# microsoft/ptgnn

Measured on AMD Instinct MI355X. Metric: edges/sec per MP layer, higher is better.
Workload: dtype f32; 1 GPU; cfg3: Graph2Class-style batch, 48 graphs N=115772, T0=8->T=17, E=625130 (incl. reverse+self), Typilus GGNN arch: 8 GGNN layers H=128 (+concat residual), max; hidden=128, mode=forward (inference), fp32, plan_build_in_step=True, message_rows=shared per (edge type, source) pair, parallelism=single GPU, minibatches_rotated=4

## Files before the change

### include/ptgnn_amd.h

```cpp
#ifndef PTGNN_AMD_H_
#define PTGNN_AMD_H_

#include <stddef.h>
#include <stdint.h>

#ifdef __cplusplus
extern "C" {
#endif

#pragma GCC visibility push(default)

#define PTGNN_AMD_VERSION 102

enum {
  PTGNN_AMD_OK = 0,
  PTGNN_AMD_EINVAL = -1,
  PTGNN_AMD_EUNSUPPORTED = -2,
  PTGNN_AMD_EHIP = -3,
  PTGNN_AMD_EWORKSPACE = -4,
  PTGNN_AMD_ERANGE = -5
};

enum { PTGNN_AMD_SUM = 0, PTGNN_AMD_MEAN = 1, PTGNN_AMD_MAX = 2, PTGNN_AMD_MIN = 3 };

// ... 157 lines not shown
                                int reduce, int epilogue, const float *ln_gamma,
                                const float *ln_beta, float ln_eps, float *out, int64_t ld_out,
                                int32_t *argout , int64_t num_edges,
                                int32_t hub_threshold, const int32_t *hub_entries ,
                                const int32_t *hub_count , void *hub_ws ,
                                size_t hub_ws_bytes, int32_t *hub_tickets ,
                                void *stream);
int ptgnn_amd_gather_reduce_rows_f32(const float *ysrc, int64_t ld_ysrc,
                                     const float *ydst , int64_t ld_ydst,
                                     const int32_t *rowptr, const int32_t *col,
                                     int32_t type_bits, int64_t num_nodes, int32_t msg_dim,
                                     int reduce, int epilogue, const float *ln_gamma,
                                     const float *ln_beta, float ln_eps, float *out, int64_t ld_out,
                                     int32_t *argout , int64_t num_edges,
                                     int32_t hub_threshold, const int32_t *hub_entries ,
                                     const int32_t *hub_count , void *hub_ws ,
                                     size_t hub_ws_bytes, int32_t *hub_tickets ,
                                     int64_t row_begin, int64_t row_end, void *stream);
int ptgnn_amd_row_headers(const int32_t *rowptr, const int32_t *entries, int64_t num_rows, int32_t *hdr, void *stream);
int ptgnn_amd_gather_reduce_hdr_f32(const float *ysrc, int64_t ld_ysrc,
                                    const float *ydst , int64_t ld_ydst,
                                    const int32_t *rowptr, const int32_t *col,
                                    int32_t type_bits, int64_t num_nodes, int32_t msg_dim,
                                    int reduce, int epilogue, const float *ln_gamma,
                                    const float *ln_beta, float ln_eps, float *out, int64_t ld_out,
                                    int32_t *argout , int64_t num_edges,
                                    int32_t hub_threshold, const int32_t *hub_entries ,
                                    const int32_t *hub_count , void *hub_ws ,
                                    size_t hub_ws_bytes, int32_t *hub_tickets ,
                                    int64_t row_begin, int64_t row_end,
                                    const int32_t *row_hdr , void *stream);

int ptgnn_amd_gather_update_supported(int32_t msg_dim, int32_t out_dim);
int ptgnn_amd_gather_update_f32(const float *msg, int64_t ld_msg, const int32_t *rowptr, const int32_t *col,
                                int32_t type_bits, int64_t num_nodes, int32_t msg_dim, int reduce, int epilogue,
                                const float *ln_gamma , const float *ln_beta , float ln_eps,
                                const float *w , const float *bias ,
                                int32_t out_dim, int act, float *out, int64_t ld_out, void *stream);

int ptgnn_amd_segment_mul_f32(const float *msg, int64_t ld_msg, const int32_t *rowptr, const int32_t *perm,
                              int64_t num_rows, int64_t num_edges, int32_t dim, float *out, int64_t ld_out,
                              void *stream);

int ptgnn_amd_gather_reduce_masked_f32(const float *grad, int64_t ld_grad, const int32_t *arg,
                                       const int32_t *rowptr, const int32_t *col,
                                       const int32_t *slot_of, int64_t num_rows, int32_t msg_dim,
                                       float *out, int64_t ld_out, int64_t num_edges,
                                       int32_t hub_threshold, const int32_t *hub_entries,
                                       const int32_t *hub_count, void *hub_ws ,
                                       size_t hub_ws_bytes, int32_t *hub_tickets ,
                                       void *stream);

int ptgnn_amd_linear_f32(const float *x, int64_t rows, int32_t k, int64_t ld_x, const float *w,
                         int32_t n_out, const float *bias, int act, float *y, int64_t ld_y,
                         void *stream);
int ptgnn_amd_linear_add_f32(const float *x, int64_t rows, int32_t k, int64_t ld_x, const float *w, int32_t n_out,
                             const float *bias , int act, const float *addend, int64_t ld_add, float *y,
                             int64_t ld_y, void *stream);

int ptgnn_amd_batch_offsets_i64(const int32_t *in, int64_t n_in, const int64_t *seg_start,
                                const int64_t *seg_add, int32_t num_segments, int64_t n_out,
                                int64_t *out, void *stream);

int ptgnn_amd_edge_linear_f32(const float *x, int64_t ld_x,
        int64_t num_rows ,
        int32_t state_dim,
                              const int64_t *const *src_per_type,
                              const int64_t *const *dst_per_type ,
                              const int64_t *edges_per_type, const float *const *w_per_type,
                              int32_t num_types, int32_t msg_dim, int act, float *msg,
                              int64_t ld_msg, void *stream);

int ptgnn_amd_edge_linear_feat_f32(const float *x, int64_t ld_x, int64_t num_rows, int32_t state_dim,
                                   const int64_t *const *src_per_type,
                                   const int64_t *const *dst_per_type ,
                                   const float *const *feat_per_type, int64_t ld_feat, int32_t feat_dim,
                                   const int64_t *edges_per_type, const float *const *w_per_type,
                                   int32_t num_types, int32_t msg_dim, int act, float *msg,
                                   int64_t ld_msg, void *stream);

int ptgnn_amd_edge_linear_dropout_f32(const float *x, int64_t ld_x,
        int64_t num_rows ,
        int32_t state_dim,
                                      const int64_t *const *src_per_type,
                                      const int64_t *edges_per_type, const float *const *w_per_type,
                                      int32_t num_types, int32_t msg_dim, float *msg, int64_t ld_msg,
                                      int dropout_mode, float dropout_p, uint64_t dropout_seed,
                                      void *stream);

size_t ptgnn_amd_dropout_bitmask_bytes(int64_t rows, int32_t width);
int ptgnn_amd_dropout_bitmask(int64_t rows, int32_t width, float dropout_p, uint64_t dropout_seed,
                              uint32_t *bits, void *stream);
int ptgnn_amd_edge_linear_masked_supported(int32_t state_dim, int32_t msg_dim, int dropout_mode);
int ptgnn_amd_edge_linear_masked_f32(const float *x, int64_t ld_x, int64_t num_rows, int32_t state_dim,
                                     const int64_t *const *src_per_type, const int64_t *edges_per_type,
                                     const float *const *w_per_type, int32_t num_types, int32_t msg_dim,
                                     float *msg, int64_t ld_msg, int dropout_mode, float dropout_p,
                                     const uint32_t *mask_bits, void *stream);
int ptgnn_amd_edge_weight_grad_masked_supported(int32_t state_dim, int32_t msg_dim);
int ptgnn_amd_edge_weight_grad_masked_f32(const float *x, int64_t ld_x, int64_t num_rows, int32_t state_dim,
                                          const int64_t *const *src_per_type, const int64_t *edges_per_type,
                                          const float *grad_msg, int64_t ld_grad_msg, int32_t num_types,
                                          int32_t msg_dim, float dropout_p, const uint32_t *mask_bits,
                                          float *grad_w, void *workspace, size_t workspace_bytes, void *stream);

size_t ptgnn_amd_edge_wgrad_workspace_bytes(int64_t num_edges, int32_t num_types, int32_t msg_dim,
                                            int32_t in_dim);
int ptgnn_amd_edge_weight_grad_f32(const float *x, int64_t ld_x,
        int64_t num_rows ,
        int32_t state_dim,
                                   const int64_t *const *src_per_type,
                                   const int64_t *const *dst_per_type ,
                                   const int64_t *edges_per_type, const float *grad_msg,
                                   int64_t ld_grad_msg, int32_t num_types, int32_t msg_dim,
                                   float dropout_p, uint64_t dropout_seed, float *grad_w,
                                   void *workspace, size_t workspace_bytes, void *stream);

int ptgnn_amd_linear_weight_grad_f32(const float *x, int64_t ld_x, int32_t k, const float *grad_y,
                                     int64_t ld_grad_y, int64_t rows, int32_t n_out, float *grad_w,
                                     float *grad_b , void *workspace,
                                     size_t workspace_bytes, void *stream);

int ptgnn_amd_gru_cell_train_f32(const float *a, int64_t ld_a, const float *h, int64_t ld_h,
                                 const float *w_ih, const float *w_hh, const float *b_ih,
                                 const float *b_hh, int64_t n, int32_t m, int32_t hd, float *out,
                                 int64_t ld_out, float *gates, void *stream);
int ptgnn_amd_gru_cell_backward_gates_f32(const float *grad_out, int64_t ld_grad_out, const float *gates,
                                          const float *h, int64_t ld_h, int64_t n, int32_t hd,
                                          float *d_gi, float *d_gh, float *d_h, void *stream);

int ptgnn_amd_segment_spread_f32(const float *grad, int64_t ld_grad, const int32_t *arg ,
                                 const int32_t *slot_row, const int32_t *perm, int64_t num_slots,
                                 int32_t dim, float *out, int64_t ld_out, void *stream);

int ptgnn_amd_row_epilogue_f32(const float *x, int64_t ld_x, int64_t rows, int32_t dim, int32_t flags,
                               const float *ln_gamma ,
                               const float *ln_beta , float ln_eps, float *y,
                               int64_t ld_y, void *stream);
size_t ptgnn_amd_row_epilogue_workspace_bytes(int64_t rows, int32_t dim);

int ptgnn_amd_act_dropout_backward_f32(const float *grad, const float *y, const uint8_t *keep, float scale, int act,
                                       int64_t n, float *out, void *stream);
int ptgnn_amd_row_epilogue_backward_f32(const float *x, int64_t ld_x, const float *grad_y, int64_t ld_gy,
                                        int64_t rows, int32_t dim, int32_t flags, const float *ln_gamma,
                                        float ln_eps, float *grad_x, int64_t ld_gx,
                                        float *grad_gamma ,
                                        float *grad_beta , void *workspace,
                                        size_t workspace_bytes, void *stream);

int ptgnn_amd_gru_cell_f32(const float *a, int64_t ld_a, const float *h, int64_t ld_h,
                           const float *w_ih, const float *w_hh, const float *b_ih,
                           const float *b_hh, int64_t n, int32_t m, int32_t hd, float *out,
                           int64_t ld_out, void *stream);

size_t ptgnn_amd_weighted_pool_workspace_bytes(int64_t num_segments, int64_t num_elements, int32_t dim);
int ptgnn_amd_weighted_pool_f32(const float *x, int64_t ld_x, const float *w, const int32_t *rowptr,
                                const int32_t *perm, int64_t num_segments, int64_t num_elements, int32_t dim,
                                float *out, int64_t ld_out, void *workspace, size_t workspace_bytes, void *stream);
size_t ptgnn_amd_weighted_pool_backward_workspace_bytes(int64_t num_elements, int32_t dim);
int ptgnn_amd_weighted_pool_backward_f32(const float *x, int64_t ld_x, const float *w, const int64_t *map,
                                         const float *grad_out, int64_t ld_go, int64_t num_elements, int32_t dim,
                                         float *grad_x, int64_t ld_gx, float *grad_w, void *workspace,
                                         size_t workspace_bytes, void *stream);

int ptgnn_amd_attention_pool_supported(int32_t dim, int32_t num_heads);
size_t ptgnn_amd_attention_pool_workspace_bytes(int64_t num_segments, int64_t num_elements, int32_t dim,
                                                int32_t num_heads);
int ptgnn_amd_attention_pool_f32(const float *x, int64_t ld_x, const float *u, const int32_t *rowptr,
                                 const int32_t *perm, int64_t num_segments, int64_t num_elements, int32_t dim,
                                 int32_t num_heads, float *out, float *stats, void *workspace, size_t workspace_bytes,
                                 void *stream);
size_t ptgnn_amd_attention_pool_backward_workspace_bytes(int64_t num_segments, int64_t num_elements, int32_t dim,
                                                         int32_t num_heads);
int ptgnn_amd_attention_pool_backward_f32(const float *x, int64_t ld_x, const float *u, const int32_t *rowptr,
                                          const int32_t *perm, int64_t num_segments, int64_t num_elements, int32_t dim,
                                          int32_t num_heads, const float *out, const float *stats,
                                          const float *grad_out, float *grad_x, int64_t ld_gx, float *grad_u,
                                          void *workspace, size_t workspace_bytes, void *stream);
int ptgnn_amd_head_projection_f32(int mode, const float *a ,
                                  const float *b , const float *w ,
                                  int64_t num_rows, int32_t num_heads, int32_t head_dim, int32_t dim, float scale,
                                  float *out, void *stream);

int ptgnn_amd_segment_scores_supported(int32_t dim, int32_t num_vectors);
size_t ptgnn_amd_segment_scores_workspace_bytes(int64_t num_segments, int64_t num_elements, int32_t dim,
                                                int32_t num_vectors);
int ptgnn_amd_segment_scores_f32(const float *y, int64_t ld_y, const float *v, const int32_t *rowptr,
                                 const int32_t *perm, int64_t num_segments, int64_t num_elements, int32_t dim,
                                 int32_t num_vectors, float *scores, float *lse, void *workspace, size_t workspace_bytes,
                                 void *stream);
size_t ptgnn_amd_segment_scores_backward_workspace_bytes(int64_t num_segments, int64_t num_elements, int32_t dim,
                                                         int32_t num_vectors);
int ptgnn_amd_segment_scores_backward_f32(const float *y, int64_t ld_y, const float *v, const int32_t *rowptr,
                                          const int32_t *perm, int64_t num_segments, int64_t num_elements, int32_t dim,
                                          int32_t num_vectors, const float *scores, const float *lse,
                                          const float *grad_scores, const float *grad_lse, float *grad_y, int64_t ld_gy,
                                          float *grad_v, void *workspace, size_t workspace_bytes, void *stream);

int ptgnn_amd_graph_norm_supported(int32_t dim);
size_t ptgnn_amd_graph_norm_workspace_bytes(int64_t num_segments, int64_t num_elements, int32_t dim);
int ptgnn_amd_graph_norm_f32(const float *x, int64_t ld_x, const float *gamma, const float *alpha, const float *bias,
                             float eps, const int32_t *rowptr, const int32_t *perm, int64_t num_segments,
                             int64_t num_elements, int32_t dim, float *y, int64_t ld_y, float *mean ,
                             void *workspace, size_t workspace_bytes, void *stream);
size_t ptgnn_amd_graph_norm_backward_workspace_bytes(int64_t num_segments, int64_t num_elements, int32_t dim);
int ptgnn_amd_graph_norm_backward_f32(const float *x, int64_t ld_x, const float *grad_y, int64_t ld_gy,
                                      const float *gamma, const float *alpha, float eps, const float *mean,
                                      const int32_t *rowptr, const int32_t *perm, int64_t num_segments,
                                      int64_t num_elements, int32_t dim,
                                      float *grad_x, int64_t ld_gx, float *grad_gamma, float *grad_alpha,
                                      float *grad_bias, void *workspace, size_t workspace_bytes, void *stream);

int ptgnn_amd_block_attention_supported(int32_t dk, int32_t dv);
int64_t ptgnn_amd_attention_windows_bound(int64_t num_graphs, int64_t num_rows, int32_t max_num_nodes);
int ptgnn_amd_attention_windows(const int32_t *rowptr, int64_t num_graphs, int64_t num_rows, int32_t max_num_nodes,
                                int32_t *windows, int64_t capacity, void *stream);
int ptgnn_amd_block_attention_f32(const float *kqv, int64_t ld_kqv, const int32_t *windows, int64_t num_windows,
                                  int64_t num_rows, int32_t max_num_nodes, int32_t num_heads, int32_t dk, int32_t dv,
                                  float dropout_p, uint64_t seed, float *out, int64_t ld_out, float *lse, void *stream);
size_t ptgnn_amd_block_attention_backward_workspace_bytes(int64_t num_rows, int32_t num_heads);
int ptgnn_amd_block_attention_backward_f32(const float *kqv, int64_t ld_kqv, const float *out, int64_t ld_out,
                                           const float *lse, const float *grad_out, int64_t ld_go,
                                           const int32_t *windows, int64_t num_windows, int64_t num_rows,
                                           int32_t max_num_nodes, int32_t num_heads, int32_t dk, int32_t dv,
                                           float dropout_p, uint64_t seed, float *grad_kqv, int64_t ld_gkqv,
                                           void *workspace, size_t workspace_bytes, void *stream);

int ptgnn_amd_egc_gather_combine_f32(const float *msg, int64_t ld_msg, const int32_t *rowptr, const int32_t *col,
                                     int32_t type_bits, int64_t num_nodes, int32_t num_heads, int32_t num_bases,
                                     int32_t head_dim, int reduce, const float *coef, int64_t ld_coef, float *out,
                                     int64_t ld_out, float *agg_out , int32_t *argout ,
                                     int64_t num_edges, int32_t hub_threshold,
                                     const int32_t *hub_entries , const int32_t *hub_count ,
                                     void *hub_ws , size_t hub_ws_bytes,
                                     int32_t *hub_tickets , void *stream);
int ptgnn_amd_egc_combine_f32(const float *agg, int64_t ld_agg, const float *coef, int64_t ld_coef, int64_t num_rows,
                              int32_t num_heads, int32_t num_bases, int32_t head_dim, float *out, int64_t ld_out,
                              void *stream);
int ptgnn_amd_egc_combine_backward_f32(const float *agg, int64_t ld_agg, const float *coef, int64_t ld_coef,
                                       const float *grad, int64_t ld_grad, int64_t num_rows, int32_t num_heads,
                                       int32_t num_bases, int32_t head_dim, float *grad_agg, int64_t ld_grad_agg,
                                       float *grad_coef, int64_t ld_grad_coef, void *stream);

int ptgnn_amd_pna_aggregate_f32(const float *ysrc, int64_t ld_y, const float *ydst , int64_t ld_yd,
                                const int32_t *rowptr, const int32_t *col, int32_t type_bits, int64_t num_nodes,
                                int32_t msg_dim, float delta, int epilogue, const float *ln_gamma ,
                                const float *ln_beta , float ln_eps, int32_t round_mode, float *out,
                                int64_t ld_out, int32_t *argmax , int32_t *argmin ,
                                float *agg_out , int64_t num_edges, void *stream);
int ptgnn_amd_pna_aggregate_backward_f32(const float *msg, int64_t ld_msg, const int32_t *rowptr, const int32_t *col,
                                         int64_t num_nodes, int32_t msg_dim, float delta, const float *agg,
                                         int64_t ld_agg, const int32_t *argmax, const int32_t *argmin,
                                         const float *grad, int64_t ld_grad, float *grad_msg, int64_t ld_grad_msg,
                                         int32_t round_mode, int64_t num_edges, void *stream);

int ptgnn_amd_gather_rows_f32(const float *x, int64_t ld_x, const int64_t *idx, int64_t n_idx,
                              int32_t dim, float *out, int64_t ld_out, void *stream);

int ptgnn_amd_embedding_bag_supported(int32_t dim, int32_t slots);
int ptgnn_amd_embedding_bag_f32(const float *table, int64_t ld_table, int64_t vocab, const int64_t *ids,
                                const int64_t *lengths, int64_t num_bags, int32_t slots, int32_t dim, int mode,
                                float *out, int64_t ld_out, int32_t *arg , void *stream);
int ptgnn_amd_embedding_bag_keys(const int64_t *ids, const int64_t *lengths, int64_t num_bags, int32_t slots,
                                 int64_t vocab, int64_t *src, int64_t *key, void *stream);
size_t ptgnn_amd_embedding_bag_backward_workspace_bytes(int64_t num_bags, int32_t slots, int32_t dim, int mode);
int ptgnn_amd_embedding_bag_backward_f32(const float *grad, int64_t ld_grad, const int64_t *lengths,
                                         const int32_t *arg , int64_t num_bags, int32_t slots,
                                         int64_t vocab, int32_t dim, int mode, const int32_t *rowptr,
                                         const int32_t *col, const int32_t *perm, float *grad_table, int64_t ld_gt,
                                         int32_t hub_threshold, const int32_t *hub_entries ,
                                         const int32_t *hub_count , void *hub_ws ,
                                         size_t hub_ws_bytes, int32_t *hub_tickets , void *workspace,
                                         size_t workspace_bytes, void *stream);

int ptgnn_amd_char_embed_supported(int32_t num_chars, int32_t window, int32_t dim);
int ptgnn_amd_char_embed_f32(const int64_t *chars, int64_t num_samples, int32_t length, int32_t num_chars,
                             int32_t window, const float *table, const float *bias , int32_t dim, int act,
                             float *out, int64_t ld_out, void *stream);
int32_t ptgnn_amd_char_embed_backward_chunk(void);
size_t ptgnn_amd_char_embed_backward_workspace_bytes(int64_t num_samples, int32_t num_chars, int32_t window,
                                                     int32_t dim);
int ptgnn_amd_char_embed_backward_f32(const float *grad, int64_t ld_grad, const float *a1, int64_t ld_a1,
                                      const int64_t *chars, int64_t num_samples, int32_t length, int32_t num_chars,
                                      int32_t window, int32_t dim, int act, float *grad_table,
                                      float *grad_bias , void *workspace, size_t workspace_bytes,
                                      void *stream);
int ptgnn_amd_window_linear_f32(const float *x, int64_t rows, int32_t c_in, int32_t window, int64_t ld_x,
                                const float *w, int32_t n_out, const float *bias , int act, float *y,
                                int64_t ld_y, void *stream);
int ptgnn_amd_window_weight_grad_f32(const float *x, int64_t rows, int32_t c_in, int32_t window, const float *grad_y,
                                     int64_t ld_grad_y, int32_t n_out, float *grad_w, float *grad_b ,
                                     void *workspace, size_t workspace_bytes, void *stream);
int ptgnn_amd_window_max_f32(const float *x, int64_t ld_x, int64_t num_samples, int32_t rows_per_sample, int32_t valid,
                             int32_t dim, float *out, int64_t ld_out, int32_t *arg , void *stream);
int ptgnn_amd_window_max_backward_f32(const float *grad, int64_t ld_grad, const int32_t *arg, int64_t num_samples,
                                      int32_t rows_per_sample, int32_t dim, float *grad_x, int64_t ld_gx, void *stream);

#define PTGNN_AMD_HEAD_TOTALS_BYTES 64
#define PTGNN_AMD_HEAD_METRICS_BYTES 32
enum { PTGNN_AMD_LOSS_SOFTMAX = 0, PTGNN_AMD_LOSS_SIGMOID = 1 };

size_t ptgnn_amd_logit_loss_workspace_bytes(int64_t rows);
int ptgnn_amd_logit_loss_f32(const float *logits, int64_t ld, int64_t rows, int32_t classes, int mode,
                             const void *targets , int64_t ld_t, float *lse,
                             int64_t *argmax , float *max_prob ,
                             float *row_loss , float *loss, void *totals, void *metrics ,
// ... 107 lines not shown
```

### ptgnn_amd/_lib.py

```python
import ctypes
import os
import threading

import torch

_HERE = os.path.dirname(os.path.abspath(__file__))
LIB_PATH = os.environ.get("PTGNN_AMD_LIB") or os.path.join(_HERE, "csrc", "libptgnn_amd.so")

_c = ctypes
_i64, _i32, _vp, _f32 = _c.c_int64, _c.c_int32, _c.c_void_p, _c.c_float

SIGNATURES = {
    "ptgnn_amd_version": (_c.c_int, []),
    "ptgnn_amd_last_error": (_c.c_char_p, []),
    "ptgnn_amd_set_gemm_mode": (_c.c_int, [_c.c_int]),
    "ptgnn_amd_get_gemm_mode": (_c.c_int, []),
    "ptgnn_amd_launch_count": (_i64, [_c.c_int]),
    "ptgnn_amd_launch_name": (_c.c_char_p, [_c.c_int]),
    "ptgnn_amd_csr_workspace_bytes": (_c.c_size_t, [_i64, _i64]),
    "ptgnn_amd_csr_control_bytes": (_c.c_size_t, []),
    "ptgnn_amd_set_plan_path": (_c.c_int, [_c.c_int]),
    "ptgnn_amd_type_bits": (_c.c_int, [_i32]),
    "ptgnn_amd_csr_build": (_c.c_int, [_vp, _vp, _vp, _i32, _i64, _i64, _c.c_int, _vp, _vp, _vp, _vp,
                                       _i32, _vp, _vp, _vp, _vp, _vp, _c.c_size_t, _vp]),
    "ptgnn_amd_hub_workspace_bytes": (_c.c_size_t, [_i64, _i32, _c.c_int]),
    "ptgnn_amd_hub_ticket_count": (_i64, [_i64, _i32]),
    "ptgnn_amd_hub_list": (_c.c_int, [_vp, _i64, _i32, _vp, _vp, _vp]),
    "ptgnn_amd_validate_indices": (_c.c_int, [_vp, _i64, _i64, _vp, _vp]),
    "ptgnn_amd_shard_index_workspace_bytes": (_c.c_size_t, [_i64]),
    "ptgnn_amd_shard_index": (_c.c_int, [_vp, _vp, _vp, _i32, _i64, _i64, _vp, _i32, _i64, _vp, _vp, _vp, _i64, _vp,
                                         _vp, _vp, _c.c_size_t, _vp]),
    "ptgnn_amd_unique_sources_workspace_bytes": (_c.c_size_t, [_i64, _i32]),
    "ptgnn_amd_edge_table_bytes": (_c.c_size_t, []),
    "ptgnn_amd_unique_sources": (_c.c_int, [_vp, _i64, _i32, _i32, _i64, _vp, _vp, _i64, _vp, _vp, _vp, _c.c_size_t,
                                            _vp]),
    "ptgnn_amd_edge_linear_shared_supported": (_c.c_int, [_i32, _i32, _i32]),
    "ptgnn_amd_edge_linear_shared_f32": (_c.c_int, [_vp, _i64, _i64, _i32, _vp, _vp, _i32, _i32, _c.c_int, _vp, _i64,
                                                    _vp]),
    "ptgnn_amd_gather_reduce_f32": (_c.c_int, [_vp, _i64, _vp, _i64, _vp, _vp, _i32, _i64, _i32, _c.c_int,
                                               _c.c_int, _vp, _vp, _f32, _vp, _i64, _vp, _i64, _i32, _vp,
                                               _vp, _vp, _c.c_size_t, _vp, _vp]),
    "ptgnn_amd_gather_reduce_rows_f32": (_c.c_int, [_vp, _i64, _vp, _i64, _vp, _vp, _i32, _i64, _i32, _c.c_int,
                                                    _c.c_int, _vp, _vp, _f32, _vp, _i64, _vp, _i64, _i32, _vp,
                                                    _vp, _vp, _c.c_size_t, _vp, _i64, _i64, _vp]),
    "ptgnn_amd_row_headers": (_c.c_int, [_vp, _vp, _i64, _vp, _vp]),
    "ptgnn_amd_gather_reduce_hdr_f32": (_c.c_int, [_vp, _i64, _vp, _i64, _vp, _vp, _i32, _i64, _i32, _c.c_int,
                                                   _c.c_int, _vp, _vp, _f32, _vp, _i64, _vp, _i64, _i32, _vp,
                                                   _vp, _vp, _c.c_size_t, _vp, _i64, _i64, _vp, _vp]),
    "ptgnn_amd_gather_update_supported": (_c.c_int, [_i32, _i32]),
    "ptgnn_amd_gather_update_f32": (_c.c_int, [_vp, _i64, _vp, _vp, _i32, _i64, _i32, _c.c_int, _c.c_int, _vp, _vp, _f32,
                                               _vp, _vp, _i32, _c.c_int, _vp, _i64, _vp]),
    "ptgnn_amd_gather_reduce_masked_f32": (_c.c_int, [_vp, _i64, _vp, _vp, _vp, _vp, _i64, _i32, _vp, _i64,
                                                      _i64, _i32, _vp, _vp, _vp, _c.c_size_t, _vp, _vp]),
    "ptgnn_amd_segment_mul_f32": (_c.c_int, [_vp, _i64, _vp, _vp, _i64, _i64, _i32, _vp, _i64, _vp]),
    "ptgnn_amd_linear_f32": (_c.c_int, [_vp, _i64, _i32, _i64, _vp, _i32, _vp, _c.c_int, _vp, _i64,
                                        _vp]),
    "ptgnn_amd_linear_add_f32": (_c.c_int, [_vp, _i64, _i32, _i64, _vp, _i32, _vp, _c.c_int, _vp, _i64, _vp, _i64,
                                            _vp]),
    "ptgnn_amd_batch_offsets_i64": (_c.c_int, [_vp, _i64, _vp, _vp, _i32, _i64, _vp, _vp]),
    "ptgnn_amd_edge_linear_f32": (_c.c_int, [_vp, _i64, _i64, _i32, _vp, _vp, _vp, _vp, _i32, _i32, _c.c_int, _vp,
                                             _i64, _vp]),
    "ptgnn_amd_edge_linear_feat_f32": (_c.c_int, [_vp, _i64, _i64, _i32, _vp, _vp, _vp, _i64, _i32, _vp, _vp, _i32, _i32,
                                                  _c.c_int, _vp, _i64, _vp]),
    "ptgnn_amd_edge_linear_dropout_f32": (_c.c_int, [_vp, _i64, _i64, _i32, _vp, _vp, _vp, _i32, _i32, _vp, _i64,
                                                     _c.c_int, _c.c_float, _c.c_uint64, _vp]),
    "ptgnn_amd_dropout_bitmask_bytes": (_c.c_size_t, [_i64, _i32]),
    "ptgnn_amd_dropout_bitmask": (_c.c_int, [_i64, _i32, _c.c_float, _c.c_uint64, _vp, _vp]),
    "ptgnn_amd_edge_linear_masked_supported": (_c.c_int, [_i32, _i32, _c.c_int]),
    "ptgnn_amd_edge_linear_masked_f32": (_c.c_int, [_vp, _i64, _i64, _i32, _vp, _vp, _vp, _i32, _i32, _vp, _i64,
                                                    _c.c_int, _c.c_float, _vp, _vp]),
    "ptgnn_amd_edge_weight_grad_masked_supported": (_c.c_int, [_i32, _i32]),
    "ptgnn_amd_edge_weight_grad_masked_f32": (_c.c_int, [_vp, _i64, _i64, _i32, _vp, _vp, _vp, _i64, _i32, _i32,
                                                         _c.c_float, _vp, _vp, _vp, _c.c_size_t, _vp]),
    "ptgnn_amd_edge_wgrad_workspace_bytes": (_c.c_size_t, [_i64, _i32, _i32, _i32]),
    "ptgnn_amd_edge_weight_grad_f32": (_c.c_int, [_vp, _i64, _i64, _i32, _vp, _vp, _vp, _vp, _i64, _i32, _i32,
                                                  _c.c_float, _c.c_uint64, _vp, _vp, _c.c_size_t, _vp]),
    "ptgnn_amd_linear_weight_grad_f32": (_c.c_int, [_vp, _i64, _i32, _vp, _i64, _i64, _i32, _vp, _vp, _vp,
                                                    _c.c_size_t, _vp]),
    "ptgnn_amd_segment_spread_f32": (_c.c_int, [_vp, _i64, _vp, _vp, _vp, _i64, _i32, _vp, _i64, _vp]),
    "ptgnn_amd_row_epilogue_f32": (_c.c_int, [_vp, _i64, _i64, _i32, _i32, _vp, _vp, _c.c_float, _vp, _i64, _vp]),
    "ptgnn_amd_row_epilogue_workspace_bytes": (_c.c_size_t, [_i64, _i32]),
    "ptgnn_amd_act_dropout_backward_f32": (_c.c_int, [_vp, _vp, _vp, _c.c_float, _c.c_int, _i64, _vp, _vp]),
    "ptgnn_amd_row_epilogue_backward_f32": (_c.c_int, [_vp, _i64, _vp, _i64, _i64, _i32, _i32, _vp, _c.c_float, _vp,
                                                       _i64, _vp, _vp, _vp, _c.c_size_t, _vp]),
    "ptgnn_amd_gru_cell_f32": (_c.c_int, [_vp, _i64, _vp, _i64, _vp, _vp, _vp, _vp, _i64, _i32, _i32,
                                          _vp, _i64, _vp]),
    "ptgnn_amd_gru_cell_train_f32": (_c.c_int, [_vp, _i64, _vp, _i64, _vp, _vp, _vp, _vp, _i64, _i32, _i32,
                                                _vp, _i64, _vp, _vp]),
    "ptgnn_amd_gru_cell_backward_gates_f32": (_c.c_int, [_vp, _i64, _vp, _vp, _i64, _i64, _i32, _vp, _vp, _vp,
                                                         _vp]),
    "ptgnn_amd_egc_gather_combine_f32": (_c.c_int, [_vp, _i64, _vp, _vp, _i32, _i64, _i32, _i32, _i32, _c.c_int, _vp,
                                                    _i64, _vp, _i64, _vp, _vp, _i64, _i32, _vp, _vp, _vp, _c.c_size_t,
                                                    _vp, _vp]),
    "ptgnn_amd_egc_combine_f32": (_c.c_int, [_vp, _i64, _vp, _i64, _i64, _i32, _i32, _i32, _vp, _i64, _vp]),
    "ptgnn_amd_egc_combine_backward_f32": (_c.c_int, [_vp, _i64, _vp, _i64, _vp, _i64, _i64, _i32, _i32, _i32, _vp,
                                                      _i64, _vp, _i64, _vp]),
    "ptgnn_amd_pna_aggregate_f32": (_c.c_int, [_vp, _i64, _vp, _i64, _vp, _vp, _i32, _i64, _i32, _f32, _c.c_int, _vp,
                                               _vp, _f32, _i32, _vp, _i64, _vp, _vp, _vp, _i64, _vp]),
    "ptgnn_amd_pna_aggregate_backward_f32": (_c.c_int, [_vp, _i64, _vp, _vp, _i64, _i32, _f32, _vp, _i64, _vp, _vp, _vp,
                                                        _i64, _vp, _i64, _i32, _i64, _vp]),
    "ptgnn_amd_gather_rows_f32": (_c.c_int, [_vp, _i64, _vp, _i64, _i32, _vp, _i64, _vp]),
    "ptgnn_amd_weighted_pool_workspace_bytes": (_c.c_size_t, [_i64, _i64, _i32]),
    "ptgnn_amd_weighted_pool_f32": (_c.c_int, [_vp, _i64, _vp, _vp, _vp, _i64, _i64, _i32, _vp, _i64, _vp, _c.c_size_t,
                                               _vp]),
    "ptgnn_amd_weighted_pool_backward_workspace_bytes": (_c.c_size_t, [_i64, _i32]),
    "ptgnn_amd_weighted_pool_backward_f32": (_c.c_int, [_vp, _i64, _vp, _vp, _vp, _i64, _i64, _i32, _vp, _i64, _vp, _vp,
                                                        _c.c_size_t, _vp]),
    "ptgnn_amd_attention_pool_supported": (_c.c_int, [_i32, _i32]),
    "ptgnn_amd_attention_pool_workspace_bytes": (_c.c_size_t, [_i64, _i64, _i32, _i32]),
    "ptgnn_amd_attention_pool_f32": (_c.c_int, [_vp, _i64, _vp, _vp, _vp, _i64, _i64, _i32, _i32, _vp, _vp, _vp,
                                                _c.c_size_t, _vp]),
    "ptgnn_amd_attention_pool_backward_workspace_bytes": (_c.c_size_t, [_i64, _i64, _i32, _i32]),
    "ptgnn_amd_attention_pool_backward_f32": (_c.c_int, [_vp, _i64, _vp, _vp, _vp, _i64, _i64, _i32, _i32, _vp, _vp,
                                                         _vp, _vp, _i64, _vp, _vp, _c.c_size_t, _vp]),
    "ptgnn_amd_head_projection_f32": (_c.c_int, [_c.c_int, _vp, _vp, _vp, _i64, _i32, _i32, _i32, _f32, _vp, _vp]),
    "ptgnn_amd_segment_scores_supported": (_c.c_int, [_i32, _i32]),
    "ptgnn_amd_segment_scores_workspace_bytes": (_c.c_size_t, [_i64, _i64, _i32, _i32]),
    "ptgnn_amd_segment_scores_f32": (_c.c_int, [_vp, _i64, _vp, _vp, _vp, _i64, _i64, _i32, _i32, _vp, _vp, _vp,
                                                _c.c_size_t, _vp]),
    "ptgnn_amd_segment_scores_backward_workspace_bytes": (_c.c_size_t, [_i64, _i64, _i32, _i32]),
    "ptgnn_amd_segment_scores_backward_f32": (_c.c_int, [_vp, _i64, _vp, _vp, _vp, _i64, _i64, _i32, _i32, _vp, _vp,
                                                         _vp, _vp, _vp, _i64, _vp, _vp, _c.c_size_t, _vp]),
    "ptgnn_amd_graph_norm_supported": (_c.c_int, [_i32]),
    "ptgnn_amd_graph_norm_workspace_bytes": (_c.c_size_t, [_i64, _i64, _i32]),
    "ptgnn_amd_graph_norm_f32": (_c.c_int, [_vp, _i64, _vp, _vp, _vp, _f32, _vp, _vp, _i64, _i64, _i32, _vp, _i64, _vp,
                                            _vp, _c.c_size_t, _vp]),
    "ptgnn_amd_graph_norm_backward_workspace_bytes": (_c.c_size_t, [_i64, _i64, _i32]),
    "ptgnn_amd_graph_norm_backward_f32": (_c.c_int, [_vp, _i64, _vp, _i64, _vp, _vp, _f32, _vp, _vp, _vp, _i64, _i64,
                                                     _i32, _vp, _i64, _vp, _vp, _vp, _vp, _c.c_size_t, _vp]),
    "ptgnn_amd_block_attention_supported": (_c.c_int, [_i32, _i32]),
    "ptgnn_amd_attention_windows_bound": (_i64, [_i64, _i64, _i32]),
    "ptgnn_amd_attention_windows": (_c.c_int, [_vp, _i64, _i64, _i32, _vp, _i64, _vp]),
    "ptgnn_amd_block_attention_f32": (_c.c_int, [_vp, _i64, _vp, _i64, _i64, _i32, _i32, _i32, _i32, _f32, _c.c_uint64,
                                                 _vp, _i64, _vp, _vp]),
    "ptgnn_amd_block_attention_backward_workspace_bytes": (_c.c_size_t, [_i64, _i32]),
    "ptgnn_amd_block_attention_backward_f32": (_c.c_int, [_vp, _i64, _vp, _i64, _vp, _vp, _i64, _vp, _i64, _i64, _i32,
                                                          _i32, _i32, _i32, _f32, _c.c_uint64, _vp, _i64, _vp,
                                                          _c.c_size_t, _vp]),
    "ptgnn_amd_embedding_bag_supported": (_c.c_int, [_i32, _i32]),
    "ptgnn_amd_embedding_bag_f32": (_c.c_int, [_vp, _i64, _i64, _vp, _vp, _i64, _i32, _i32, _c.c_int, _vp, _i64, _vp,
                                               _vp]),
    "ptgnn_amd_embedding_bag_keys": (_c.c_int, [_vp, _vp, _i64, _i32, _i64, _vp, _vp, _vp]),
    "ptgnn_amd_embedding_bag_backward_workspace_bytes": (_c.c_size_t, [_i64, _i32, _i32, _c.c_int]),
    "ptgnn_amd_embedding_bag_backward_f32": (_c.c_int, [_vp, _i64, _vp, _vp, _i64, _i32, _i64, _i32, _c.c_int, _vp, _vp,
                                                        _vp, _vp, _i64, _i32, _vp, _vp, _vp, _c.c_size_t, _vp, _vp,
                                                        _c.c_size_t, _vp]),
    "ptgnn_amd_char_embed_supported": (_c.c_int, [_i32, _i32, _i32]),
    "ptgnn_amd_char_embed_f32": (_c.c_int, [_vp, _i64, _i32, _i32, _i32, _vp, _vp, _i32, _c.c_int, _vp, _i64, _vp]),
    "ptgnn_amd_char_embed_backward_chunk": (_i32, []),
    "ptgnn_amd_char_embed_backward_workspace_bytes": (_c.c_size_t, [_i64, _i32, _i32, _i32]),
    "ptgnn_amd_char_embed_backward_f32": (_c.c_int, [_vp, _i64, _vp, _i64, _vp, _i64, _i32, _i32, _i32, _i32, _c.c_int,
                                                     _vp, _vp, _vp, _c.c_size_t, _vp]),
    "ptgnn_amd_window_linear_f32": (_c.c_int, [_vp, _i64, _i32, _i32, _i64, _vp, _i32, _vp, _c.c_int, _vp, _i64, _vp]),
    "ptgnn_amd_window_weight_grad_f32": (_c.c_int, [_vp, _i64, _i32, _i32, _vp, _i64, _i32, _vp, _vp, _vp, _c.c_size_t,
                                                    _vp]),
    "ptgnn_amd_window_max_f32": (_c.c_int, [_vp, _i64, _i64, _i32, _i32, _i32, _vp, _i64, _vp, _vp]),
    "ptgnn_amd_window_max_backward_f32": (_c.c_int, [_vp, _i64, _vp, _i64, _i32, _i32, _vp, _i64, _vp]),
    "ptgnn_amd_logit_loss_workspace_bytes": (_c.c_size_t, [_i64]),
    "ptgnn_amd_logit_loss_f32": (_c.c_int, [_vp, _i64, _i64, _i32, _c.c_int, _vp, _i64, _vp, _vp, _vp, _vp, _vp, _vp, _vp,
                                            _vp, _c.c_size_t, _vp]),
    "ptgnn_amd_logit_loss_backward_f32": (_c.c_int, [_vp, _i64, _i64, _i32, _c.c_int, _vp, _i64, _vp, _vp, _vp, _vp, _i64,
                                                     _vp]),
    "ptgnn_amd_candidate_scores_supported": (_c.c_int, [_i32]),
    "ptgnn_amd_candidate_scores_workspace_bytes": (_c.c_size_t, [_i64]),
    "ptgnn_amd_candidate_scores_f32": (_c.c_int, [_vp, _i64, _i64, _vp, _vp, _vp, _vp, _vp, _i64, _i64, _i32, _vp, _vp,
                                                  _vp, _vp, _vp, _vp, _vp, _vp, _vp, _c.c_size_t, _vp]),
    "ptgnn_amd_candidate_scores_backward_workspace_bytes": (_c.c_size_t, [_i64, _i32]),
    "ptgnn_amd_candidate_scores_backward_f32": (_c.c_int, [_vp, _i64, _i64, _vp, _vp, _vp, _vp, _vp, _i64, _i64, _i32,
                                                           _vp, _vp, _vp, _vp, _vp, _vp, _vp, _vp, _vp, _c.c_size_t,
                                                           _vp]),
    "ptgnn_amd_vocab_loss_workspace_bytes": (_c.c_size_t, [_i64, _i32]),
    "ptgnn_amd_vocab_loss_f32": (_c.c_int, [_vp, _i64, _i64, _i32, _vp, _vp, _vp, _vp, _vp, _vp, _vp, _c.c_size_t,
                                            _vp]),
    "ptgnn_amd_vocab_loss_backward_workspace_bytes": (_c.c_size_t, [_i64, _i32]),
    "ptgnn_amd_vocab_loss_backward_f32": (_c.c_int, [_vp, _i64, _i64, _i32, _vp, _vp, _vp, _vp, _vp, _vp, _vp, _i64, _vp,
                                                     _vp, _vp, _c.c_size_t, _vp]),
    "ptgnn_amd_copy_loss_finish_workspace_bytes": (_c.c_size_t, [_i64]),
    "ptgnn_amd_copy_loss_finish_f32": (_c.c_int, [_vp, _vp, _vp, _vp, _i64, _vp, _i64, _i32, _vp, _vp, _vp, _vp,
                                                  _c.c_size_t, _vp]),
    "ptgnn_amd_decode_step_workspace_bytes": (_c.c_size_t, [_i64, _i32, _i32]),
    "ptgnn_amd_decode_step_f32": (_c.c_int, [_vp, _i64, _vp, _vp, _vp, _vp, _vp, _vp, _i64, _i64, _i32, _i32, _i64, _i64,
                                             _i32, _i32, _vp, _vp, _vp, _vp, _vp, _vp, _vp, _c.c_size_t, _vp]),
    "ptgnn_amd_beam_step_workspace_bytes": (_c.c_size_t, [_i64, _i64, _i32, _i32, _i32]),
    "ptgnn_amd_beam_step_f32": (_c.c_int, [_vp, _i64, _vp, _vp, _vp, _vp, _vp, _vp, _i64, _i64, _i32, _i32, _i32, _i64,
                                           _i64, _i32, _i32, _vp, _vp, _vp, _vp, _vp, _vp, _vp, _vp, _vp, _vp, _vp, _vp,
                                           _c.c_size_t, _vp]),
    "ptgnn_amd_half_supported": (_c.c_int, [_c.c_int, _i32, _i32, _c.c_int]),
    "ptgnn_amd_half_linear": (_c.c_int, [_vp, _i64, _i32, _i64, _vp, _i32, _vp, _c.c_int, _c.c_int, _vp, _i64, _vp]),
    "ptgnn_amd_half_gru_cell": (_c.c_int, [_vp, _i64, _vp, _i64, _vp, _vp, _vp, _vp, _i64, _i32, _i32, _c.c_int, _vp,
                                           _i64, _vp]),
    "ptgnn_amd_linear_weight_grad16": (_c.c_int, [_vp, _i64, _i32, _vp, _i64, _i64, _i32, _c.c_int, _vp, _vp, _vp,
                                                  _c.c_size_t, _vp]),
    "ptgnn_amd_wgrad16_workspace_bytes": (_c.c_size_t, [_i64, _i32, _i32]),
    "ptgnn_amd_wgrad16_chunk_rows": (_i64, [_i64, _i32, _i32]),
    "ptgnn_amd_gru_cell_train16": (_c.c_int, [_vp, _i64, _vp, _i64, _vp, _vp, _vp, _vp, _i64, _i32, _i32, _c.c_int, _vp,
                                              _i64, _vp, _vp]),
    "ptgnn_amd_linear_add16": (_c.c_int, [_vp, _i64, _i32, _i64, _vp, _i32, _vp, _c.c_int, _c.c_int, _vp, _i64, _vp, _i64,
                                          _vp]),
    "ptgnn_amd_edge_linear16_supported": (_c.c_int, [_i32, _i32, _i32, _c.c_int]),
    "ptgnn_amd_edge_linear16": (_c.c_int, [_vp, _i64, _i64, _i32, _vp, _vp, _vp, _i32, _i32, _c.c_int, _c.c_int, _vp,
                                           _i64, _vp]),
    "ptgnn_amd_edge_linear16_shared": (_c.c_int, [_vp, _i64, _i64, _i32, _vp, _vp, _i32, _i32, _c.c_int, _c.c_int, _vp,
                                                  _i64, _vp]),
    "ptgnn_amd_edge_dst_linear16_supported": (_c.c_int, [_i32, _i32, _i32, _c.c_int]),
    "ptgnn_amd_edge_dst_linear16": (_c.c_int, [_vp, _i64, _i64, _i32, _vp, _vp, _vp, _vp, _i32, _i32, _c.c_int, _c.c_int,
                                               _vp, _i64, _vp]),
}

MIN_VERSION = 102

_lock = threading.Lock()
_lib = None


EUNSUPPORTED = -2


class PtgnnAmdError(RuntimeError):
    pass


def load():
    global _lib
    if _lib is not None:
        return _lib
    with _lock:
        if _lib is None:
            if not os.path.exists(LIB_PATH):
                raise PtgnnAmdError(
                    f"{LIB_PATH} is missing: build it with `python -m ptgnn_amd.build` "
                    "(ptgnn_amd has no CPU/eager fallback by design)")
            lib = ctypes.CDLL(LIB_PATH)
            for name, (res, args) in SIGNATURES.items():
                fn = getattr(lib, name)
                fn.restype, fn.argtypes = res, args
            have = lib.ptgnn_amd_version()
            if have < MIN_VERSION:
                raise PtgnnAmdError(f"{LIB_PATH} reports ABI version {have}, this host needs >= {MIN_VERSION}: "
                                    "rebuild it with `python -m ptgnn_amd.build --force`")
# ... 9 lines not shown
```

### ptgnn_amd/csrc/dense_f32.hip

```cpp
#include <stdlib.h>

#include <type_traits>

#include "dense_common.h"
#include "stream_gemm.h"

namespace ptgnn_amd {
namespace {

template <bool ALIGNED, int ACT, int NJ>
__global__ __launch_bounds__(256, (NJ == 1 ? 4 : 3)) void k_linear_tlp(
    const float *__restrict__ x, int64_t rows, int K, int64_t ld_x, const float *__restrict__ w,
    int n_out, const float *__restrict__ bias, float *__restrict__ y, int64_t ld_y,
    int64_t num_tiles, int col_tiles, int vec_store) {
  constexpr int BN = 64 * NJ;
  constexpr int B_FLOATS = BN * LDS_LD;
  constexpr int SLAB_LD = 32 * NJ + 4;
  constexpr int SLAB_FLOATS = 32 * SLAB_LD;
  constexpr int OPER = TILE_FLOATS + B_FLOATS;
  constexpr int kLds = OPER > 4 * SLAB_FLOATS ? OPER : 4 * SLAB_FLOATS;
  __shared__ __attribute__((aligned(16))) float smem[kLds];
  float *const As = smem, *const Bs = smem + TILE_FLOATS;

  const int64_t tile = xcd_swizzle(blockIdx.x, gridDim.x);
// ... 255 lines not shown
  }
}

__global__ __launch_bounds__(256) void k_gru_gates_backward(const float *__restrict__ g, int64_t ld_g,
                                                            const float *__restrict__ gates,
                                                            const float *__restrict__ h, int64_t ld_h,
                                                            int64_t n, int H, float *__restrict__ d_gi,
                                                            float *__restrict__ d_gh,
                                                            float *__restrict__ d_h) {
  const int q = H / 4;
  const int64_t total = n * q;
  for (int64_t i = blockIdx.x * (int64_t)256 + threadIdx.x; i < total; i += (int64_t)gridDim.x * 256) {
    const int64_t row = i / q;
    const int c = (int)(i - row * q) * 4;
    const float4 gv = *reinterpret_cast<const float4 *>(g + row * ld_g + c);
    const float4 hv = *reinterpret_cast<const float4 *>(h + row * ld_h + c);
    const float *gp = gates + row * (int64_t)(4 * H) + c;
    const float4 r = *reinterpret_cast<const float4 *>(gp);
    const float4 z = *reinterpret_cast<const float4 *>(gp + H);
    const float4 nn = *reinterpret_cast<const float4 *>(gp + 2 * H);
    const float4 hn = *reinterpret_cast<const float4 *>(gp + 3 * H);
    float4 o_r, o_z, o_n, o_hn, o_h;
#define PTGNN_GRU_BWD(C)                                         \
    {                                                            \
      const float dn = gv.C * (1.0f - z.C);                      \
      const float dz = gv.C * (hv.C - nn.C);                     \
      const float dnp = dn * (1.0f - nn.C * nn.C);               \
      o_h.C = gv.C * z.C;                                        \
      o_n.C = dnp;                                               \
      o_hn.C = dnp * r.C;                                        \
      o_r.C = (dnp * hn.C) * (r.C * (1.0f - r.C));               \
      o_z.C = dz * (z.C * (1.0f - z.C));                         \
    }
    PTGNN_GRU_BWD(x) PTGNN_GRU_BWD(y) PTGNN_GRU_BWD(z) PTGNN_GRU_BWD(w)
#undef PTGNN_GRU_BWD
    float *gi = d_gi + row * (int64_t)(3 * H) + c, *gh = d_gh + row * (int64_t)(3 * H) + c;
    *reinterpret_cast<float4 *>(gi) = o_r;
    *reinterpret_cast<float4 *>(gi + H) = o_z;
    *reinterpret_cast<float4 *>(gi + 2 * H) = o_n;
    *reinterpret_cast<float4 *>(gh) = o_r;
    *reinterpret_cast<float4 *>(gh + H) = o_z;
    *reinterpret_cast<float4 *>(gh + 2 * H) = o_hn;
    *reinterpret_cast<float4 *>(d_h + row * (int64_t)H + c) = o_h;
  }
}

}

int num_compute_units() {
  static int cus = 0;
  if (cus == 0) {
    int dev = 0;
    hipDeviceProp_t prop;
    if (hipGetDevice(&dev) == hipSuccess && hipGetDeviceProperties(&prop, dev) == hipSuccess)
      cus = prop.multiProcessorCount;
    if (cus <= 0) cus = 256;
  }
  return cus;
}

static int linear_nj() {
  static int nj = -1;
  if (nj < 0) {
    const char *e = getenv("PTGNN_AMD_LINEAR_NJ");
    nj = e ? atoi(e) : 0;
    if (nj < 0 || nj > 2) nj = 0;
  }
  return nj;
}

}

using namespace ptgnn_amd;

static int linear_launch(const float *x, int64_t rows, int32_t k, int64_t ld_x, const float *w, int32_t n_out,
                         const float *bias, int act, float *y, int64_t ld_y, void *stream_) {
  if (stream_linear(x, rows, k, ld_x, w, n_out, bias, act, y, ld_y, (hipStream_t)stream_)) {
    PTGNN_LAUNCH_CHECK();
    return PTGNN_AMD_OK;
  }
  int nj = linear_nj();
  if (nj == 0) nj = n_out <= 128 ? 1 : 2;
  const int bn = 64 * nj;
  const int64_t row_tiles = (rows + 127) / 128;
  const int col_tiles = (n_out + bn - 1) / bn;
  const int64_t num_tiles = row_tiles * col_tiles;
  PTGNN_REQUIRE(num_tiles < ((int64_t)1 << 31), PTGNN_AMD_EUNSUPPORTED, "linear: too many tiles");
  const unsigned grid = (unsigned)xcd_padded_blocks(num_tiles);
  const bool al = (k % 4 == 0) && (ld_x % 4 == 0) && aligned16(x) && aligned16(w);
  const int vec_store = ((ld_y % 4 == 0) && aligned16(y) ? 1 : 0) | ((bias && aligned16(bias) && n_out % 4 == 0) ? 2 : 0);
  hipStream_t st = (hipStream_t)stream_;
#define PTGNN_LINEAR_LAUNCH(AL, ACT, NJ)                                                         \
  k_linear_tlp<AL, ACT, NJ><<<grid, 256, 0, st>>>(x, rows, k, ld_x, w, n_out, bias, y, ld_y,     \
                                                  num_tiles, col_tiles, vec_store)
#define PTGNN_LINEAR_ACT(AL, NJ)                                                          \
  do {                                                                                    \
    if (act == PTGNN_AMD_ACT_TANH) PTGNN_LINEAR_LAUNCH(AL, PTGNN_AMD_ACT_TANH, NJ);       \
    else if (act == PTGNN_AMD_ACT_RELU) PTGNN_LINEAR_LAUNCH(AL, PTGNN_AMD_ACT_RELU, NJ);  \
    else PTGNN_LINEAR_LAUNCH(AL, PTGNN_AMD_ACT_NONE, NJ);                                 \
  } while (0)
  if (al) { if (nj == 1) PTGNN_LINEAR_ACT(true, 1); else PTGNN_LINEAR_ACT(true, 2); }
  else    { if (nj == 1) PTGNN_LINEAR_ACT(false, 1); else PTGNN_LINEAR_ACT(false, 2); }
#undef PTGNN_LINEAR_ACT
#undef PTGNN_LINEAR_LAUNCH
  PTGNN_LAUNCH_CHECK();
  count_launch(PTGNN_AMD_KERNEL_TILE_LINEAR);
  return PTGNN_AMD_OK;
}

extern "C" int ptgnn_amd_linear_f32(const float *x, int64_t rows, int32_t k, int64_t ld_x,
                                    const float *w, int32_t n_out, const float *bias, int act,
                                    float *y, int64_t ld_y, void *stream_) {
  PTGNN_REQUIRE(rows >= 0 && k > 0 && n_out > 0, PTGNN_AMD_EINVAL, "linear: bad sizes");
  PTGNN_REQUIRE(act >= 0 && act <= PTGNN_AMD_ACT_RELU, PTGNN_AMD_EINVAL, "linear: bad act");
  if (rows == 0) return PTGNN_AMD_OK;
  PTGNN_REQUIRE(x && w && y && ld_x >= k && ld_y >= n_out, PTGNN_AMD_EINVAL, "linear: null/ld");
  return linear_launch(x, rows, k, ld_x, w, n_out, bias, act, y, ld_y, stream_);
}

extern "C" int ptgnn_amd_window_linear_f32(const float *x, int64_t rows, int32_t c_in, int32_t window, int64_t ld_x,
                                           const float *w, int32_t n_out, const float *bias, int act, float *y,
                                           int64_t ld_y, void *stream_) {
  PTGNN_REQUIRE(rows >= 0 && c_in > 0 && window > 0 && n_out > 0 && (int64_t)c_in * window < ((int64_t)1 << 31),
                PTGNN_AMD_EINVAL, "window_linear: bad sizes");
  PTGNN_REQUIRE(act >= 0 && act <= PTGNN_AMD_ACT_RELU, PTGNN_AMD_EINVAL, "window_linear: bad act");
  if (rows == 0) return PTGNN_AMD_OK;
  PTGNN_REQUIRE(x && w && y && ld_x >= c_in && ld_y >= n_out, PTGNN_AMD_EINVAL, "window_linear: null/ld");
  PTGNN_REQUIRE(window == 1 || ld_x == c_in, PTGNN_AMD_EINVAL,
                "window_linear: a window spans rows only where they are packed (ld_x=%lld, c_in=%d)", (long long)ld_x,
                c_in);
  return linear_launch(x, rows, c_in * window, ld_x, w, n_out, bias, act, y, ld_y, stream_);
}

extern "C" int ptgnn_amd_linear_add_f32(const float *x, int64_t rows, int32_t k, int64_t ld_x, const float *w,
                                        int32_t n_out, const float *bias, int act, const float *addend,
                                        int64_t ld_add, float *y, int64_t ld_y, void *stream_) {
  PTGNN_REQUIRE(rows >= 0 && k > 0 && n_out > 0, PTGNN_AMD_EINVAL, "linear_add: bad sizes");
  PTGNN_REQUIRE(act >= 0 && act <= PTGNN_AMD_ACT_RELU, PTGNN_AMD_EINVAL, "linear_add: bad act");
  if (rows == 0) return PTGNN_AMD_OK;
  PTGNN_REQUIRE(x && w && y && addend && ld_x >= k && ld_y >= n_out && ld_add >= n_out, PTGNN_AMD_EINVAL,
                "linear_add: null/ld");
  PTGNN_REQUIRE(addend != y, PTGNN_AMD_EINVAL, "linear_add: in-place accumulation is not supported");
  if (stream_linear(x, rows, k, ld_x, w, n_out, bias, act, y, ld_y, (hipStream_t)stream_, addend, ld_add)) {
    PTGNN_LAUNCH_CHECK();
    return PTGNN_AMD_OK;
  }
  set_error("linear_add: rows=%lld k=%d n_out=%d is not a shape of the streaming GEMM (use ptgnn_amd_linear_f32 and add)",
            (long long)rows, k, n_out);
  return PTGNN_AMD_EUNSUPPORTED;
}

static int gru_launch(const float *a, int64_t ld_a, const float *h, int64_t ld_h, const float *w_ih,
                      const float *w_hh, const float *b_ih, const float *b_hh, int64_t n, int32_t m,
                      int32_t hd, float *out, int64_t ld_out, float *gates, void *stream_) {
  PTGNN_REQUIRE(n >= 0 && m > 0 && hd > 0, PTGNN_AMD_EINVAL, "gru_cell: bad sizes");
  if (n == 0) return PTGNN_AMD_OK;
  PTGNN_REQUIRE(a && h && w_ih && w_hh && b_ih && b_hh && out, PTGNN_AMD_EINVAL, "gru_cell: null");
  PTGNN_REQUIRE(ld_a >= m && ld_h >= hd && ld_out >= hd, PTGNN_AMD_EINVAL, "gru_cell: bad ld");
  PTGNN_REQUIRE(out != h, PTGNN_AMD_EINVAL, "gru_cell: in-place update is not supported");
  if (stream_gru(a, ld_a, h, ld_h, w_ih, w_hh, b_ih, b_hh, n, m, hd, out, ld_out, gates, (hipStream_t)stream_)) {
    PTGNN_LAUNCH_CHECK();
    return PTGNN_AMD_OK;
  }
  const int64_t row_tiles = (n + 127) / 128;
  const int col_tiles = (hd + 31) / 32;
  const int64_t num_tiles = row_tiles * col_tiles;
  PTGNN_REQUIRE(num_tiles < ((int64_t)1 << 31), PTGNN_AMD_EUNSUPPORTED, "gru_cell: too many tiles");
  const unsigned grid = (unsigned)xcd_padded_blocks(num_tiles);
  const bool al = (m % 4 == 0) && (hd % 4 == 0) && (ld_a % 4 == 0) && (ld_h % 4 == 0) &&
                  aligned16(a) && aligned16(h) && aligned16(w_ih) && aligned16(w_hh);
  if (al)
    k_gru<true><<<grid, 256, 0, (hipStream_t)stream_>>>(a, ld_a, h, ld_h, w_ih, w_hh, b_ih, b_hh, n, m, hd,
                                                        out, ld_out, num_tiles, col_tiles, gates);
  else
    k_gru<false><<<grid, 256, 0, (hipStream_t)stream_>>>(a, ld_a, h, ld_h, w_ih, w_hh, b_ih, b_hh, n, m, hd,
                                                         out, ld_out, num_tiles, col_tiles, gates);
  PTGNN_LAUNCH_CHECK();
  count_launch(PTGNN_AMD_KERNEL_TILE_GRU);
  return PTGNN_AMD_OK;
}

extern "C" int ptgnn_amd_gru_cell_f32(const float *a, int64_t ld_a, const float *h, int64_t ld_h,
                                      const float *w_ih, const float *w_hh, const float *b_ih,
                                      const float *b_hh, int64_t n, int32_t m, int32_t hd,
                                      float *out, int64_t ld_out, void *stream_) {
  return gru_launch(a, ld_a, h, ld_h, w_ih, w_hh, b_ih, b_hh, n, m, hd, out, ld_out, nullptr, stream_);
}

extern "C" int ptgnn_amd_gru_cell_train_f32(const float *a, int64_t ld_a, const float *h, int64_t ld_h,
                                            const float *w_ih, const float *w_hh, const float *b_ih,
                                            const float *b_hh, int64_t n, int32_t m, int32_t hd,
                                            float *out, int64_t ld_out, float *gates, void *stream_) {
  PTGNN_REQUIRE(gates != nullptr || n == 0, PTGNN_AMD_EINVAL, "gru_cell_train: gates is null");
  return gru_launch(a, ld_a, h, ld_h, w_ih, w_hh, b_ih, b_hh, n, m, hd, out, ld_out, gates, stream_);
}

extern "C" int ptgnn_amd_gru_cell_backward_gates_f32(const float *grad_out, int64_t ld_grad_out,
                                                     const float *gates, const float *h, int64_t ld_h,
                                                     int64_t n, int32_t hd, float *d_gi, float *d_gh,
                                                     float *d_h, void *stream_) {
  PTGNN_REQUIRE(n >= 0 && hd > 0, PTGNN_AMD_EINVAL, "gru_cell_backward_gates: bad sizes");
  if (n == 0) return PTGNN_AMD_OK;
  PTGNN_REQUIRE(grad_out && gates && h && d_gi && d_gh && d_h, PTGNN_AMD_EINVAL,
                "gru_cell_backward_gates: null pointer");
  PTGNN_REQUIRE(hd % 4 == 0 && ld_grad_out % 4 == 0 && ld_h % 4 == 0 && ld_grad_out >= hd && ld_h >= hd &&
                    aligned16(grad_out) && aligned16(gates) && aligned16(h) && aligned16(d_gi) &&
                    aligned16(d_gh) && aligned16(d_h),
                PTGNN_AMD_EUNSUPPORTED, "gru_cell_backward_gates: needs hd %% 4 == 0 and 16-byte aligned rows");
  const int64_t items = n * (hd / 4);
  int64_t blocks = (items + 255) / 256;
  if (blocks > 65536) blocks = 65536;
  k_gru_gates_backward<<<(unsigned)blocks, 256, 0, (hipStream_t)stream_>>>(grad_out, ld_grad_out, gates, h,
                                                                          ld_h, n, hd, d_gi, d_gh, d_h);
  PTGNN_LAUNCH_CHECK();
  return PTGNN_AMD_OK;
}
```

### ptgnn_amd/csrc/stream_gemm.h

```cpp
#pragma once
#include "common.h"

namespace ptgnn_amd {

constexpr int kStreamMaxTypes = 64;

struct StreamEdgeTable {
  const int64_t *src[kStreamMaxTypes];
  const int64_t *dst[kStreamMaxTypes];
  const float *w[kStreamMaxTypes];
  int64_t edge_off[kStreamMaxTypes + 1];
  int32_t unit_off[kStreamMaxTypes + 1];
  int32_t wg_off[kStreamMaxTypes + 1];
  int32_t num_types;
};

int num_compute_units();

int stream_gemm_mode();
void stream_gemm_set_mode(int mode);

int stream_linear(const float *x, int64_t rows, int32_t k, int64_t ld_x, const float *w, int32_t n_out,
                  const float *bias, int act, float *y, int64_t ld_y, hipStream_t st, const float *addend = nullptr,
                  int64_t ld_add = 0);
int stream_gru(const float *a, int64_t ld_a, const float *h, int64_t ld_h, const float *w_ih,
               const float *w_hh, const float *b_ih, const float *b_hh, int64_t n, int32_t m, int32_t hd,
               float *out, int64_t ld_out, float *gates, hipStream_t st);
int stream_edge_supported(int32_t state_dim, int32_t msg_dim, int use_dst);
int stream_edge_masked_supported(int32_t state_dim, int32_t msg_dim);
struct StreamEdgeMask {
  int mode;
  const uint32_t *bits;
  int ld, col0;
  float scale;
};
int stream_edge(const StreamEdgeTable &tab, const float *x, int64_t ld_x, int64_t num_rows, int32_t state_dim,
                int use_dst, int32_t msg_dim, int act, float *msg, int64_t ld_msg, int64_t msg_row_base,
                hipStream_t st, const StreamEdgeMask *mask = nullptr);

int edge_table_budget();
int stream_edge_indirect(const StreamEdgeTable *tab_dev, const float *const *w_per_type, int num_types, const float *x,
                         int64_t ld_x, int64_t num_rows, int32_t state_dim, int32_t msg_dim, int act, float *msg,
                         int64_t ld_msg, hipStream_t st);

}
```

### ptgnn_amd/csrc/stream_gemm.hip

```cpp
#include <stdlib.h>

#include "dense_common.h"
#include <atomic>

#include "stream_gemm.h"

namespace ptgnn_amd {
namespace {

using u32x4 = __attribute__((ext_vector_type(4))) uint32_t;

constexpr int kLdsBudget = 160 * 1024;
constexpr size_t kEpiBytes = 16 + 8 * 8 * 36 * sizeof(float);

__device__ __forceinline__ f32x16 zero16() {
  f32x16 v;
#pragma unroll
  for (int r = 0; r < 16; ++r) v[r] = 0.f;
  return v;
}

struct ARows {
  const float *c0, *c1, *n0, *n1;
};
// ... 12 lines not shown
template <int NBLK, int NACC, int PH, bool GRU>
__device__ __forceinline__ void chunk_f32(f32x16 (&acc)[NACC], float4 (&buf)[4], float4 (&bcur)[NBLK],
                                          const float *bl, int cbs, int kofs, int kofs_next, const ARows &rows,
                                          int cnext, int ch0, int nch) {
#pragma unroll
  for (int g = 0; g < 4; ++g) {
    float4 bn[NBLK];
    const int ko = g < 3 ? kofs + (g + 1) * 8 : kofs_next;
#pragma unroll
    for (int n = 0; n < NBLK; ++n) bn[n] = *reinterpret_cast<const float4 *>(bl + n * cbs + ko);
    __builtin_amdgcn_sched_barrier(0);
    const float4 a = buf[g];
#define PTGNN_STEP(C)                                                                     \
    _Pragma("unroll") for (int n = 0; n < NBLK; ++n) {                                    \
      const int t = (GRU && PH == 1 && n == NBLK - 1) ? NACC - 1 : n;                     \
      acc[t] = __builtin_amdgcn_mfma_f32_32x32x2f32(a.C, bcur[n].C, acc[t], 0, 0, 0);     \
    }
    PTGNN_STEP(x) PTGNN_STEP(y) PTGNN_STEP(z) PTGNN_STEP(w)
#undef PTGNN_STEP
    __builtin_amdgcn_sched_barrier(0);
#pragma unroll
    for (int n = 0; n < NBLK; ++n) bcur[n] = bn[n];
  }
#pragma unroll
  for (int g = 0; g < 4; ++g) {
    buf[g] = load_piece(rows, cnext, ch0, nch, g);
    __builtin_amdgcn_sched_barrier(0);
  }
}

struct Slab {
  int ld;
  __device__ __forceinline__ Slab(int K, int ) { ld = K + 4; }
  static size_t bytes(int K, int rows) { return (size_t)rows * (K + 4) * 4; }

  __device__ __forceinline__ void put4(float *smem, int r, int k, float4 v) const {
    *reinterpret_cast<float4 *>(smem + r * ld + k) = v;
  }
};

template <int NT, typename SrcFn, typename LiveFn>
__device__ __forceinline__ void fill_slab(float *smem, const Slab &sl, int rows, int kq, SrcFn src, LiveFn live) {
  constexpr int UB = 8;
  const int total = rows * kq;
  for (int i0 = threadIdx.x; i0 < total; i0 += NT * UB) {
    float4 v[UB];
    int rr[UB], qq[UB];
#pragma unroll
    for (int u = 0; u < UB; ++u) {
      const int i = i0 + u * NT;
      const int ic = i < total ? i : total - 1;
      rr[u] = ic / kq;
      qq[u] = ic - rr[u] * kq;
    }
#pragma unroll
    for (int u = 0; u < UB; ++u) {
      v[u] = *reinterpret_cast<const float4 *>(src(rr[u], qq[u]));
      __builtin_amdgcn_sched_barrier(0);
    }
#pragma unroll
    for (int u = 0; u < UB; ++u) {
      if (i0 + u * NT < total) sl.put4(smem, rr[u], qq[u] * 4, live(rr[u]) ? v[u] : make_float4(0.f, 0.f, 0.f, 0.f));
    }
  }
}

template <int NBLK, int NACC, bool GRU>
__device__ __forceinline__ void unit_kloop(f32x16 (&acc)[NACC], float4 (&a0)[4], float4 (&a1)[4],
                                           const float *smem, const Slab &sl, int li, int hi,
                                           const ARows &rows, int ch0, int nch) {
  const float *bl = smem + li * sl.ld + hi * 4;
  const int cbs = 32 * sl.ld;
  const int e0 = GRU ? ch0 : nch;
  float4 bcur[NBLK];
#pragma unroll
  for (int n = 0; n < NBLK; ++n) bcur[n] = *reinterpret_cast<const float4 *>(bl + n * cbs);
  for (int c = 0; c < e0; c += 2) {
    const int kn = c + 2 < nch ? c * 32 + 64 : 0;
    chunk_f32<NBLK, NACC, 0, GRU>(acc, a0, bcur, bl, cbs, c * 32, c * 32 + 32, rows, c + 2, ch0, nch);
    chunk_f32<NBLK, NACC, 0, GRU>(acc, a1, bcur, bl, cbs, c * 32 + 32, kn, rows, c + 3, ch0, nch);
  }
  if constexpr (GRU) {
    for (int c = ch0; c < nch; c += 2) {
      const int kn = c + 2 < nch ? c * 32 + 64 : 0;
      chunk_f32<NBLK, NACC, 1, GRU>(acc, a0, bcur, bl, cbs, c * 32, c * 32 + 32, rows, c + 2, ch0, nch);
      chunk_f32<NBLK, NACC, 1, GRU>(acc, a1, bcur, bl, cbs, c * 32 + 32, kn, rows, c + 3, ch0, nch);
    }
  }
}

__device__ __forceinline__ void prologue_loads(float4 (&a0)[4], float4 (&a1)[4], const ARows &rows, int ch0,
                                               int nch) {
#pragma unroll
  for (int g = 0; g < 4; ++g) {
    a0[g] = load_piece(rows, 0, ch0, nch, g);
    __builtin_amdgcn_sched_barrier(0);
  }
#pragma unroll
  for (int g = 0; g < 4; ++g) {
    a1[g] = load_piece(rows, 1, ch0, nch, g);
    __builtin_amdgcn_sched_barrier(0);
  }
}

__device__ __forceinline__ void unit_fence() {
  __builtin_amdgcn_s_waitcnt(0x0F70);
  __builtin_amdgcn_sched_barrier(0);
}

__device__ __forceinline__ int claim_unit(int *counter) {
  int v = 0;
  if ((threadIdx.x & 63) == 0) v = atomicAdd(counter, 1);
  return __builtin_amdgcn_readfirstlane(v);
}

#ifndef PTGNN_TAIL_SPLIT
#define PTGNN_TAIL_SPLIT 1
#endif
constexpr bool kSplitGru = PTGNN_TAIL_SPLIT != 0;

constexpr int kTqLd = 36;
constexpr int kTqFloats = 8 * kTqLd;

__device__ __forceinline__ float4 tq_transpose(float *tq, int lane, int li, int hi, float v0, float v1, float v2,
                                               float v3) {
  float *w = tq + (4 * hi) * kTqLd + li;
  w[0] = v0; w[kTqLd] = v1; w[2 * kTqLd] = v2; w[3 * kTqLd] = v3;
  __builtin_amdgcn_wave_barrier();
  const float4 o = *reinterpret_cast<const float4 *>(tq + (lane >> 3) * kTqLd + (lane & 7) * 4);
  __builtin_amdgcn_wave_barrier();
  return o;
}

__device__ __forceinline__ void tq_untranspose(float *tq, int lane, int li, int hi, float4 in, float (&v)[4]) {
  *reinterpret_cast<float4 *>(tq + (lane >> 3) * kTqLd + (lane & 7) * 4) = in;
  __builtin_amdgcn_wave_barrier();
  const float *r = tq + (4 * hi) * kTqLd + li;
  v[0] = r[0]; v[1] = r[kTqLd]; v[2] = r[2 * kTqLd]; v[3] = r[3 * kTqLd];
  __builtin_amdgcn_wave_barrier();
}

using u32x4 = __attribute__((ext_vector_type(4))) uint32_t;

__device__ __forceinline__ __amdgpu_buffer_rsrc_t rows_descriptor(float *base , int64_t ld, int64_t rows_left,
                                                                  int width ) {
  const uint64_t b = reinterpret_cast<uint64_t>(base);
  const uint32_t lo = __builtin_amdgcn_readfirstlane((uint32_t)b), hi = __builtin_amdgcn_readfirstlane((uint32_t)(b >> 32));
  const int64_t rows = rows_left < 32 ? rows_left : 32;
  const int64_t bytes = rows > 0 ? ((rows - 1) * ld + width) * 4 : 0;
  return __builtin_amdgcn_make_buffer_rsrc(reinterpret_cast<float *>(((uint64_t)hi << 32) | lo), 0,
                                           __builtin_amdgcn_readfirstlane((int)bytes), 0x00020000);
}

__device__ __forceinline__ void store_row4(__amdgpu_buffer_rsrc_t rsrc, int lane_bytes, int uniform_bytes, float4 o) {
  const u32x4 v = {__float_as_uint(o.x), __float_as_uint(o.y), __float_as_uint(o.z), __float_as_uint(o.w)};
  __builtin_amdgcn_raw_buffer_store_b128(v, rsrc, lane_bytes + uniform_bytes, 0, 0);
}

template <int ACT, bool BIAS = true>
__device__ __forceinline__ void store_block_tq(const f32x16 &c, float *tq, float *yblk ,
                                               int64_t ld_y, float bv, int64_t rows_left, int lane, int li, int hi,
                                               const float *addblk = nullptr, int64_t ld_add = 0) {
  auto val = [&](int r) { return BIAS ? act_apply<ACT>(c[r] + bv) : act_apply<ACT>(c[r]); };
  float4 addv[4];
  if (addblk) {
#pragma unroll
    for (int q = 0; q < 4; ++q) {
      int64_t r = 8 * q + (lane >> 3);
      r = r < rows_left ? r : rows_left - 1;
      addv[q] = *reinterpret_cast<const float4 *>(addblk + r * ld_add + (lane & 7) * 4);
    }
  }
#ifdef PTGNN_GLOBAL_STORES
  float *yp = yblk + (int64_t)(lane >> 3) * ld_y + (lane & 7) * 4;
#pragma unroll
  for (int q = 0; q < 4; ++q) {
    float4 o = tq_transpose(tq, lane, li, hi, val(4 * q), val(4 * q + 1), val(4 * q + 2), val(4 * q + 3));
    if (addblk) { o.x += addv[q].x; o.y += addv[q].y; o.z += addv[q].z; o.w += addv[q].w; }
    if (8 * q + (lane >> 3) < rows_left) *reinterpret_cast<float4 *>(yp + (int64_t)(8 * q) * ld_y) = o;
  }
#else
  const __amdgpu_buffer_rsrc_t rsrc = rows_descriptor(yblk, ld_y, rows_left, 32);
  const int ldb = (int)ld_y * 4;
  const int lane_bytes = (lane >> 3) * ldb + (lane & 7) * 16;
#pragma unroll
  for (int q = 0; q < 4; ++q) {
    float4 o = tq_transpose(tq, lane, li, hi, val(4 * q), val(4 * q + 1), val(4 * q + 2), val(4 * q + 3));
    if (addblk) { o.x += addv[q].x; o.y += addv[q].y; o.z += addv[q].z; o.w += addv[q].w; }
    store_row4(rsrc, lane_bytes, 8 * q * ldb, o);
  }
#endif
}

struct LinearArgs {
  const float *x; int64_t rows; int K; int64_t ld_x;
  const float *w; int n_out; const float *bias; int act;
  float *y; int64_t ld_y;
  const float *addend; int64_t ld_add;
  int nrb, ncs, rps, run_len;
  int lds_floats;
  int vec_store;
};

template <int ACT>
__device__ __forceinline__ void store_block(const f32x16 &c, float *yp, int64_t ld_y, float bv, int64_t row0,
                                            int64_t rows, int hi) {
  if (row0 + 32 <= rows) {
#pragma unroll
    for (int r = 0; r < 16; ++r)
      yp[(int64_t)((r & 3) + 8 * (r >> 2)) * ld_y] = act_apply<ACT>(c[r] + bv);
  } else {
#pragma unroll
    for (int r = 0; r < 16; ++r) {
      const int rr = (r & 3) + 8 * (r >> 2);
      if (row0 + rr + 4 * hi < rows) yp[(int64_t)rr * ld_y] = act_apply<ACT>(c[r] + bv);
    }
  }
}

template <int NB>
__device__ __forceinline__ void linear_epilogue(const LinearArgs &p, f32x16 (&acc)[NB], float *tq, int64_t row0,
                                                int col_base, int lane, int li, int hi) {
#pragma unroll
  for (int n = 0; n < NB; ++n) {
    const int col = col_base + n * 32 + li;
    if (col_base + n * 32 < p.n_out) {
      const float bv = p.bias ? p.bias[col] : 0.f;
      if (p.vec_store) {
        float *yb = p.y + row0 * p.ld_y + col_base + n * 32;
        const int64_t left = p.rows - row0;
        if (p.bias) {
#pragma unroll
          for (int r = 0; r < 16; ++r) acc[n][r] += bv;
        }
        const float *ab = p.addend ? p.addend + row0 * p.ld_add + col_base + n * 32 : nullptr;
        if (p.act == PTGNN_AMD_ACT_TANH) store_block_tq<PTGNN_AMD_ACT_TANH, false>(acc[n], tq, yb, p.ld_y, 0.f, left, lane, li, hi, ab, p.ld_add);
        else if (p.act == PTGNN_AMD_ACT_RELU) store_block_tq<PTGNN_AMD_ACT_RELU, false>(acc[n], tq, yb, p.ld_y, 0.f, left, lane, li, hi, ab, p.ld_add);
        else store_block_tq<PTGNN_AMD_ACT_NONE, false>(acc[n], tq, yb, p.ld_y, 0.f, left, lane, li, hi, ab, p.ld_add);
      } else {
        float *yp = p.y + (row0 + 4 * hi) * p.ld_y + col;
        if (p.act == PTGNN_AMD_ACT_TANH) store_block<PTGNN_AMD_ACT_TANH>(acc[n], yp, p.ld_y, bv, row0, p.rows, hi);
        else if (p.act == PTGNN_AMD_ACT_RELU) store_block<PTGNN_AMD_ACT_RELU>(acc[n], yp, p.ld_y, bv, row0, p.rows, hi);
        else store_block<PTGNN_AMD_ACT_NONE>(acc[n], yp, p.ld_y, bv, row0, p.rows, hi);
      }
    }
    acc[n] = zero16();
  }
}

template <int NB>
__global__ __launch_bounds__(512, 2) void k_stream_linear(LinearArgs p) {
  extern __shared__ __attribute__((aligned(16))) float smem[];
  constexpr int NT = 512, BN = 32 * NB;
  const int b = blockIdx.x, G = gridDim.x;
  int slab, part;
  if (G % (kNumXcd * p.ncs) == 0) {
    const int xcd = b % kNumXcd, j = b / kNumXcd;
    slab = j % p.ncs;
    part = xcd + kNumXcd * (j / p.ncs);
  } else {
    slab = b / p.rps;
    part = b % p.rps;
  }
  const int rb0 = part * p.run_len;
  const int rb1 = rb0 + p.run_len < p.nrb ? rb0 + p.run_len : p.nrb;
  if (rb0 >= rb1) return;
  const int count = rb1 - rb0;

  const Slab sl(p.K, BN);
  int *counter = reinterpret_cast<int *>(smem + p.lds_floats);
  float *const tq = smem + p.lds_floats + 4 + (threadIdx.x >> 6) * kTqFloats;
  if (threadIdx.x == 0) *counter = 0;
  const int col_base = slab * BN;
  fill_slab<NT>(smem, sl, BN, p.K >> 2,
                       [&](int r, int q) {
                         const int wr = col_base + r < p.n_out ? col_base + r : p.n_out - 1;
                         return p.w + (int64_t)wr * p.K + q * 4;
                       },
                       [&](int r) { return col_base + r < p.n_out; });
  __syncthreads();

  const int lane = threadIdx.x & 63;
  const int li = lane & 31, hi = lane >> 5;
  const int nch = p.K >> 5;
  const int lofs = lane_piece_offset(hi);
  auto rowp = [&](int u) {
    int64_t row = (int64_t)(rb0 + (u < count ? u : count - 1)) * 32 + li;
    row = row < p.rows ? row : p.rows - 1;
    return p.x + row * p.ld_x + lofs;
  };
  int cur = claim_unit(counter);
  if (cur >= count) return;
  int nxt = claim_unit(counter);
  ARows rows;
  rows.c0 = rows.c1 = rowp(cur);
  rows.n0 = rows.n1 = rowp(nxt);
  float4 a0[4], a1[4];
  prologue_loads(a0, a1, rows, nch, nch);
  f32x16 acc[NB];
#pragma unroll
  for (int n = 0; n < NB; ++n) acc[n] = zero16();

  while (cur < count) {
    const int nn = claim_unit(counter);
    unit_fence();
    unit_kloop<NB, NB, false>(acc, a0, a1, smem, sl, li, hi, rows, nch, nch);
    const int64_t row0 = (int64_t)(rb0 + cur) * 32;
    linear_epilogue<NB>(p, acc, tq, row0, col_base, lane, li, hi);
    cur = nxt;
    nxt = nn;
    rows.c0 = rows.c1 = rows.n0;
    rows.n0 = rows.n1 = rowp(nxt);
  }
}

struct GruArgs {
  const float *a; int64_t ld_a; const float *h; int64_t ld_h;
  const float *w_ih, *w_hh, *b_ih, *b_hh;
  int64_t n; int M, H;
  float *out; int64_t ld_out; float *gates;
  int nrb, ncs, rps, run_len;
  int lds_floats;
  int split;
};

constexpr int kGruSplitUnits = 6;
constexpr size_t kGruSplitBytes = (size_t)kGruSplitUnits * 2 * 4096 + 32;

__device__ __forceinline__ float fast_sigmoid(float v) {
  return __builtin_amdgcn_rcpf(1.0f + __builtin_amdgcn_exp2f(-1.4426950408889634f * v));
}

using f32x2 = __attribute__((ext_vector_type(2))) float;
__device__ __forceinline__ f32x2 splat2(float v) { return f32x2{v, v}; }
__device__ __forceinline__ f32x2 rcp_1_plus_exp2(f32x2 t) {
  const f32x2 d = f32x2{__builtin_amdgcn_exp2f(t.x), __builtin_amdgcn_exp2f(t.y)} + splat2(1.0f);
  return f32x2{__builtin_amdgcn_rcpf(d.x), __builtin_amdgcn_rcpf(d.y)};
}

__device__ __forceinline__ void gru_epilogue(const GruArgs &p, const f32x16 (&acc)[4], float *tq, int64_t row0,
                                             int j0, int lane, int li, int hi, float bir, float biz, float bin,
                                             float bhr, float bhz, float bhn) {
  const int trow = lane >> 3, tcol = (lane & 7) * 4;
#ifndef PTGNN_GLOBAL_STORES
  const __amdgpu_buffer_rsrc_t out_rsrc = rows_descriptor(p.out + row0 * p.ld_out + j0, p.ld_out, p.n - row0, 32);
  const __amdgpu_buffer_rsrc_t gate_rsrc =
      rows_descriptor(p.gates ? p.gates + row0 * (int64_t)(4 * p.H) + j0 : p.out, 4 * (int64_t)p.H, p.n - row0, 3 * p.H + 32);
#endif
#pragma unroll
  for (int q = 0; q < 4; ++q) {
    int64_t hrow = row0 + 8 * q + trow;
    const bool rvalid = hrow < p.n;
    hrow = rvalid ? hrow : p.n - 1;
    float hp[4];
    tq_untranspose(tq, lane, li, hi, *reinterpret_cast<const float4 *>(p.h + hrow * p.ld_h + j0 + tcol), hp);
    float res[4], rg[4], zg[4], ng[4], hn[4];
    {
#pragma clang fp contract(off)
#pragma unroll
      for (int i = 0; i < 4; i += 2) {
        const int r = 4 * q + i;
        const f32x2 ar = {acc[0][r], acc[0][r + 1]}, az = {acc[1][r], acc[1][r + 1]};
        const f32x2 an = {acc[2][r], acc[2][r + 1]}, ah = {acc[3][r], acc[3][r + 1]};
        const f32x2 hp2 = {hp[i], hp[i + 1]};
        const f32x2 r2 = rcp_1_plus_exp2(((ar + splat2(bir)) + splat2(bhr)) * splat2(-1.4426950408889634f));
        const f32x2 z2 = rcp_1_plus_exp2(((az + splat2(biz)) + splat2(bhz)) * splat2(-1.4426950408889634f));
        const f32x2 h2 = ah + splat2(bhn);
        const f32x2 pre = (an + splat2(bin)) + r2 * h2;
        const f32x2 n2 = splat2(2.0f) * rcp_1_plus_exp2(pre * splat2(-2.8853900817779268f)) - splat2(1.0f);
        const f32x2 o2 = (splat2(1.0f) - z2) * n2 + z2 * hp2;
        rg[i] = r2.x; rg[i + 1] = r2.y; zg[i] = z2.x; zg[i + 1] = z2.y; hn[i] = h2.x; hn[i + 1] = h2.y;
        ng[i] = n2.x; ng[i + 1] = n2.y; res[i] = o2.x; res[i + 1] = o2.y;
      }
    }
    const float4 o = tq_transpose(tq, lane, li, hi, res[0], res[1], res[2], res[3]);
#ifdef PTGNN_GLOBAL_STORES
    if (rvalid) *reinterpret_cast<float4 *>(p.out + hrow * p.ld_out + j0 + tcol) = o;
#else
    store_row4(out_rsrc, trow * (int)p.ld_out * 4 + tcol * 4, 8 * q * (int)p.ld_out * 4, o);
#endif
    if (p.gates) {
      const float4 o_r = tq_transpose(tq, lane, li, hi, rg[0], rg[1], rg[2], rg[3]);
      const float4 o_z = tq_transpose(tq, lane, li, hi, zg[0], zg[1], zg[2], zg[3]);
      const float4 o_n = tq_transpose(tq, lane, li, hi, ng[0], ng[1], ng[2], ng[3]);
      const float4 o_h = tq_transpose(tq, lane, li, hi, hn[0], hn[1], hn[2], hn[3]);
#ifdef PTGNN_GLOBAL_STORES
      float *gp = p.gates + hrow * (int64_t)(4 * p.H) + j0 + tcol;
      if (rvalid) {
        *reinterpret_cast<float4 *>(gp) = o_r;
        *reinterpret_cast<float4 *>(gp + p.H) = o_z;
        *reinterpret_cast<float4 *>(gp + 2 * p.H) = o_n;
        *reinterpret_cast<float4 *>(gp + 3 * p.H) = o_h;
      }
#else
      const int gl = trow * 16 * p.H + tcol * 4, gu = 8 * q * 16 * p.H;
      store_row4(gate_rsrc, gl, gu, o_r);
      store_row4(gate_rsrc, gl, gu + 4 * p.H, o_z);
      store_row4(gate_rsrc, gl, gu + 8 * p.H, o_n);
      store_row4(gate_rsrc, gl, gu + 12 * p.H, o_h);
#endif
    }
  }
}

__global__ __launch_bounds__(512, 2) void k_stream_gru(GruArgs p) {
  extern __shared__ __attribute__((aligned(16))) float smem[];
  constexpr int NT = 512;
  const int b = blockIdx.x, G = gridDim.x;
  int slab, part;
  if (G % (kNumXcd * p.ncs) == 0) {
    const int xcd = b % kNumXcd, j = b / kNumXcd;
    slab = j % p.ncs;
    part = xcd + kNumXcd * (j / p.ncs);
  } else {
    slab = b / p.rps;
    part = b % p.rps;
  }
  const int rb0 = part * p.run_len;
  const int rb1 = rb0 + p.run_len < p.nrb ? rb0 + p.run_len : p.nrb;
  if (rb0 >= rb1) return;
  const int count = rb1 - rb0;

  const int K = p.M + p.H;
  const Slab sl(K, 96);
  int *counter = reinterpret_cast<int *>(smem + p.lds_floats);
  float *const tq = smem + p.lds_floats + 4 + (threadIdx.x >> 6) * kTqFloats;
  float *const xch = smem + p.lds_floats + 4 + 8 * kTqFloats;
  int *const flags = reinterpret_cast<int *>(xch + kGruSplitUnits * 2048);
  if (threadIdx.x == 0) counter[0] = counter[1] = 0;
  if (kSplitGru && p.split && threadIdx.x < 8) flags[threadIdx.x] = 0;
  const int j0 = slab * 32;
  {
    const int mq = p.M >> 2;
    fill_slab<NT>(smem, sl, 96, K >> 2,
                         [&](int r, int q) {
                           const int gate = r >> 5, jj = j0 + (r & 31);
                           return q < mq ? p.w_ih + ((int64_t)gate * p.H + jj) * p.M + q * 4
                                         : p.w_hh + ((int64_t)gate * p.H + jj) * p.H + (q - mq) * 4;
                         },
                         [](int) { return true; });
  }
  __syncthreads();

  const int lane = threadIdx.x & 63;
  const int li = lane & 31, hi = lane >> 5;
  const int ch0 = p.M >> 5, nch = K >> 5;
  const int lofs = lane_piece_offset(hi);
  auto clampr = [&](int u) {
    const int64_t row = (int64_t)(rb0 + (u < count ? u : count - 1)) * 32 + li;
    return row < p.n ? row : p.n - 1;
  };
  int tail = kSplitGru && p.split ? count & 7 : 0;
  if (tail > kGruSplitUnits) tail = 0;
  const int whole = count - tail;
  const int j = j0 + li;
  const float bir = p.b_ih[j], biz = p.b_ih[p.H + j], bin = p.b_ih[2 * p.H + j];
  const float bhr = p.b_hh[j], bhz = p.b_hh[p.H + j], bhn = p.b_hh[2 * p.H + j];

  int cur = claim_unit(counter);
  if (cur < whole) {
    int nxt = claim_unit(counter);
    ARows rows;
    {
      const int64_t r0 = clampr(cur), r1 = clampr(nxt);
      rows.c0 = p.a + r0 * p.ld_a + lofs; rows.c1 = p.h + r0 * p.ld_h + lofs;
      rows.n0 = p.a + r1 * p.ld_a + lofs; rows.n1 = p.h + r1 * p.ld_h + lofs;
    }
    float4 a0[4], a1[4];
    prologue_loads(a0, a1, rows, ch0, nch);
    f32x16 acc[4];
#pragma unroll
    for (int n = 0; n < 4; ++n) acc[n] = zero16();

    while (cur < whole) {
      const int nn = claim_unit(counter);
      unit_fence();
      unit_kloop<3, 4, true>(acc, a0, a1, smem, sl, li, hi, rows, ch0, nch);
      gru_epilogue(p, acc, tq, (int64_t)(rb0 + cur) * 32, j0, lane, li, hi, bir, biz, bin, bhr, bhz, bhn);
#pragma unroll
      for (int n = 0; n < 4; ++n) acc[n] = zero16();
      cur = nxt;
      nxt = nn;
      rows.c0 = rows.n0; rows.c1 = rows.n1;
      const int64_t r1 = clampr(nxt);
      rows.n0 = p.a + r1 * p.ld_a + lofs; rows.n1 = p.h + r1 * p.ld_h + lofs;
    }
  }
  if (tail > 0) {
    const int nsub = 3 * tail;
    int s = claim_unit(counter + 1);
    if (s >= nsub) return;
    const int cbs = 32 * sl.ld;
    auto rows_of = [&](int q, const float *&ra, const float *&rh) {
      const int64_t r = clampr(whole + (q < nsub ? q : nsub - 1) / 3);
      ra = p.a + r * p.ld_a + lofs; rh = p.h + r * p.ld_h + lofs;
    };
    ARows rows;
    rows_of(s, rows.c0, rows.c1);
    rows_of(s + 8, rows.n0, rows.n1);
    float4 a0[4], a1[4];
    prologue_loads(a0, a1, rows, ch0, nch);
    for (; s < nsub; s += 8) {
      const int unit = s / 3, grp = s - unit * 3;
      float4 *const park = reinterpret_cast<float4 *>(xch) + (unit * 2) * 256 + lane;
      unit_fence();
      if (grp < 2) {
        f32x16 acc[1] = {zero16()};
        unit_kloop<1, 1, false>(acc, a0, a1, smem + grp * cbs, sl, li, hi, rows, ch0, nch);
#pragma unroll
        for (int q = 0; q < 4; ++q)
          park[grp * 256 + q * 64] = make_float4(acc[0][4 * q], acc[0][4 * q + 1], acc[0][4 * q + 2], acc[0][4 * q + 3]);
        if (lane == 0) __hip_atomic_fetch_add(flags + unit, 1, __ATOMIC_RELEASE, __HIP_MEMORY_SCOPE_WORKGROUP);
      } else {
        f32x16 nh[2] = {zero16(), zero16()};
        unit_kloop<1, 2, true>(nh, a0, a1, smem + 2 * cbs, sl, li, hi, rows, ch0, nch);
        while (__hip_atomic_load(flags + unit, __ATOMIC_ACQUIRE, __HIP_MEMORY_SCOPE_WORKGROUP) < 2) __builtin_amdgcn_s_sleep(1);
        f32x16 acc[4];
#pragma unroll
        for (int g = 0; g < 2; ++g) {
#pragma unroll
          for (int q = 0; q < 4; ++q) {
            const float4 v = park[g * 256 + q * 64];
            acc[g][4 * q] = v.x; acc[g][4 * q + 1] = v.y; acc[g][4 * q + 2] = v.z; acc[g][4 * q + 3] = v.w;
          }
        }
        acc[2] = nh[0]; acc[3] = nh[1];
        gru_epilogue(p, acc, tq, (int64_t)(rb0 + whole + unit) * 32, j0, lane, li, hi, bir, biz, bin, bhr, bhz, bhn);
      }
      rows.c0 = rows.n0; rows.c1 = rows.n1;
      rows_of(s + 16, rows.n0, rows.n1);
    }
  }
}

constexpr int kRingPanel = 64;
constexpr int kRingLd = kRingPanel + 4;
constexpr int kRingPanelFloats = 96 * kRingLd;
constexpr int kRingWaves = 4;

__global__ __launch_bounds__(kRingWaves * 64, 2) void k_stream_gru_ring(GruArgs p) {
  extern __shared__ __attribute__((aligned(16))) float smem[];
  const int b = blockIdx.x, G = gridDim.x;
  int slab, part;
  if (G % (kNumXcd * p.ncs) == 0) {
    const int xcd = b % kNumXcd, j = b / kNumXcd;
    slab = j % p.ncs;
    part = xcd + kNumXcd * (j / p.ncs);
  } else {
    slab = b / p.rps;
    part = b % p.rps;
  }
  const int rb0 = part * p.run_len;
  const int rb1 = rb0 + p.run_len < p.nrb ? rb0 + p.run_len : p.nrb;
  if (rb0 >= rb1) return;
// ... 516 lines not shown
          (void)yp;
#ifndef PTGNN_GLOBAL_STORES
          const __amdgpu_buffer_rsrc_t msg_rsrc = rows_descriptor(p.msg + out_row0 * p.ld_msg, p.ld_msg, left, 32 * NB);
          const int ldb = (int)p.ld_msg * 4;
#endif
#pragma unroll
          for (int n = 0; n < NB; ++n) {
#pragma unroll
            for (int r = 0; r < 4; ++r) {
#ifdef PTGNN_GLOBAL_STORES
              float *const yr = 8 * r + srow < left ? yp + (int64_t)(8 * r) * p.ld_msg : sink;
#endif
              float4 o = tq_transpose(tq, lane, li, hi, acc[n][4 * r], acc[n][4 * r + 1], acc[n][4 * r + 2],
                                      acc[n][4 * r + 3]);
              if constexpr (DROP == 2) {
                const uint32_t w = n == 0 ? mq[r].x : n == 1 ? mq[r].y : n == 2 ? mq[r].z : mq[r].w;
                const uint32_t m = w >> scol;
                o.x = keep_scaled(o.x, m, 0, q.scale); o.y = keep_scaled(o.y, m, 1, q.scale);
                o.z = keep_scaled(o.z, m, 2, q.scale); o.w = keep_scaled(o.w, m, 3, q.scale);
              }
#ifdef PTGNN_GLOBAL_STORES
              *reinterpret_cast<float4 *>(yr + n * 32) = o;
#else
              store_row4(msg_rsrc, srow * ldb + (scol + n * 32) * 4, 8 * r * ldb, o);
#endif
              __builtin_amdgcn_sched_barrier(0);
            }
          }
#pragma unroll
          for (int n = 0; n < NB; ++n) acc[n] = zero16();
        }
        if (nxt >= count) break;
        cur = nxt; nxt = n2;
        c0 = n0; c1 = n1;
        if constexpr (DROP == 1) mc = mn;
      }
    }
    u = seg_end;
  }
}

std::atomic<int> g_mode{-1};

bool debug_on() {
  static int v = -1;
  if (v < 0) v = getenv("PTGNN_AMD_DEBUG") ? 1 : 0;
  return v == 1;
}

template <typename Kern>
bool set_lds(Kern kern, size_t bytes) {
  const char *why = "";
  if (raise_dynamic_lds(kern, bytes, &why)) return true;
  if (debug_on()) fprintf(stderr, "[ptgnn_amd] stream kernel: %zu B of LDS refused (%s) -> tile kernel\n", bytes, why);
  return false;
}

void dense_runs(int nrb, int ncs, int &rps, int &run_len, int max_wg = 0) {
  if (max_wg <= 0) max_wg = num_compute_units();
  rps = max_wg / ncs;
  if (rps < 1) rps = 1;
  if (rps >= kNumXcd && (rps / kNumXcd * kNumXcd) * ncs * 10 >= max_wg * 9) rps = rps / kNumXcd * kNumXcd;
  if (rps > nrb) rps = nrb;
  run_len = (nrb + rps - 1) / rps;
  rps = (nrb + run_len - 1) / run_len;
}

}

int stream_gemm_mode() {
  int mode = g_mode.load(std::memory_order_relaxed);
  if (mode < 0) {
    const char *e = getenv("PTGNN_AMD_GEMM");
    const int m = e ? atoi(e) : 1;
    mode = (m == 0 || m == 1) ? m : 1;
    g_mode.store(mode, std::memory_order_relaxed);
  }
  return mode;
}

void stream_gemm_set_mode(int mode) { g_mode.store(mode, std::memory_order_relaxed); }

#define PTGNN_STREAM_DISPATCH_NB(NBV, KERN, ...)     \
  switch (NBV) {                                      \
    case 1: KERN(1, __VA_ARGS__); break;              \
    case 2: KERN(2, __VA_ARGS__); break;              \
    case 3: KERN(3, __VA_ARGS__); break;              \
    default: KERN(4, __VA_ARGS__); break;             \
  }

int stream_linear(const float *x, int64_t rows, int32_t k, int64_t ld_x, const float *w, int32_t n_out,
                  const float *bias, int act, float *y, int64_t ld_y, hipStream_t st, const float *addend,
                  int64_t ld_add) {
  const int mode = stream_gemm_mode();
  if (mode == 0) return 0;
  if (addend && (ld_y % 4 != 0 || !aligned16(y) || ld_add % 4 != 0 || !aligned16(addend))) return 0;
  if (k % 64 != 0 || n_out % 32 != 0 || ld_x % 4 != 0 || !aligned16(x) || !aligned16(w)) return 0;
  if (rows >= ((int64_t)1 << 31) * 32) return 0;
  int bn = n_out >= 128 ? 128 : n_out;
  {
    const bool fits128 = Slab::bytes(k, 128) + kEpiBytes <= (size_t)kLdsBudget;
    const bool fits64 = Slab::bytes(k, 64) + kEpiBytes <= (size_t)kLdsBudget;
    const char *bn_env = getenv("PTGNN_AMD_LINEAR_BN");
    const int want = bn_env ? atoi(bn_env) : 0;
    const char *ring_force = getenv("PTGNN_AMD_LINEAR_RING");
    const bool ring_forced = ring_force && ring_force[0] == '1';
    if (!ring_forced && n_out % 128 == 0 && n_out <= 256 && fits64 && (want == 64 || (want != 128 && !fits128))) bn = 64;
  }
  const int nb = bn / 32;
  const char *ring_env = getenv("PTGNN_AMD_LINEAR_RING");
  const bool force_ring = ring_env && ring_env[0] == '1', no_ring = ring_env && ring_env[0] == '0';
  const char *force = getenv("PTGNN_AMD_FORCE_STREAM");
  const bool forced = force && force[0] == '1';
  const bool ring_shape = n_out % 128 == 0 && (int64_t)n_out * k < ((int64_t)1 << 30) && (rows >= 32 * 64 || forced);
  const bool ring = ring_shape && (force_ring || (!no_ring && Slab::bytes(k, bn) + kEpiBytes > (size_t)kLdsBudget));
  if (!ring) {
    const int64_t units = (rows + 31) / 32 * ((n_out + bn - 1) / bn);
    if (!forced && (units < (int64_t)num_compute_units() * 8 * 3 || (n_out + bn - 1) / bn > 4)) return 0;
  }
  const size_t slab = Slab::bytes(k, bn);
  const size_t lds = slab + 16 + 8 * kTqFloats * sizeof(float);
  LinearArgs p;
  p.x = x; p.rows = rows; p.K = k; p.ld_x = ld_x; p.w = w; p.n_out = n_out; p.bias = bias; p.act = act;
  p.y = y; p.ld_y = ld_y; p.addend = addend; p.ld_add = ld_add;
  p.nrb = (int)((rows + 31) / 32);
  p.ncs = (n_out + bn - 1) / bn;
  p.vec_store = (ld_y % 4 == 0 && aligned16(y)) ? 1 : 0;
  if (ring) {
    const size_t rlds = (size_t)(2 * kLinRingPanelFloats + kRingWaves * kTqFloats) * sizeof(float);
    dense_runs(p.nrb, p.ncs, p.rps, p.run_len, 2 * num_compute_units());
    p.lds_floats = 0;
    auto kern = k_stream_linear_ring;
    if (!set_lds(kern, rlds)) return 0;
    kern<<<(unsigned)(p.ncs * p.rps), kRingWaves * 64, rlds, st>>>(p);
    count_launch(PTGNN_AMD_KERNEL_STREAM_LINEAR_RING);
    return 1;
  }
  if (lds > (size_t)kLdsBudget) return 0;
  dense_runs(p.nrb, p.ncs, p.rps, p.run_len);
  p.lds_floats = (int)(slab / 4);
  const unsigned grid = (unsigned)(p.ncs * p.rps);
#define PTGNN_K(NBV, UNUSED)                                                        \
  do {                                                                              \
    auto kern = k_stream_linear<NBV>;                                               \
    if (!set_lds(kern, lds)) return 0;                                              \
    kern<<<grid, 512, lds, st>>>(p);                                                \
  } while (0)
  PTGNN_STREAM_DISPATCH_NB(nb, PTGNN_K, 0);
#undef PTGNN_K
  count_launch(PTGNN_AMD_KERNEL_STREAM_LINEAR);
  return 1;
}

int stream_gru(const float *a, int64_t ld_a, const float *h, int64_t ld_h, const float *w_ih,
               const float *w_hh, const float *b_ih, const float *b_hh, int64_t n, int32_t m, int32_t hd,
               float *out, int64_t ld_out, float *gates, hipStream_t st) {
  const int mode = stream_gemm_mode();
  if (mode == 0) return 0;
  if (m % 64 != 0 || hd % 64 != 0 || ld_a % 4 != 0 || ld_h % 4 != 0 || ld_out % 4 != 0 || !aligned16(a) ||
      !aligned16(h) || !aligned16(out) || (gates && !aligned16(gates)) || !aligned16(w_ih) || !aligned16(w_hh))
    return 0;
  if (n >= ((int64_t)1 << 31) * 32) return 0;
  const int K = m + hd;
  const size_t slab = Slab::bytes(K, 96);
  const size_t lds = slab + 16 + 8 * kTqFloats * sizeof(float);
  GruArgs p;
  p.a = a; p.ld_a = ld_a; p.h = h; p.ld_h = ld_h; p.w_ih = w_ih; p.w_hh = w_hh; p.b_ih = b_ih; p.b_hh = b_hh;
  p.n = n; p.M = m; p.H = hd; p.out = out; p.ld_out = ld_out; p.gates = gates;
  p.nrb = (int)((n + 31) / 32);
  p.ncs = hd / 32;
  p.split = 0;
  const char *ring_env = getenv("PTGNN_AMD_GRU_RING");
  const bool force_ring = ring_env && ring_env[0] == '1';
  if ((lds > (size_t)kLdsBudget && !(ring_env && ring_env[0] == '0')) || force_ring) {
    const size_t rlds = (size_t)(2 * kRingPanelFloats + kRingWaves * kTqFloats) * sizeof(float);
    dense_runs(p.nrb, p.ncs, p.rps, p.run_len, 2 * num_compute_units());
    p.lds_floats = 0;
    auto kern = k_stream_gru_ring;
    if (!set_lds(kern, rlds)) return 0;
    kern<<<(unsigned)(p.ncs * p.rps), kRingWaves * 64, rlds, st>>>(p);
    count_launch(PTGNN_AMD_KERNEL_STREAM_GRU_RING);
    return 1;
  }
  if (lds > (size_t)kLdsBudget) return 0;
  dense_runs(p.nrb, p.ncs, p.rps, p.run_len);
  p.lds_floats = (int)(slab / 4);
  p.split = (kSplitGru && !gates && lds + kGruSplitBytes <= (size_t)kLdsBudget) ? 1 : 0;
  const size_t lds_launch = p.split ? lds + kGruSplitBytes : lds;
  const unsigned grid = (unsigned)(p.ncs * p.rps);
  {
    auto kern = k_stream_gru;
    if (!set_lds(kern, lds_launch)) return 0;
    kern<<<grid, 512, lds_launch, st>>>(p);
  }
  count_launch(PTGNN_AMD_KERNEL_STREAM_GRU);
  return 1;
}

static bool edge_v2_shape(int32_t state_dim, int32_t msg_dim, int use_dst, int act) {
  if (stream_gemm_mode() != 1 || act != PTGNN_AMD_ACT_NONE || use_dst) return false;
  const int K = state_dim;
  if (!(K == 64 || K == 128 || K == 256)) return false;
  if (!(msg_dim == 64 || msg_dim == 128)) return false;
  return Slab::bytes(K, msg_dim) + kEpiBytes <= (size_t)kLdsBudget;
}

template <int DROP>
static int edge_v2_launch(const EdgeV2Args &q, int K, int msg_dim, unsigned grid, size_t lds, hipStream_t st) {
#define PTGNN_K(NBV, NCHV)                                            \
  do {                                                                \
    auto kern = k_stream_edge_v2<NBV, NCHV, DROP, 0>;                 \
    if (!set_lds(kern, lds)) return 0;                                \
    kern<<<grid, 512, lds, st>>>(q);                                  \
    count_launch(PTGNN_AMD_KERNEL_STREAM_EDGE_V2);                    \
    return 1;                                                         \
  } while (0)
  if (msg_dim == 128) {
    if (K == 64) PTGNN_K(4, 2);
    if (K == 128) PTGNN_K(4, 4);
    if (K == 256) PTGNN_K(4, 8);
  } else {
    if (K == 64) PTGNN_K(2, 2);
    if (K == 128) PTGNN_K(2, 4);
    if (K == 256) PTGNN_K(2, 8);
  }
#undef PTGNN_K
  return 0;
}

constexpr size_t kEdgeEpiBytes = 16 + (size_t)kEdgeWaves * kTqFloats * sizeof(float);

static int edge_plan(int32_t state_dim, int32_t msg_dim, int use_dst, size_t *slab_bytes) {
  const int mode = stream_gemm_mode();
  if (mode == 0) return 0;
  const int K = use_dst ? 2 * state_dim : state_dim;
  if (K % 64 != 0 || state_dim % 32 != 0 || msg_dim % 32 != 0 || msg_dim > 128) return 0;
  if (Slab::bytes(K, msg_dim) + kEdgeEpiBytes <= (size_t)kLdsBudget) {
    *slab_bytes = Slab::bytes(K, msg_dim);
    return 1;
  }
  return 0;
}

int stream_edge_supported(int32_t state_dim, int32_t msg_dim, int use_dst) {
  size_t b;
  return edge_plan(state_dim, msg_dim, use_dst, &b) != 0;
}

int stream_edge_masked_supported(int32_t state_dim, int32_t msg_dim) {
  return edge_v2_shape(state_dim, msg_dim, 0, PTGNN_AMD_ACT_NONE) ? 1 : 0;
}

int stream_edge(const StreamEdgeTable &tab, const float *x, int64_t ld_x, int64_t num_rows, int32_t state_dim,
                int use_dst, int32_t msg_dim, int act, float *msg, int64_t ld_msg, int64_t msg_row_base,
                hipStream_t st, const StreamEdgeMask *mask) {
  size_t slab = 0;
  const int kind = edge_plan(state_dim, msg_dim, use_dst, &slab);
  const bool v2 = edge_v2_shape(state_dim, msg_dim, use_dst, act);
  if (mask && mask->mode != 0 && !v2) return 0;
  if (kind == 0) return 0;
  const int nb = msg_dim / 32;
  const size_t lds = slab + 16 + kEdgeWaves * kTqFloats * sizeof(float);
  const int total = tab.unit_off[tab.num_types];
  if (total == 0) return 1;
  EdgeArgs p;
  p.tab = tab; p.tab_dev = nullptr; p.x = x; p.ld_x = ld_x; p.H = state_dim; p.use_dst = use_dst; p.M = msg_dim; p.act = act;
  p.msg = msg; p.ld_msg = ld_msg; p.msg_row_base = msg_row_base; p.num_rows = num_rows;
  int budget = num_compute_units();
  if (budget > total / 8 + 1) budget = total / 8 + 1;
  int w[kStreamMaxTypes], sum = 0, nonempty = 0;
  for (int t = 0; t < tab.num_types; ++t) {
    const int64_t u_t = tab.unit_off[t + 1] - tab.unit_off[t];
    w[t] = u_t == 0 ? 0 : (int)(u_t * budget / total);
    if (u_t > 0 && w[t] == 0) w[t] = 1;
    sum += w[t];
    nonempty += u_t > 0;
  }
  if (budget < nonempty) budget = nonempty;
  while (sum != budget) {
    int best = -1;
    double best_v = 0.0;
    for (int t = 0; t < tab.num_types; ++t) {
      const double u_t = (double)(tab.unit_off[t + 1] - tab.unit_off[t]);
      if (u_t == 0) continue;
      if (sum < budget) {
        const double v = u_t / w[t];
        if (best < 0 || v > best_v) { best = t; best_v = v; }
      } else if (w[t] > 1) {
        const double v = u_t / (w[t] - 1);
        if (best < 0 || v < best_v) { best = t; best_v = v; }
      }
    }
    if (best < 0) break;
    w[best] += sum < budget ? 1 : -1;
    sum += sum < budget ? 1 : -1;
  }
  p.tab.wg_off[0] = 0;
  for (int t = 0; t < tab.num_types; ++t) p.tab.wg_off[t + 1] = p.tab.wg_off[t] + w[t];
  for (int t = tab.num_types + 1; t <= kStreamMaxTypes; ++t) {
    p.tab.wg_off[t] = p.tab.wg_off[tab.num_types];
    p.tab.unit_off[t] = p.tab.unit_off[tab.num_types];
  }
  p.run_len = 0;
  p.lds_floats = (int)(slab / 4);
  const unsigned grid = (unsigned)p.tab.wg_off[tab.num_types];
  if (mask && mask->mode != 0) {
    EdgeV2Args q;
    q.e = p;
    q.mask = mask->bits; q.mask_ld = mask->ld; q.mask_col0 = mask->col0; q.scale = mask->scale;
    return mask->mode == 1 ? edge_v2_launch<1>(q, state_dim, msg_dim, grid, lds, st)
                           : edge_v2_launch<2>(q, state_dim, msg_dim, grid, lds, st);
  }
#define PTGNN_K(NBV, UNUSED)                                  \
  do {                                                        \
    auto kern = k_stream_edge<NBV, false>;                    \
    if (!set_lds(kern, lds)) return 0;                        \
    kern<<<grid, kEdgeWaves * 64, lds, st>>>(p);              \
  } while (0)
  PTGNN_STREAM_DISPATCH_NB(nb, PTGNN_K, 0);
#undef PTGNN_K
  count_launch(PTGNN_AMD_KERNEL_STREAM_EDGE);
  return 1;
}

int stream_edge_indirect(const StreamEdgeTable *tab_dev, const float *const *w_per_type, int num_types, const float *x,
                         int64_t ld_x, int64_t num_rows, int32_t state_dim, int32_t msg_dim, int act, float *msg,
                         int64_t ld_msg, hipStream_t st) {
  if (num_types > kStreamMaxTypes) return 0;
  size_t slab = 0;
  const int kind = edge_plan(state_dim, msg_dim, 0, &slab);
  if (kind == 0) return 0;
  const int nb = msg_dim / 32;
  const size_t lds = slab + 16 + kEdgeWaves * kTqFloats * sizeof(float);
  EdgeArgs p;
  p.tab.num_types = num_types;
  for (int t = 0; t < num_types; ++t) p.tab.w[t] = w_per_type[t];
  p.tab_dev = tab_dev;
  p.x = x; p.ld_x = ld_x; p.H = state_dim; p.use_dst = 0; p.M = msg_dim; p.act = act;
  p.msg = msg; p.ld_msg = ld_msg; p.msg_row_base = 0; p.num_rows = num_rows;
  p.run_len = 0;
  p.lds_floats = (int)(slab / 4);
  const unsigned grid = (unsigned)edge_table_budget();
#define PTGNN_K(NBV, UNUSED)                                  \
  do {                                                        \
    auto kern = k_stream_edge<NBV, true>;                     \
// ... 28 lines not shown
```

### ptgnn_amd/gnn.py

```python
from typing import Any, Dict, List, NamedTuple, Optional, Tuple

import torch
from torch import nn

from ptgnn_amd import ops
from ptgnn_amd.layers import AbstractMessagePassingLayer, ConcatResidualLayer, forward_scope, set_output_hint

try:
    from ptgnn.neuralmodels.gnn.structs import GnnOutput
except Exception:
    class GnnOutput(NamedTuple):
        input_node_representations: torch.Tensor
        output_node_representations: torch.Tensor
        node_to_graph_idx: torch.Tensor
        node_idx_references: Dict[str, torch.Tensor]
        node_graph_idx_reference: Dict[str, torch.Tensor]
        num_graphs: int

        @property
        def reference_nodes_idx(self) -> Dict[str, torch.Tensor]:
            return self.node_idx_references

        @property
        def reference_nodes_graph_idx(self) -> Dict[str, torch.Tensor]:
            return self.node_graph_idx_reference

try:
    from ptgnn.baseneuralmodel import ModuleWithMetrics
except Exception:
    class ModuleWithMetrics(nn.Module):

        def __init__(self):
            super().__init__()
            self._reset_module_metrics()

        def _reset_module_metrics(self) -> None:
            pass

        def _module_metrics(self) -> Dict[str, Any]:
            return {}

        def report_metrics(self) -> Dict[str, Any]:
            out: Dict[str, Any] = {}
            for m in self.modules():
                if isinstance(m, ModuleWithMetrics):
                    out.update(m._module_metrics())
            return out

        def reset_metrics(self) -> None:
            for m in self.modules():
                if isinstance(m, ModuleWithMetrics):
                    m._reset_module_metrics()

        def train(self, mode: bool = True):
            self.reset_metrics()
            return super().train(mode)


class GraphNeuralNetwork(ModuleWithMetrics):

    def __init__(self, message_passing_layers: List[AbstractMessagePassingLayer],
                 node_embedder: nn.Module, introduce_backwards_edges: bool, add_self_edges: bool,
                 edge_dropout_rate: float = 0.0, edge_feature_embedder: Optional[nn.Module] = None):
        super().__init__()
        self.__message_passing_layers = nn.ModuleList(message_passing_layers)
        self.__node_embedder = node_embedder
        self.__introduce_backwards_edges = introduce_backwards_edges
        self.__add_self_edges = add_self_edges
        assert 0 <= edge_dropout_rate < 1
        self.__edge_dropout_rate = edge_dropout_rate
        self.__edge_feature_embedder = edge_feature_embedder
        self._idents: Optional[torch.Tensor] = None

    @property
    def input_node_state_dim(self) -> int:
        return self.__message_passing_layers[0].input_state_dimension

    @property
    def output_node_state_dim(self) -> int:
        return self.__message_passing_layers[-1].output_state_dimension

    @property
    def message_passing_layers(self):
        return self.__message_passing_layers

    def _reset_module_metrics(self) -> None:
        self.__num_graphs, self.__num_edges, self.__num_nodes = 0, 0, 0

    def _module_metrics(self) -> Dict[str, Any]:
        if torch.cuda.is_available():
            from ptgnn_amd import ops
            ops.check_indices(sync=True)
        return {"num_graphs": int(self.__num_graphs), "num_nodes": int(self.__num_nodes),
                "num_edges": int(self.__num_edges)}

    def _identity_edges(self, num_nodes: int, device) -> torch.Tensor:
        ids = self._idents
        if ids is None or ids.shape[0] != num_nodes or ids.device != device:
            ids = torch.arange(num_nodes, dtype=torch.int64, device=device)
            self._idents = ids
        return ids

    def gnn(self, node_representations: torch.Tensor,
            adjacency_lists: List[Tuple[torch.Tensor, torch.Tensor]],
            edge_feature_embeddings: List[torch.Tensor], node_to_graph_idx: torch.Tensor,
            reference_node_ids: Dict[str, torch.Tensor],
            reference_node_graph_idx: Dict[str, torch.Tensor],
            return_all_states: bool = False) -> torch.Tensor:
        if self.__edge_dropout_rate > 0 and self.training:
            kept_adj, kept_feats = [], []
            for (src, dst), feats in zip(adjacency_lists, edge_feature_embeddings):
                mask = torch.rand_like(src, dtype=torch.float32) > self.__edge_dropout_rate
                kept_adj.append((src.masked_select(mask), dst.masked_select(mask)))
                kept_feats.append(feats[mask])
            adjacency_lists, edge_feature_embeddings = kept_adj, kept_feats

        if node_representations.is_cuda:
            ops.plan_for(adjacency_lists, node_representations.shape[0])
        all_states = [node_representations]
        with forward_scope():
            layers = list(self.__message_passing_layers)
            for li, mp_layer in enumerate(layers):
                buf = None
                nxt = layers[li + 1] if li + 1 < len(layers) else None
                if (isinstance(nxt, ConcatResidualLayer) and node_representations.is_cuda and not return_all_states
                        and node_representations.dtype == torch.float32
                        and not (torch.is_grad_enabled() and (node_representations.requires_grad or self.training))):
                    out_dim = mp_layer.output_state_dimension
                    buf = nxt.make_result_buffer(node_representations.shape[0], out_dim, node_representations)
                    set_output_hint(buf[:, buf.shape[1] - out_dim:])
                try:
                    node_representations = mp_layer(
                        node_states=node_representations, adjacency_lists=adjacency_lists,
                        node_to_graph_idx=node_to_graph_idx, reference_node_ids=reference_node_ids,
                        reference_node_graph_idx=reference_node_graph_idx,
                        edge_features=edge_feature_embeddings)
                finally:
                    set_output_hint(None)
                if buf is not None and node_representations.data_ptr() == buf[:, buf.shape[1] - out_dim:].data_ptr():
                    node_representations._ptgnn_amd_concat_buffer = buf
                all_states.append(node_representations)
        if return_all_states:
            node_representations = torch.cat(all_states, dim=-1)
        return node_representations

    def forward(self, *, node_data, adjacency_lists: List[Tuple[torch.Tensor, torch.Tensor]],
                edge_feature_data: List, node_to_graph_idx: torch.Tensor,
                reference_node_ids: Dict[str, torch.Tensor],
                reference_node_graph_idx: Dict[str, torch.Tensor], num_graphs, **kwargs) -> GnnOutput:
        initial = self.__node_embedder(**node_data)
        device = node_to_graph_idx.device
        if self.__edge_feature_embedder is None:
            feats = [torch.empty(f.shape[0], 0, device=device) for f, _ in adjacency_lists]
        else:
            feats = [self.__edge_feature_embedder(**e) for e in edge_feature_data]

        adj = list(adjacency_lists)
        if self.__introduce_backwards_edges:
            adj += [(t, f) for f, t in adj]
            feats += [e for e in feats]
        if self.__add_self_edges:
            num_nodes = node_to_graph_idx.shape[0]
            idents = self._identity_edges(num_nodes, device)
            adj.append((idents, idents))
            feats.append(torch.zeros(num_nodes, feats[-1].shape[-1], device=device))

        output = self.gnn(initial, adj, feats, node_to_graph_idx, reference_node_ids,
                          reference_node_graph_idx, **kwargs)
        with torch.no_grad():
            self.__num_edges += sum(a[0].shape[0] for a in adj)
            self.__num_graphs += num_graphs
            self.__num_nodes += node_to_graph_idx.shape[0]
        return GnnOutput(input_node_representations=initial, output_node_representations=output,
                         node_to_graph_idx=node_to_graph_idx, node_idx_references=reference_node_ids,
                         node_graph_idx_reference=reference_node_graph_idx, num_graphs=num_graphs)
```

### ptgnn_amd/layers.py

```python
import contextlib
import os
import threading
import weakref
from typing import Dict, List, Optional, Tuple, Union

import torch
from torch import nn

from ptgnn_amd import _lib, dense, ops, precision, torch_route
from ptgnn_amd.scatter import (block_attention as block_attention_autograd, edge_linear as edge_linear_autograd,
                               edge_linear_feat as edge_linear_feat_autograd,
                               gather_reduce as gather_reduce_autograd, graph_norm as graph_norm_autograd,
                               pna_aggregate as pna_aggregate_autograd, scatter_mean, segment_reduce)

try:
    from ptgnn.neuralmodels.gnn.messagepassing.abstractmessagepassing import (
        AbstractMessageAggregation, AbstractMessagePassingLayer)
except Exception:
    class AbstractMessagePassingLayer(nn.Module):

        def forward(self, node_states, adjacency_lists, node_to_graph_idx, reference_node_ids,
                    reference_node_graph_idx, edge_features) -> torch.Tensor:
            raise NotImplementedError

        def _aggregate_messages(self, messages, message_targets, num_nodes, aggregation_fn: str):
            from ptgnn_amd.scatter import scatter
            msg_dtype = messages.dtype
            return scatter(messages.to(torch.float32), index=message_targets, dim=0,
                           dim_size=num_nodes, reduce=aggregation_fn).to(msg_dtype)

        @property
        def input_state_dimension(self) -> int:
            raise NotImplementedError

        @property
        def output_state_dimension(self) -> int:
            raise NotImplementedError

    class AbstractMessageAggregation(nn.Module):
        def forward(self, messages, message_targets, num_nodes):
            raise NotImplementedError

        def output_state_size(self, message_input_size: int) -> int:
            raise NotImplementedError

Adj = List[Tuple[torch.Tensor, torch.Tensor]]


_SCOPE = threading.local()


@contextlib.contextmanager
def forward_scope():
    outer = getattr(_SCOPE, "cache", None)
    if outer is None:
        _SCOPE.cache = {}
        from ptgnn_amd import dense
        dense.clear_transposed_cache()
    try:
        yield
    finally:
        _SCOPE.cache = outer


def _scoped(owner, name, make):
    cache = getattr(_SCOPE, "cache", None)
    if cache is None or not torch.is_grad_enabled():
        return make()
    key = (owner, name)
    val = cache.get(key)
    if val is None:
        val = cache[key] = make()
    return val


def set_output_hint(buf: Optional[torch.Tensor]) -> None:
    _SCOPE.out_hint = buf


def _take_output_hint(rows: int, cols: int, like: torch.Tensor, vector_stores: bool = False) -> Optional[torch.Tensor]:
    hint = getattr(_SCOPE, "out_hint", None)
    _SCOPE.out_hint = None
    if hint is None or torch.is_grad_enabled() and like.requires_grad:
        return None
    if tuple(hint.shape) != (rows, cols) or hint.dtype != torch.float32 or hint.device != like.device:
        return None
    if vector_stores and (hint.data_ptr() % 16 != 0 or (rows > 1 and hint.stride(0) % 4 != 0) or hint.stride(1) != 1):
        return None
    return hint


def _no_grad_needed(*tensors) -> bool:
    if not torch.is_grad_enabled():
        return True
    return not any(t is not None and t.requires_grad for t in tensors)


EDGE_PATH_BIAS = 1.25
UNIQUE_MESSAGES = os.environ.get("PTGNN_AMD_UNIQUE_MESSAGES", "1") not in ("", "0")


def _prefer_edge_path(num_edges: int, num_nodes: int, num_types: int, state_dim: int, msg_dim: int) -> bool:
    if state_dim % 32 != 0 or msg_dim % 4 != 0 or num_types < 2:
        return False
    return num_edges * EDGE_PATH_BIAS < num_nodes * num_types


def _has_edge_features(feature_dim: int, edge_features) -> bool:
    return feature_dim != 0 or any(f is not None and f.shape[-1] != 0 for f in edge_features)


def _stack_detached(weights) -> torch.Tensor:
    return weights[0].detach() if len(weights) == 1 else torch.cat([w.detach() for w in weights], dim=0)


def _kernel_act(act: Optional[nn.Module]) -> Optional[str]:
    return "tanh" if isinstance(act, nn.Tanh) else ("relu" if isinstance(act, nn.ReLU) else None)


def _edge_messages(table: torch.Tensor, adjacency_lists, plan, weights, inputs=None, rounded=None):
    if UNIQUE_MESSAGES and ops.edge_linear_shared_supported(table.shape[1], weights[0].shape[0], len(weights)):
        uniq = plan.unique_messages()
        if uniq is not None:
            return ops.edge_linear_shared(table, uniq, weights, inputs=inputs, rounded=rounded), uniq.slot_row
    return ops.edge_linear(table, adjacency_lists, weights, False, inputs=inputs, rounded=rounded), plan.perm


def _feat_gemm_ok(node_states, edge_features, state_dim: int, out_dim: int, *params, shapes_only: bool = False) -> bool:
    if node_states.dtype != torch.float32 or state_dim % 32 != 0 or out_dim % 4 != 0:
        return False
    if any(f is None or f.shape[-1] == 0 or f.device != node_states.device or f.dtype != torch.float32
           for f in edge_features):
        return False
    if len({int(f.shape[-1]) for f in edge_features}) != 1:
        return False
    if shapes_only:
        return True
    return (not torch.is_grad_enabled()) or _no_grad_needed(node_states, *edge_features, *params)


def _edge_training_ok(state_dim: int, msg_dim: int) -> bool:
    return state_dim % 32 == 0 and msg_dim % 32 == 0


def _dropout_seed() -> int:
    return int(torch.randint(0, 2 ** 62, (1,), dtype=torch.int64).item())


def _train_edge_messages(owner, x, plan, weights, use_dst: bool, p: float = 0.0, seed_xor: int = 0, key: str = "edge_w"):
    w_stack = _scoped(owner, key, lambda: torch.stack(weights))
    return edge_linear_autograd(x, plan, w_stack, use_dst, p, (_dropout_seed() ^ seed_xor) if p > 0 else 0)


_AMP_DTYPES = (torch.float16, torch.bfloat16)


def _half_weights(owner, name: str, dtype, kind: int, k_or_m: int, n_out_or_hd: int, make):
    if dtype == torch.float32 or not ops.half_supported(kind, k_or_m, n_out_or_hd, dtype):
        return None
    return _scoped(owner, (name, dtype), make)


def _amp_forward(layer, node_states, adjacency_lists, edge_features, cast_features: bool = True) -> torch.Tensor:
    if cast_features:
        edge_features = [f.float() if f is not None and f.dtype in _AMP_DTYPES else f for f in edge_features]
    return layer.forward(node_states.float(), adjacency_lists, None, None, None, edge_features).to(node_states.dtype)


def _overlap_reduces():
    from ptgnn_amd import sharded
    return sharded.OVERLAP_REDUCES


def _run_mlp(mlp: "MLP", x: torch.Tensor) -> torch.Tensor:
    for m in mlp.modules_in_order:
        x = dense.linear(x, m.weight, m.bias) if isinstance(m, nn.Linear) else m(x)
    return x


def _first_linear_gemm_ok(mlps, training: bool, state_dim: int, differentiable: bool) -> bool:
    first = [m.linears[0] for m in mlps]
    if any(l.bias is not None for l in first):
        return False
    if training and any(isinstance(m, nn.Dropout) and m.p > 0 for e in mlps for m in e.modules_in_order):
        return False
    if not differentiable:
        return True
    return len({tuple(l.weight.shape) for l in first}) == 1 and _edge_training_ok(state_dim, first[0].weight.shape[0])


def _edge_mlp_tail(mlps, adjacency_lists, hid: torch.Tensor, differentiable: bool, single_block_as_is: bool = False):
    messages = None
    if not differentiable:
        messages = torch.empty(hid.shape[0], mlps[0].linears[-1].out_features, dtype=torch.float32, device=hid.device)
    outs, off = [], 0
    for (src, _), edge_mlp in zip(adjacency_lists, mlps):
        n = int(src.shape[0])
        mods = edge_mlp.modules_in_order
        rest = mods[next(i for i, m in enumerate(mods) if isinstance(m, nn.Linear)) + 1:]
        h = hid[off:off + n]
        last = max((i for i, m in enumerate(rest) if isinstance(m, nn.Linear)), default=-1)
        for i, m in enumerate(rest):
            if not isinstance(m, nn.Linear):
                h = m(h)
            elif differentiable:
                h = dense.linear(h, m.weight, m.bias)
            else:
                h = ops.linear(h, m.weight, m.bias, out=messages[off:off + n] if i == last and n > 0 else None)
        if differentiable:
            outs.append(h)
        elif last < 0 and n > 0:
            messages[off:off + n].copy_(h)
        off += n
    if not differentiable:
        return messages
    return outs[0] if single_block_as_is and len(outs) == 1 else torch.cat(outs, dim=0)


def _shard_source_table(shard, node_states: torch.Tensor, w: torch.Tensor) -> torch.Tensor:
    if w.shape[0] <= w.shape[1]:
        y = shard.new_table(w.shape[0], node_states)
        ops.linear(node_states, w, out=y[: shard.n_local])
        shard.exchange_into(y)
        return y
    return ops.linear(shard.exchange(node_states), w)


def _shard_source_table_autograd(shard, node_states: torch.Tensor, w: torch.Tensor) -> torch.Tensor:
    if w.shape[0] <= w.shape[1]:
        return shard.exchange_autograd(dense.linear(node_states, w))
    return dense.linear(shard.exchange_autograd(node_states), w)


def _shard_two_blocks(shard, node_states: torch.Tensor, w: Optional[torch.Tensor], edge_messages=None):
    n, H = shard.n_local, node_states.shape[1]
    if edge_messages is not None or w.shape[0] > H:
        table = shard.new_table(H, node_states)
        table[:n].copy_(node_states)
        work = shard.begin_exchange(table)
        if edge_messages is not None:
            def table_of(block):
                adj, plan = (shard.adj_own, shard.plan_own) if block == "own" else (shard.adj_halo, shard.plan_halo)
# ... 40 lines not shown
    return ops.plan_for([(index, index)], int(num_samples))


class MLP(nn.Module):
    def __init__(self, input_dimension: int, output_dimension: int,
                 hidden_layers: Union[List[int], int] = 1, use_biases: bool = False,
                 activation: Optional[nn.Module] = nn.ReLU(), dropout_rate: float = 0.0):
        super().__init__()
        if isinstance(hidden_layers, int):
            width = 32 if output_dimension == 1 else output_dimension
            sizes = [width] * hidden_layers
        else:
            sizes = list(hidden_layers)
        if len(sizes) > 1:
            assert activation is not None, "Multiple linear layers without an activation"
        mods: List[nn.Module] = []
        d = input_dimension
        for h in sizes:
            lin = nn.Linear(d, h, bias=use_biases)
            nn.init.xavier_uniform_(lin.weight)
            mods += [nn.Dropout(p=dropout_rate), lin] + ([activation] if activation is not None else [])
            d = h
        out = nn.Linear(d, output_dimension, bias=use_biases)
        nn.init.xavier_uniform_(out.weight)
        mods += [nn.Dropout(p=dropout_rate), out]
        self.__mlp_modules = nn.Sequential(*mods)

    @property
    def linears(self) -> List[nn.Linear]:
        return [m for m in self.__mlp_modules if isinstance(m, nn.Linear)]

    @property
    def modules_in_order(self) -> List[nn.Module]:
        return list(self.__mlp_modules)

    @property
    def is_single_linear(self) -> bool:
        ls = self.linears
        return len(ls) == 1 and ls[0].bias is None

    def forward(self, x: torch.Tensor) -> torch.Tensor:
        return self.__mlp_modules(x)


class GatedMessagePassingLayer(AbstractMessagePassingLayer):

    def __init__(self, state_dimension: int, message_dimension: int, num_edge_types: int,
                 message_aggregation_function: str, dropout_rate: float = 0.0,
                 edge_feature_dimension: int = 0):
        super().__init__()
        self.__edge_message_transformation_layers = nn.ModuleList(
            [nn.Linear(state_dimension + edge_feature_dimension, message_dimension, bias=False)
             for _ in range(num_edge_types)])
        for lin in self.__edge_message_transformation_layers:
            nn.init.xavier_normal_(lin.weight, gain=(1 / num_edge_types) ** 0.5)
        self.__state_update = nn.GRUCell(input_size=message_dimension, hidden_size=state_dimension)
        nn.init.orthogonal_(self.__state_update.weight_hh)
        nn.init.xavier_uniform_(self.__state_update.weight_ih)
        nn.init.normal_(self.__state_update.bias_hh, std=1e-5)
        nn.init.normal_(self.__state_update.bias_ih, std=1e-5)
        self.__state_dimension = state_dimension
        self.__aggregation_fn = message_aggregation_function
        self.__dropout = nn.Dropout(p=dropout_rate)
        self._message_dimension = message_dimension
        self._edge_feature_dimension = edge_feature_dimension

    def _stacked_edge_weights(self) -> torch.Tensor:
        return _stack_detached([lin.weight for lin in self.__edge_message_transformation_layers])

    def _table_ok(self, node_states, edge_features) -> bool:
        if _has_edge_features(self._edge_feature_dimension, edge_features):
            return False
        if self.training and self.__dropout.p > 0:
            return False
        if self.__aggregation_fn not in ops.REDUCE_IDS:
            return False
        return node_states.dtype == torch.float32

    def _fused_ok(self, node_states, edge_features) -> bool:
        if not self._table_ok(node_states, edge_features):
            return False
        return (not torch.is_grad_enabled()) or _no_grad_needed(node_states, *self.parameters())

    def forward(self, node_states: torch.Tensor, adjacency_lists: Adj, node_to_graph_idx,
                reference_node_ids: Dict[str, torch.Tensor],
                reference_node_graph_idx: Dict[str, torch.Tensor],
                edge_features: List[torch.Tensor]) -> torch.Tensor:
        assert len(adjacency_lists) == len(self.__edge_message_transformation_layers)
        if _on_host(node_states):
            return torch_route.ggnn_layer(node_states, adjacency_lists, edge_features,
                                          list(self.__edge_message_transformation_layers), self.__dropout,
                                          self.__state_update, self.__aggregation_fn,
                                          inputs=self._host_matrix_inputs(node_states, edge_features))
        if node_states.dtype in _AMP_DTYPES:
            return _amp_forward(self, node_states, adjacency_lists, edge_features)
        num_nodes, H, M = node_states.shape[0], self.__state_dimension, self._message_dimension
        plan = ops.plan_for(adjacency_lists, num_nodes)
        if self._fused_ok(node_states, edge_features):
            return self._forward_fused(node_states, adjacency_lists, plan)

        agg_fn = self.__aggregation_fn
        has_feats = _has_edge_features(self._edge_feature_dimension, edge_features)
        p = self.__dropout.p if self.training else 0.0
        ws = [l.weight for l in self.__edge_message_transformation_layers]
        train_inputs = precision.training_inputs(node_states)
        if (not has_feats and node_states.dtype == torch.float32 and _edge_training_ok(H, M)
                and (p > 0 or _prefer_edge_path(plan.num_edges, num_nodes, len(ws), H, M))):
            agg = segment_reduce(_train_edge_messages(self, node_states, plan, ws, False, p), plan, agg_fn)
        elif self._table_ok(node_states, edge_features):
            agg = gather_reduce_autograd(dense.linear(node_states, torch.cat(ws, dim=0), inputs=train_inputs), None, plan,
                                         M, agg_fn)
        elif (has_feats and p == 0.0 and agg_fn in ops.REDUCE_IDS
                and _feat_gemm_ok(node_states, edge_features, H, M, *self.parameters())):
            return self._forward_features_inference(node_states, adjacency_lists, plan, edge_features)
        elif (has_feats and p == 0.0 and agg_fn in ops.REDUCE_IDS and _edge_training_ok(H, M)
                and _feat_gemm_ok(node_states, edge_features, H, M, shapes_only=True)):
            agg = segment_reduce(edge_linear_feat_autograd(node_states, plan, ws, False, edge_features), plan, agg_fn)
        else:
            agg = segment_reduce(self._general_messages(node_states, adjacency_lists, edge_features), plan, agg_fn)
        return dense.gru_cell(self.__state_update, agg, node_states, inputs=train_inputs)

    def _host_matrix_inputs(self, node_states, edge_features):
        if node_states.dtype != torch.float32 or (self.training and self.__dropout.p > 0):
            return torch.float32
        if torch.is_grad_enabled() and not _no_grad_needed(node_states, *self.parameters(),
                                                           *[f for f in edge_features if f is not None]):
            return torch.float32
        return precision.resolve(node_states)

    def _rounded_gru_weights(self, dtype):
        gru = self.__state_update
        return _half_weights(self, "gru_w16", dtype, ops.HALF_KIND_GRU, self._message_dimension, self.__state_dimension,
                             lambda: (gru.weight_ih.detach().to(dtype).contiguous(),
                                      gru.weight_hh.detach().to(dtype).contiguous()))

    def _forward_fused(self, node_states, adjacency_lists, plan) -> torch.Tensor:
        num_nodes, H, M = node_states.shape[0], self.__state_dimension, self._message_dimension
        gru = self.__state_update
        inputs = precision.resolve(node_states)
        if _prefer_edge_path(plan.num_edges, num_nodes, len(adjacency_lists), H, M):
            weights = [l.weight for l in self.__edge_message_transformation_layers]
            edge_inputs = precision.edge_gemm_inputs(node_states)
            w16 = None
            if edge_inputs != torch.float32 and ops.edge_linear16_supported(H, M, len(weights), edge_inputs):
                w16 = _scoped(self, ("edge_stack16", edge_inputs),
                              lambda: torch.stack([w.detach() for w in weights]).to(edge_inputs))
            msgs, col = _edge_messages(node_states, adjacency_lists, plan, weights, inputs=edge_inputs, rounded=w16)
            tb = 0
        else:
            w = self._stacked_edge_weights()
            w16 = _half_weights(self, "edge_w16", inputs, ops.HALF_KIND_LINEAR, H, w.shape[0],
                                lambda: w.to(inputs).contiguous())
            msgs, col, tb = ops.linear(node_states, w, inputs=inputs, rounded=w16), None, None
        return ops.aggregate_gru(msgs, plan, M, self.__aggregation_fn, node_states, gru.weight_ih, gru.weight_hh,
                                 gru.bias_ih, gru.bias_hh, type_bits=tb, col=col,
                                 out=_take_output_hint(num_nodes, H, node_states), inputs=inputs,
                                 rounded=self._rounded_gru_weights(inputs))

    def _forward_features_inference(self, node_states, adjacency_lists, plan, edge_features) -> torch.Tensor:
        gru = self.__state_update
        inputs = precision.resolve(node_states)
        msgs = ops.edge_linear(node_states, adjacency_lists,
                               [l.weight for l in self.__edge_message_transformation_layers], False,
                               edge_feats=edge_features)
        agg = ops.gather_reduce(msgs, plan, self._message_dimension, self.__aggregation_fn, type_bits=0, col=plan.perm)
        return ops.gru_cell(agg, node_states, gru.weight_ih, gru.weight_hh, gru.bias_ih, gru.bias_hh, inputs=inputs,
                            rounded=self._rounded_gru_weights(inputs))

    def _general_messages(self, node_states, adjacency_lists, edge_features) -> torch.Tensor:
        all_messages = []
        for (src, _), feats, lin in zip(adjacency_lists, edge_features,
                                        self.__edge_message_transformation_layers):
            inp = node_states.index_select(0, src)
            if feats is not None and feats.shape[-1] > 0:
                inp = torch.cat([inp, feats.to(inp.dtype)], dim=-1)
            all_messages.append(dense.linear(self.__dropout(inp), lin.weight))
        return torch.cat(all_messages, dim=0)

    def forward_sharded(self, node_states: torch.Tensor, shard) -> torch.Tensor:
        _check_device(node_states)
        feats = [None] * len(shard.local_adj)
        T = len(shard.local_adj)
        assert T == len(self.__edge_message_transformation_layers)
        if self._edge_feature_dimension != 0 or node_states.dtype != torch.float32:
            raise _lib.PtgnnAmdError("forward_sharded: edge features / non-fp32 states are not supported on a "
                                     "sharded graph")
        agg_fn = self.__aggregation_fn
        if agg_fn not in ops.REDUCE_IDS:
            raise _lib.PtgnnAmdError(f"forward_sharded: aggregation {agg_fn!r} is not supported on a "
                                     "sharded graph (sum / mean / max / min are)")
        M, H = self._message_dimension, self.__state_dimension
        gru = self.__state_update
        p = self.__dropout.p if self.training else 0.0
        ws = [l.weight for l in self.__edge_message_transformation_layers]
        edge_form = _prefer_edge_path(*shard.form_sizes(T * M > H), T, H, M)
        if not self._fused_ok(node_states, feats):
            if _edge_training_ok(H, M) and (p > 0 or edge_form):
                msgs = _train_edge_messages(self, shard.exchange_autograd(node_states), shard.plan, ws, False, p,
                                            seed_xor=0x9E3779B97F4A7C15 * (shard.rank + 1) & (2 ** 62 - 1))
                agg = segment_reduce(msgs, shard.plan, agg_fn)
            elif p > 0:
                raise _lib.PtgnnAmdError("forward_sharded: per-edge dropout needs state and message widths that "
                                         "are multiples of 32")
            else:
                y = _shard_source_table_autograd(shard, node_states, torch.cat(ws, dim=0))
                agg = gather_reduce_autograd(y, None, shard.plan, M, agg_fn)
            return dense.gru_cell(gru, agg, node_states)

        def edge_messages(table, adj, plan):
            return _edge_messages(table, adj, plan, ws)
        if shard.overlap and agg_fn in _overlap_reduces():
            from ptgnn_amd import sharded
            work, table_of = _shard_two_blocks(shard, node_states, None if edge_form else self._stacked_edge_weights(),
                                               edge_messages if edge_form else None)
            agg = sharded.aggregate_two_blocks(shard, work, table_of, M, agg_fn)
        elif edge_form:
            msgs, col = edge_messages(shard.exchange(node_states), shard.local_adj, shard.plan)
            agg = ops.gather_reduce(msgs, shard.plan, M, agg_fn, type_bits=0, col=col)
        else:
            y = _shard_source_table(shard, node_states, self._stacked_edge_weights())
            agg = ops.gather_reduce(y, shard.plan, M, agg_fn)
        return ops.gru_cell(agg, node_states, gru.weight_ih, gru.weight_hh, gru.bias_ih, gru.bias_hh)

    @property
    def input_state_dimension(self) -> int:
        return self.__state_dimension

    @property
    def output_state_dimension(self) -> int:
        return self.__state_dimension

    def export_weights(self) -> Dict:
        gru = self.__state_update
        return {"kind": "ggnn",
                "edge_w": [l.weight.detach().cpu() for l in self.__edge_message_transformation_layers],
                "w_ih": gru.weight_ih.detach().cpu(), "w_hh": gru.weight_hh.detach().cpu(),
                "b_ih": gru.bias_ih.detach().cpu(), "b_hh": gru.bias_hh.detach().cpu(),
                "agg": self.__aggregation_fn}


class EGCMessagePassingLayer(AbstractMessagePassingLayer):

    def __init__(self, input_state_dimension: int, output_state_dimension: int, num_edge_types: int,
                 message_aggregation_function: str, num_bases: int = 4, num_heads: int = 8,
                 dropout_rate: float = 0.0):
        super().__init__()
        self.__input_state_dim = input_state_dimension
        assert output_state_dimension % num_heads == 0
        self.__aggregation_fn = message_aggregation_function
        self.__num_bases = num_bases
        self.__num_heads = num_heads
        self.__output_state_dim = output_state_dimension
        self.__dropout = nn.Dropout(p=dropout_rate)
        self.__bases = nn.ModuleList(
            [nn.Linear(input_state_dimension, num_bases * output_state_dimension, bias=False)
             for _ in range(num_edge_types)])
        self.__weight_coeffs = nn.Linear(input_state_dimension, num_heads * num_bases)

    def forward(self, node_states: torch.Tensor, adjacency_lists: Adj, node_to_graph_idx,
                reference_node_ids: Dict[str, torch.Tensor],
                reference_node_graph_idx: Dict[str, torch.Tensor],
                edge_features: List[torch.Tensor]) -> torch.Tensor:
        assert len(adjacency_lists) == len(self.__bases)
        K, B, D = self.__num_heads, self.__num_bases, self.__output_state_dim
        if _on_host(node_states):
            return torch_route.egc_layer(node_states, adjacency_lists, edge_features, list(self.__bases),
                                         self.__weight_coeffs, self.__dropout, K, B, D, self.__aggregation_fn)
        if node_states.dtype in _AMP_DTYPES:
            return _amp_forward(self, node_states, adjacency_lists, edge_features, cast_features=False)
        if node_states.dtype != torch.float32:
            raise _lib.PtgnnAmdError(f"EGCMessagePassingLayer: node states must be float32 / float16 / bfloat16 on the "
                                     f"GPU (got {node_states.dtype})")
        N, H, T = node_states.shape[0], self.__input_state_dim, len(adjacency_lists)
        Dh, M = D // K, B * D
        agg_fn = self.__aggregation_fn
        plan = ops.plan_for(adjacency_lists, N)
        wc = self.__weight_coeffs
        weights = [l.weight for l in self.__bases]
        p = self.__dropout.p if self.training else 0.0
        reduce_ok = agg_fn in ops.REDUCE_IDS
        edge_form = _prefer_edge_path(plan.num_edges, N, T, H, M)

        if reduce_ok and p == 0.0 and _no_grad_needed(node_states, *self.parameters()):
            coef = ops.linear(node_states, wc.weight, wc.bias)
            if edge_form:
                msgs = ops.edge_linear(node_states, adjacency_lists, weights, False)
                return ops.gather_combine(msgs, plan, K, B, Dh, agg_fn, coef, type_bits=0, col=plan.perm)
            return ops.gather_combine(ops.linear(node_states, _stack_detached(weights)), plan, K, B, Dh, agg_fn,
                                      coef)

        coef = dense.linear(node_states, wc.weight, wc.bias)
        if reduce_ok and _edge_training_ok(H, M) and (p > 0 or edge_form):
            agg = segment_reduce(_train_edge_messages(self, node_states, plan, weights, False, p), plan, agg_fn)
        elif reduce_ok and p == 0.0:
            y = dense.linear(node_states, weights[0] if T == 1 else torch.cat(weights, dim=0))
            agg = gather_reduce_autograd(y, None, plan, M, agg_fn)
        else:
            msgs = [dense.linear(self.__dropout(node_states.index_select(0, src)), lin.weight)
                    for (src, _), lin in zip(adjacency_lists, self.__bases)]
            agg = segment_reduce(torch.cat(msgs, dim=0), plan, agg_fn)
        return dense.basis_combine(agg, coef, K, B, Dh)

    def forward_sharded(self, node_states: torch.Tensor, shard) -> torch.Tensor:
        raise _lib.PtgnnAmdError("EGCMessagePassingLayer is not supported under dst-range sharding "
                                 "(ptgnn_amd.sharded); run it unsharded")

    @property
    def input_state_dimension(self) -> int:
        return self.__input_state_dim

# ... 409 lines not shown

        if type(self.__aggregation_fn) is PnaMessageAggregation:
            out = self._forward_pna(node_states, adjacency_lists, edge_features)
            if out is not None:
                return out
        if self._fused_ok(node_states, edge_features):
            return self._forward_fused(node_states, adjacency_lists)
        if self._table_ok(node_states, edge_features):
            return self._forward_training(node_states, adjacency_lists)

        mlps = list(self.__edge_message_transformation_layers)
        H, hidden = self.__input_state_dim, mlps[0].linears[0].weight.shape[0]
        string_agg = isinstance(self.__aggregation_fn, str)
        if (_has_edge_features(0, edge_features) and string_agg
                and _first_linear_gemm_ok(mlps, self.training, H, differentiable=False)
                and _feat_gemm_ok(node_states, edge_features, H, hidden, *self.parameters())):
            return self._forward_features_inference(node_states, adjacency_lists, edge_features, mlps)
        has_feats = _has_edge_features(self._features_dimension, edge_features)
        gemm_ok = string_agg and _first_linear_gemm_ok(mlps, self.training, H, differentiable=True)
        if gemm_ok and has_feats and _feat_gemm_ok(node_states, edge_features, H, hidden, shapes_only=True):
            return self._forward_features_training(node_states, adjacency_lists, edge_features, mlps)
        if gemm_ok and not has_feats and node_states.dtype == torch.float32:
            return self._forward_deep_mlps(node_states, adjacency_lists, mlps)
        return self._forward_general(node_states, adjacency_lists, edge_features)

    def _forward_fused(self, node_states, adjacency_lists) -> torch.Tensor:
        N, T = node_states.shape[0], len(adjacency_lists)
        plan = ops.plan_for(adjacency_lists, N)
        if _prefer_edge_path(plan.num_edges, N, T, self.__input_state_dim, self._message_dimension):
            msgs = self._edge_form_messages(node_states, adjacency_lists)
            return self._aggregate_and_update(msgs, None, plan, col=plan.perm, type_bits=0)
        ysrc, ydst = self._table_halves(self._message_table(node_states), T)
        return self._aggregate_and_update(ysrc, ydst, plan)

    def _message_table(self, node_states) -> torch.Tensor:
        w = self._stacked_edge_weights()
        inputs = precision.mlp_inputs(node_states)
        w16 = _half_weights(self, "mlp_table_w16", inputs, ops.HALF_KIND_LINEAR, self.__input_state_dim, w.shape[0],
                            lambda: w.to(inputs).contiguous())
        return ops.linear(node_states, w, inputs=inputs, rounded=w16)

    def _edge_form_messages(self, node_states, adjacency_lists) -> torch.Tensor:
        ws = self._first_weights()
        use_dst = self.__use_target_state_as_message_input
        H, M, T = self.__input_state_dim, self._message_dimension, len(ws)
        inputs = precision.mlp_inputs(node_states)
        w16 = None
        if inputs != torch.float32 and (ops.edge_linear16_dst_supported if use_dst
                                        else ops.edge_linear16_supported)(H, M, T, inputs):
            w16 = _scoped(self, ("mlp_edge_stack16", inputs), lambda: torch.stack([w.detach() for w in ws]).to(inputs))
        return ops.edge_linear(node_states, adjacency_lists, ws, use_dst, inputs=inputs, rounded=w16)

    def _host_matrix_inputs(self, node_states, edge_features):
        if node_states.dtype != torch.float32 or _has_edge_features(self._features_dimension, edge_features):
            return torch.float32
        if not all(m.is_single_linear for m in self.__edge_message_transformation_layers):
            return torch.float32
        agg = self.__aggregation_fn
        if not (agg in ops.REDUCE_IDS if isinstance(agg, str) else type(agg) is PnaMessageAggregation):
            return torch.float32
        if torch.is_grad_enabled() and not _no_grad_needed(node_states, *self.parameters()):
            return torch.float32
        return precision.mlp_inputs(node_states)

    def _forward_training(self, node_states, adjacency_lists) -> torch.Tensor:
        N, T, M, H = node_states.shape[0], len(adjacency_lists), self._message_dimension, self.__input_state_dim
        plan = ops.plan_for(adjacency_lists, N)
        if _edge_training_ok(H, M) and _prefer_edge_path(plan.num_edges, N, T, H, M):
            msgs = _train_edge_messages(self, node_states, plan, self._first_weights(),
                                        self.__use_target_state_as_message_input)
            return self._aggregate_edge_messages(msgs, plan, False)
        ysrc, ydst = self._table_halves(dense.linear(node_states, self._stacked_edge_weights(detach=False)), T)
        return self._update(gather_reduce_autograd(ysrc, ydst, plan, M, self.__aggregation_fn), False)

    def _forward_features_inference(self, node_states, adjacency_lists, edge_features, mlps) -> torch.Tensor:
        plan = ops.plan_for(adjacency_lists, node_states.shape[0])
        messages = ops.edge_linear(node_states, adjacency_lists, self._first_weights(),
                                   self.__use_target_state_as_message_input, edge_feats=edge_features)
        if not all(m.is_single_linear for m in mlps):
            messages = _edge_mlp_tail(mlps, adjacency_lists, messages, differentiable=True)
        return self._aggregate_edge_messages(messages, plan, True)

    def _forward_features_training(self, node_states, adjacency_lists, edge_features, mlps) -> torch.Tensor:
        plan = ops.plan_for(adjacency_lists, node_states.shape[0])
        hid = edge_linear_feat_autograd(node_states, plan, self._first_weights(),
                                        self.__use_target_state_as_message_input, edge_features)
        messages = _edge_mlp_tail(mlps, adjacency_lists, hid, differentiable=True, single_block_as_is=True)
        return self._aggregate_edge_messages(messages, plan, False)

    def _forward_deep_mlps(self, node_states, adjacency_lists, mlps) -> torch.Tensor:
        plan = ops.plan_for(adjacency_lists, node_states.shape[0])
        grad = not _no_grad_needed(node_states, *self.parameters())
        use_dst = self.__use_target_state_as_message_input
        if grad:
            hid = _train_edge_messages(self, node_states, plan, self._first_weights(), use_dst, key="edge_w0")
        else:
            hid = ops.edge_linear(node_states, adjacency_lists, self._first_weights(), use_dst)
        messages = _edge_mlp_tail(mlps, adjacency_lists, hid, differentiable=grad)
        return self._aggregate_edge_messages(messages, plan, not grad)

    def _forward_general(self, node_states, adjacency_lists, edge_features) -> torch.Tensor:
        all_targets, all_messages = [], []
        for (src, dst), feats, edge_mlp in zip(adjacency_lists, edge_features,
                                               self.__edge_message_transformation_layers):
            all_targets.append(dst)
            inp = node_states.index_select(0, src)
            if self.__use_target_state_as_message_input:
                inp = torch.cat([inp, node_states.index_select(0, dst)], dim=-1)
            if feats is not None and feats.shape[-1] > 0:
                inp = torch.cat([inp, feats.to(inp.dtype)], dim=-1)
            all_messages.append(_run_mlp(edge_mlp, inp))
        messages = torch.cat(all_messages, dim=0)
        if isinstance(self.__aggregation_fn, str):
            plan = ops.plan_for(adjacency_lists, node_states.shape[0])
            return self._aggregate_edge_messages(messages, plan, False)
        agg = self.__aggregation_fn(messages=messages, message_targets=torch.cat(all_targets, dim=0),
                                    num_nodes=node_states.shape[0])
        return self._update(agg, False)

    @property
    def input_state_dimension(self) -> int:
        return self.__input_state_dim

    @property
    def output_state_dimension(self) -> int:
        return self.__output_state_dim

    def export_weights(self) -> Dict:
        c = lambda t: None if t is None else t.detach().cpu()
        return {"kind": "mlp",
                "edge_mlp": [[l.weight.detach().cpu() for l in m.linears]
                             for m in self.__edge_message_transformation_layers],
                "use_target": self.__use_target_state_as_message_input, "agg": self.__aggregation_fn,
                "gelu": self.__message_activation is not None,
                "ln_w": c(self._ln.weight) if self._ln is not None else None,
                "ln_b": c(self._ln.bias) if self._ln is not None else None,
                "dense_w": c(self._dense.weight) if self._dense is not None else None,
                "dense_b": c(self._dense.bias) if self._dense is not None else None,
                "tanh": self._dense_act is not None}


class _ResidualOriginLayer(AbstractMessagePassingLayer):
    def __init__(self, input_dim: int, target_layer):
        super().__init__()
        self.__target_layer = target_layer
        self.__input_dim = input_dim

    def forward(self, node_states, adjacency_lists, node_to_graph_idx, reference_node_ids,
                reference_node_graph_idx, edge_features):
        self.__target_layer._original_input = node_states
        return node_states

    @property
    def input_state_dimension(self) -> int:
        return self.__input_dim

    @property
    def output_state_dimension(self) -> int:
        return self.__input_dim


class _ResidualBase(AbstractMessagePassingLayer):
    def __init__(self, input_dim: int):
        super().__init__()
        self._original_input = None
        self._input_dim = input_dim

    def pass_through_dummy_layer(self) -> _ResidualOriginLayer:
        return _ResidualOriginLayer(self._input_dim, target_layer=self)

    def _pop(self) -> torch.Tensor:
        assert self._original_input is not None, "Initial Pass Through Layer was not used."
        x, self._original_input = self._original_input, None
        return x

    @property
    def input_state_dimension(self) -> int:
        return self._input_dim


class MeanResidualLayer(_ResidualBase):
    def forward(self, node_states, adjacency_lists, node_to_graph_idx, reference_node_ids,
                reference_node_graph_idx, edge_features):
        return (self._pop() + node_states) * 0.5

    @property
    def output_state_dimension(self) -> int:
        return self._input_dim


class ConcatResidualLayer(_ResidualBase):
    def forward(self, node_states, adjacency_lists, node_to_graph_idx, reference_node_ids,
                reference_node_graph_idx, edge_features):
        orig = self._pop()
        buf = getattr(node_states, "_ptgnn_amd_concat_buffer", None)
        if (buf is not None and buf.shape[1] == orig.shape[1] + node_states.shape[1] and buf.dtype == orig.dtype
                and node_states.data_ptr() == buf[:, orig.shape[1]:].data_ptr()):
            buf[:, : orig.shape[1]].copy_(orig)
            return buf
        return torch.cat((orig, node_states), dim=-1)

    def make_result_buffer(self, num_nodes: int, next_dim: int, like: torch.Tensor) -> torch.Tensor:
        return torch.empty(num_nodes, self._input_dim + next_dim, dtype=like.dtype, device=like.device)

    @property
    def output_state_dimension(self) -> int:
        return 2 * self._input_dim


class LinearResidualLayer(_ResidualBase):
    def __init__(self, state_dimension1: int, state_dimension2: int, target_state_size: int,
                 dropout_rate: float = 0.0):
        super().__init__(state_dimension1)
        self.__input_dim2 = state_dimension2
        self.__linear_combination = nn.Linear(state_dimension1 + state_dimension2, target_state_size,
                                              bias=False)
        self.__dropout = nn.Dropout(p=dropout_rate)

    def forward(self, node_states, adjacency_lists, node_to_graph_idx, reference_node_ids,
                reference_node_graph_idx, edge_features):
        x = torch.cat((self._pop(), node_states), dim=-1)
        lin = self.__linear_combination
        if _on_host(x):
            return self.__dropout(lin(x))
        if x.dtype in _AMP_DTYPES:
            return self.__dropout(dense.linear(x.float(), lin.weight).to(x.dtype))
        if _no_grad_needed(x, lin.weight):
            return self.__dropout(ops.linear(x, lin.weight))
        return self.__dropout(dense.linear(x, lin.weight))

    @property
    def input_state_dimension(self) -> int:
        return self.__input_dim2

    @property
    def output_state_dimension(self) -> int:
        return self.__linear_combination.out_features
```

### ptgnn_amd/ops.py

```python
import ctypes
import os
import weakref
from typing import List, Optional, Sequence, Tuple

import torch

from ptgnn_amd import _lib
from ptgnn_amd._readback import LOCK, Backoff, Readback, take_arrived

REDUCE_IDS = {"sum": 0, "add": 0, "mean": 1, "max": 2, "min": 3}
EPI_NONE, EPI_GELU, EPI_LAYERNORM, EPI_GELU_LAYERNORM = 0, 1, 2, 3
ACT_IDS = {None: 0, "none": 0, "tanh": 1, "relu": 2}


GEMM_MODES = {"tile": 0, "stream": 1}


def set_gemm_mode(mode) -> int:
    lib = _lib.load()
    prev = lib.ptgnn_amd_get_gemm_mode()
    if isinstance(mode, str) and mode not in GEMM_MODES:
        raise _lib.PtgnnAmdError(f"unknown GEMM mode {mode!r} (have {sorted(GEMM_MODES)}; the split mode was removed)")
    _lib.check(lib.ptgnn_amd_set_gemm_mode(int(GEMM_MODES.get(mode, mode))), "ptgnn_amd_set_gemm_mode")
    return prev


def get_gemm_mode() -> int:
    return _lib.load().ptgnn_amd_get_gemm_mode()


_AGG_FAMILY_FIRST = 64


_CHAR_FAMILY_FIRST = 128


_HEAD_FAMILY_FIRST = 192


_SEQ_FAMILY_FIRST = 256


_DECODE_FAMILY_FIRST = 320


_BEAM_FAMILY_FIRST = 384


_HALF_FAMILY_FIRST = 448


_EDGE16_FAMILY_FIRST = 512


_HALF_TRAIN_FAMILY_FIRST = 576


_EDGE16_DST_FAMILY_FIRST = 640


def launch_counts(aggregation: bool = False, char_cnn: bool = False, heads: bool = False,
                  sequence: bool = False, decode: bool = False, beam: bool = False, half: bool = False,
                  edge16: bool = False, half_training: bool = False, edge16_dst: bool = False) -> dict:
    lib = _lib.load()
    out = {}
    for first in (0,) + ((_AGG_FAMILY_FIRST,) if aggregation else ()) + ((_CHAR_FAMILY_FIRST,) if char_cnn else ()) \
            + ((_HEAD_FAMILY_FIRST,) if heads else ()) + ((_SEQ_FAMILY_FIRST,) if sequence else ()) \
            + ((_DECODE_FAMILY_FIRST,) if decode else ()) + ((_BEAM_FAMILY_FIRST,) if beam else ()) \
            + ((_HALF_FAMILY_FIRST,) if half else ()) + ((_EDGE16_FAMILY_FIRST,) if edge16 else ()) \
            + ((_HALF_TRAIN_FAMILY_FIRST,) if half_training else ()) \
            + ((_EDGE16_DST_FAMILY_FIRST,) if edge16_dst else ()):
        i = first
        while True:
            name = lib.ptgnn_amd_launch_name(i)
            if name is None:
                break
            out[name.decode()] = int(lib.ptgnn_amd_launch_count(i))
            i += 1
    return out


def launches_since(before: dict) -> dict:
    now = launch_counts(aggregation=True, char_cnn=True, heads=True, sequence=True, decode=True, beam=True, half=True,
                        edge16=True, half_training=True, edge16_dst=True)
    return {k: now[k] - v for k, v in before.items() if now[k] != v}


def _stream(t: torch.Tensor) -> int:
    return torch.cuda.current_stream(t.device).cuda_stream


class KernelTimer:

    def __init__(self):
        self.records = []

    def summary(self):
        torch.cuda.synchronize()
        out = {}
        for name, s, e, work in self.records:
            d = out.setdefault(name, {"calls": 0, "ms": 0.0, "bytes": 0.0, "flops": 0.0})
            d["calls"] += 1
            d["ms"] += s.elapsed_time(e)
            b, f = work.get("bytes", 0.0), work.get("flops", 0.0)
            d["bytes"] += b() if callable(b) else b
            d["flops"] += f() if callable(f) else f
        return out


_TIMER: Optional[KernelTimer] = None


def set_kernel_timer(timer: Optional[KernelTimer]):
    global _TIMER
    _TIMER = timer


class _timed:
    __slots__ = ("name", "work", "s")

    def __init__(self, name, **work):
        self.name, self.work = name, work

    def __enter__(self):
        if _TIMER is not None:
            self.s = torch.cuda.Event(enable_timing=True)
            self.s.record()
        return self

    def __exit__(self, *exc):
        if _TIMER is not None:
            e = torch.cuda.Event(enable_timing=True)
            e.record()
            _TIMER.records.append((self.name, self.s, e, self.work))
        return False


def _require_cuda_f32(name: str, t: torch.Tensor, dims: int = 2):
    if not t.is_cuda:
        raise _lib.PtgnnAmdError(
            f"{name} must live on the GPU: the C-ABI wrappers have no CPU path (got device {t.device}; CPU tensors are served "
            "one level up, by the layers' and the facade's plain-torch route)")
    if t.dtype != torch.float32:
        raise _lib.PtgnnAmdError(f"{name} must be float32 (got {t.dtype})")
    if t.dim() != dims:
        raise _lib.PtgnnAmdError(f"{name} must be {dims}-D (got shape {tuple(t.shape)})")


def _rowmajor(t: torch.Tensor) -> torch.Tensor:
    if t.stride(1) == 1 and t.stride(0) >= t.shape[1]:
        return t
    if t.shape[1] == 1 and t.stride(0) >= 1:
        return t
    return t.contiguous()


def _ptr_or(t: torch.Tensor, stand_in: torch.Tensor) -> int:
    return t.data_ptr() if t.numel() else stand_in.data_ptr()


def _ld(t: torch.Tensor) -> int:
    return t.stride(0) if t.shape[0] > 1 else max(t.stride(0), t.shape[1])


def _rows_arg(t: torch.Tensor, d: int):
    return (t.data_ptr(), _ld(t)) if t.numel() else (None, d)


def _workspace(nbytes: int, device) -> torch.Tensor:
    return torch.empty(max(nbytes, 1), dtype=torch.uint8, device=device)


class _DeviceState:
    __slots__ = ("device", "bad_ids", "bad_readback", "uniq_backoff", "uniq_pending", "hub_backoff", "hub_pending",
                 "side_stream", "plan_control")

    def __init__(self, index: int):
        self.device = torch.device("cuda", index)
        self.bad_ids = self.bad_readback = self.side_stream = None
        self.uniq_backoff, self.uniq_pending = Backoff(), []
        self.hub_backoff, self.hub_pending = Backoff(), []
        self.plan_control = {}


_STATES = {}


def _device_state(device) -> _DeviceState:
    key = torch.device(device).index or 0
    st = _STATES.get(key)
    if st is None:
        with LOCK:
            st = _STATES.setdefault(key, _DeviceState(key))
    return st


class GraphPlan:

    __slots__ = ("rowptr", "col", "perm", "type_bits", "num_nodes", "num_edges", "num_types",
                 "num_src_rows", "_backward", "_adj", "_adj_refs", "_inv_perm", "_ready", "_waited",
                 "_hub_tickets", "hub_entries", "hub_count", "_slot_rows", "_ident", "_transposed", "_uniq", "_hub_posted",
                 "_has_hubs", "_hdrs", "__weakref__")

    def __init__(self, rowptr, col, perm, type_bits, num_nodes, num_edges, num_types):
        self.rowptr, self.col, self.perm = rowptr, col, perm
        self.type_bits, self.num_nodes = type_bits, num_nodes
        self.num_edges, self.num_types = num_edges, num_types
        self.num_src_rows = num_nodes
        self._backward = None
        self._adj = None
        self._adj_refs = None
        self._inv_perm = None
        self._ready = None
        self._waited = set()
        self._hub_tickets = {}
        self.hub_entries = self.hub_count = None
        self._slot_rows = self._ident = self._transposed = None
        self._uniq = None
        self._hub_posted = False
        self._has_hubs = None
        self._hdrs = {}

    def may_have_hubs(self) -> bool:
        return self.hub_entries is not None

    def hub_tickets(self, msg_dim: int) -> torch.Tensor:
        n = _lib.load().ptgnn_amd_hub_ticket_count(self.num_edges, msg_dim)
        dev = self.rowptr.device
        key = (n, torch.cuda.current_stream(dev).cuda_stream)
        t = self._hub_tickets.get(key)
        if t is None:
            t = torch.zeros(max(n, 1), dtype=torch.int32, device=dev)
            self._hub_tickets[key] = t
        return t

    def wait(self) -> None:
        if self._ready is not None:
            cur = torch.cuda.current_stream(self.rowptr.device)
# ... 1142 lines not shown
            gm_ptr, _ld(grad_msg) if E > 0 else M, T, M, float(dropout_p),
            int(dropout_seed) & 0xFFFFFFFFFFFFFFFF, grad_w.data_ptr(), ws.data_ptr(), ws_bytes, _stream(grad_w))
    _lib.check(rc, "ptgnn_amd_edge_weight_grad_f32")
    return grad_w


def linear_weight_grad(x: torch.Tensor, grad_y: torch.Tensor, want_bias: bool = False):
    lib = _lib.load()
    _require_cuda_f32("x", x)
    _require_cuda_f32("grad_y", grad_y)
    x, grad_y = _rowmajor(x), _rowmajor(grad_y)
    rows, k = x.shape
    n_out = grad_y.shape[1]
    if grad_y.shape[0] != rows:
        raise _lib.PtgnnAmdError("linear_weight_grad: x and grad_y row counts differ")
    if rows == 0:
        gw = torch.zeros(n_out, k, dtype=torch.float32, device=x.device)
        return (gw, torch.zeros(n_out, dtype=torch.float32, device=x.device)) if want_bias else gw
    grad_w = torch.empty(n_out, k, dtype=torch.float32, device=x.device)
    grad_b = torch.empty(n_out, dtype=torch.float32, device=x.device) if want_bias else None
    ws_bytes = lib.ptgnn_amd_edge_wgrad_workspace_bytes(rows, 1, n_out, k)
    ws = torch.empty(max(ws_bytes, 1), dtype=torch.uint8, device=x.device)
    with _timed("linear_weight_grad", flops=2.0 * rows * k * n_out, bytes=4.0 * (rows * k + rows * n_out + n_out * k)):
        rc = lib.ptgnn_amd_linear_weight_grad_f32(x.data_ptr(), _ld(x), k, grad_y.data_ptr(), _ld(grad_y),
                                                  rows, n_out, grad_w.data_ptr(),
                                                  grad_b.data_ptr() if want_bias else None,
                                                  ws.data_ptr(), ws_bytes, _stream(grad_w))
    _lib.check(rc, "ptgnn_amd_linear_weight_grad_f32")
    return (grad_w, grad_b) if want_bias else grad_w


def half_wgrad_chunk_rows(rows: int, n_out: int, k: int) -> int:
    return int(_lib.load().ptgnn_amd_wgrad16_chunk_rows(int(rows), int(n_out), int(k)))


def half_linear_weight_grad(x: torch.Tensor, grad_y: torch.Tensor, dtype, want_bias: bool = False):
    lib = _lib.load()
    _require_cuda_f32("x", x)
    _require_cuda_f32("grad_y", grad_y)
    x, grad_y = _rowmajor(x), _rowmajor(grad_y)
    rows, k = x.shape
    n_out = grad_y.shape[1]
    if grad_y.shape[0] != rows:
        raise _lib.PtgnnAmdError("half_linear_weight_grad: x and grad_y row counts differ")
    half = _half_inputs(dtype)
    if half is None or not half_supported(HALF_KIND_WGRAD, k, n_out, half) or not (_half_rows_ok(x)
                                                                                   and _half_rows_ok(grad_y)):
        return linear_weight_grad(x, grad_y, want_bias=want_bias)
    if rows == 0:
        gw = torch.zeros(n_out, k, dtype=torch.float32, device=x.device)
        return (gw, torch.zeros(n_out, dtype=torch.float32, device=x.device)) if want_bias else gw
    grad_w = torch.empty(n_out, k, dtype=torch.float32, device=x.device)
    grad_b = torch.empty(n_out, dtype=torch.float32, device=x.device) if want_bias else None
    ws_bytes = lib.ptgnn_amd_wgrad16_workspace_bytes(rows, n_out, k)
    ws = torch.empty(max(ws_bytes, 1), dtype=torch.uint8, device=x.device)
    with _timed("half_linear_weight_grad", flops=2.0 * rows * k * n_out,
                bytes=4.0 * (rows * k + rows * n_out + n_out * k) + 2.0 * ws_bytes):
        rc = lib.ptgnn_amd_linear_weight_grad16(x.data_ptr(), _ld(x), k, grad_y.data_ptr(), _ld(grad_y), rows, n_out,
                                                HALF_IDS[half], grad_w.data_ptr(),
                                                grad_b.data_ptr() if want_bias else None, ws.data_ptr(), ws_bytes,
                                                _stream(grad_w))
    _lib.check(rc, "ptgnn_amd_linear_weight_grad16")
    return (grad_w, grad_b) if want_bias else grad_w


def segment_spread(grad: torch.Tensor, arg: Optional[torch.Tensor], plan: GraphPlan) -> torch.Tensor:
    lib = _lib.load()
    _require_cuda_f32("grad", grad)
    grad = _rowmajor(grad)
    E, D = plan.num_edges, grad.shape[1]
    out = torch.empty(E, D, dtype=torch.float32, device=grad.device)
    if E == 0:
        return out
    if arg is not None:
        arg = arg.contiguous()
    plan.wait()
    with _timed("segment_spread", bytes=E * (4.0 * D + 8) + plan.num_nodes * 4.0 * D * (2 if arg is not None else 1)):
        rc = lib.ptgnn_amd_segment_spread_f32(grad.data_ptr(), _ld(grad),
                                              arg.data_ptr() if arg is not None else None,
                                              plan.slot_rows().data_ptr(), plan.perm.data_ptr(), E, D,
                                              out.data_ptr(), D, _stream(out))
    _lib.check(rc, "ptgnn_amd_segment_spread_f32")
    return out


def row_epilogue(x: torch.Tensor, flags: int, ln_weight: Optional[torch.Tensor] = None,
                 ln_bias: Optional[torch.Tensor] = None, ln_eps: float = 1e-5) -> torch.Tensor:
    lib = _lib.load()
    _require_cuda_f32("x", x)
    x = _rowmajor(x)
    n, d = x.shape
    y = torch.empty(n, d, dtype=torch.float32, device=x.device)
    if flags & EPI_LAYERNORM:
        ln_weight, ln_bias = ln_weight.contiguous(), ln_bias.contiguous()
    with _timed("row_epilogue", bytes=8.0 * n * d):
        rc = lib.ptgnn_amd_row_epilogue_f32(x.data_ptr(), _ld(x), n, d, flags,
                                            ln_weight.data_ptr() if flags & EPI_LAYERNORM else None,
                                            ln_bias.data_ptr() if flags & EPI_LAYERNORM else None, float(ln_eps),
                                            y.data_ptr(), d, _stream(y))
    _lib.check(rc, "ptgnn_amd_row_epilogue_f32")
    return y


def row_epilogue_backward(x: torch.Tensor, grad_y: torch.Tensor, flags: int, ln_weight: Optional[torch.Tensor] = None,
                          ln_eps: float = 1e-5):
    lib = _lib.load()
    _require_cuda_f32("x", x)
    _require_cuda_f32("grad_y", grad_y)
    x, grad_y = _rowmajor(x), _rowmajor(grad_y)
    n, d = x.shape
    gx = torch.empty(n, d, dtype=torch.float32, device=x.device)
    ln = bool(flags & EPI_LAYERNORM)
    gg = gb = ws = None
    ws_bytes = 0
    if ln:
        ln_weight = ln_weight.contiguous()
        gg = torch.empty(d, dtype=torch.float32, device=x.device)
        gb = torch.empty(d, dtype=torch.float32, device=x.device)
        ws_bytes = int(lib.ptgnn_amd_row_epilogue_workspace_bytes(n, d))
        ws = torch.empty(max(ws_bytes, 1), dtype=torch.uint8, device=x.device)
    with _timed("row_epilogue_backward", bytes=12.0 * n * d):
        rc = lib.ptgnn_amd_row_epilogue_backward_f32(x.data_ptr(), _ld(x), grad_y.data_ptr(), _ld(grad_y), n, d, flags,
                                                     ln_weight.data_ptr() if ln else None, float(ln_eps),
                                                     gx.data_ptr(), d, gg.data_ptr() if ln else None,
                                                     gb.data_ptr() if ln else None,
                                                     ws.data_ptr() if ln else None, ws_bytes, _stream(gx))
    _lib.check(rc, "ptgnn_amd_row_epilogue_backward_f32")
    return gx, gg, gb


def act_dropout_backward(grad: torch.Tensor, y: torch.Tensor, keep: Optional[torch.Tensor], scale: float,
                         act: Optional[str], out: Optional[torch.Tensor] = None) -> torch.Tensor:
    lib = _lib.load()
    _require_cuda_f32("grad", grad)
    grad, y = grad.contiguous(), y.contiguous()
    n = grad.numel()
    if out is None:
        out = torch.empty_like(grad)
    elif not (out.is_cuda and out.dtype == torch.float32 and out.is_contiguous() and out.numel() == n):
        raise _lib.PtgnnAmdError("act_dropout_backward: out must be a contiguous float32 CUDA tensor of grad's size")
    if keep is not None:
        keep = keep.contiguous()
        if keep.dtype != torch.bool or keep.numel() != n:
            raise _lib.PtgnnAmdError("act_dropout_backward: keep must be a bool mask of grad's shape")
    with _timed("act_dropout_backward", bytes=(12.0 + (1.0 if keep is not None else 0.0)) * n):
        rc = lib.ptgnn_amd_act_dropout_backward_f32(grad.data_ptr(), y.data_ptr(),
                                                    keep.data_ptr() if keep is not None else None, float(scale),
                                                    ACT_IDS[act], n, out.data_ptr(), _stream(out))
    _lib.check(rc, "ptgnn_amd_act_dropout_backward_f32")
    return out


def gru_cell(a: torch.Tensor, h: torch.Tensor, w_ih, w_hh, b_ih, b_hh, out: Optional[torch.Tensor] = None,
             inputs=None, rounded=None) -> torch.Tensor:
    lib = _lib.load()
    _require_cuda_f32("a", a)
    _require_cuda_f32("h", h)
    a, h = _rowmajor(a), _rowmajor(h)
    n, m = a.shape
    hd = h.shape[1]
    if out is None:
        out = torch.empty(n, hd, dtype=torch.float32, device=a.device)
    elif tuple(out.shape) != (n, hd) or out.dtype != torch.float32 or out.stride(1) != 1 or not out.is_cuda:
        raise _lib.PtgnnAmdError(f"gru_cell: `out` must be a float32 CUDA [{n}, {hd}] view with unit inner stride")
    half = _half_inputs(inputs)
    if half is not None and half_supported(HALF_KIND_GRU, m, hd, half) and _half_rows_ok(a) and _half_rows_ok(h):
        given = rounded if rounded is not None else (None, None)
        wi16, wh16 = _rounded_weight(w_ih, half, given[0]), _rounded_weight(w_hh, half, given[1])
        with _timed("half_gru_cell", flops=2.0 * n * 3 * hd * (m + hd), bytes=4.0 * n * (m + 2 * hd) + 6.0 * hd * (m + hd)):
            rc = lib.ptgnn_amd_half_gru_cell(a.data_ptr(), _ld(a), h.data_ptr(), _ld(h), wi16.data_ptr(), wh16.data_ptr(),
                                             b_ih.contiguous().data_ptr(), b_hh.contiguous().data_ptr(), n, m, hd,
                                             HALF_IDS[half], out.data_ptr(), _ld(out), _stream(out))
        _lib.check(rc, "ptgnn_amd_half_gru_cell")
        return out
    with _timed("gru_cell", flops=2.0 * n * 3 * hd * (m + hd), bytes=4.0 * (n * (m + 2 * hd) + 3 * hd * (m + hd))):
        rc = lib.ptgnn_amd_gru_cell_f32(a.data_ptr(), _ld(a), h.data_ptr(), _ld(h),
                                        w_ih.contiguous().data_ptr(), w_hh.contiguous().data_ptr(),
                                        b_ih.contiguous().data_ptr(), b_hh.contiguous().data_ptr(),
                                        n, m, hd, out.data_ptr(), _ld(out), _stream(out))
    _lib.check(rc, "ptgnn_amd_gru_cell_f32")
    return out


AGG_PIPELINE = int(os.environ.get("PTGNN_AMD_AGG_PIPELINE", "1"))
AGG_PIPELINE_MIN_ROWS = int(os.environ.get("PTGNN_AMD_AGG_PIPELINE_MIN_ROWS", "65536"))


def aggregate_gru(ysrc: torch.Tensor, plan: GraphPlan, msg_dim: int, reduce: str, h: torch.Tensor, w_ih, w_hh, b_ih,
                  b_hh, type_bits: Optional[int] = None, col: Optional[torch.Tensor] = None,
                  out: Optional[torch.Tensor] = None, inputs=None, rounded=None) -> torch.Tensor:
    N = plan.num_nodes
    pieces = AGG_PIPELINE
    if (pieces < 2 or N < AGG_PIPELINE_MIN_ROWS or N < 64 * pieces or torch.cuda.is_current_stream_capturing()):
        agg = gather_reduce(ysrc, plan, msg_dim, reduce, type_bits=type_bits, col=col)
        return gru_cell(agg, h, w_ih, w_hh, b_ih, b_hh, out=out, inputs=inputs, rounded=rounded)
    dev = h.device
    hd = h.shape[1]
    agg = torch.empty(N, msg_dim, dtype=torch.float32, device=dev)
    if out is None:
        out = torch.empty(N, hd, dtype=torch.float32, device=dev)
    bounds = [min(N, (N * i // pieces + 31) // 32 * 32) for i in range(pieces)] + [N]
    main, side = torch.cuda.current_stream(dev), _side_stream(dev)
    plan.wait()
    gather_reduce(ysrc, plan, msg_dim, reduce, type_bits=type_bits, col=col, out=agg, rows=(bounds[0], bounds[1]))
    first_done = torch.cuda.Event()
    first_done.record(main)
    ready = []
    with torch.cuda.stream(side):
        side.wait_event(first_done)
        for i in range(1, pieces):
            gather_reduce(ysrc, plan, msg_dim, reduce, type_bits=type_bits, col=col, out=agg,
                          rows=(bounds[i], bounds[i + 1]))
            ev = torch.cuda.Event()
            ev.record(side)
            ready.append(ev)
    for i in range(pieces):
        if i > 0:
            main.wait_event(ready[i - 1])
        lo, hi = bounds[i], bounds[i + 1]
        if hi > lo:
            gru_cell(agg[lo:hi], h[lo:hi], w_ih, w_hh, b_ih, b_hh, out=out[lo:hi], inputs=inputs, rounded=rounded)
    return out


def gru_cell_train(a: torch.Tensor, h: torch.Tensor, w_ih, w_hh, b_ih, b_hh, inputs=None, rounded=None):
    lib = _lib.load()
    _require_cuda_f32("a", a)
    _require_cuda_f32("h", h)
    a, h = _rowmajor(a), _rowmajor(h)
    n, m = a.shape
    hd = h.shape[1]
    out = torch.empty(n, hd, dtype=torch.float32, device=a.device)
    gates = torch.empty(n, 4 * hd, dtype=torch.float32, device=a.device)
    half = _half_inputs(inputs)
    if half is not None and half_supported(HALF_KIND_GRU, m, hd, half) and _half_rows_ok(a) and _half_rows_ok(h):
        given = rounded if rounded is not None else (None, None)
        wi16, wh16 = _rounded_weight(w_ih, half, given[0]), _rounded_weight(w_hh, half, given[1])
        with _timed("half_gru_cell_train", flops=2.0 * n * 3 * hd * (m + hd),
                    bytes=4.0 * n * (m + 2 * hd + 4 * hd) + 6.0 * hd * (m + hd)):
            rc = lib.ptgnn_amd_gru_cell_train16(a.data_ptr(), _ld(a), h.data_ptr(), _ld(h), wi16.data_ptr(),
                                                wh16.data_ptr(), b_ih.contiguous().data_ptr(),
                                                b_hh.contiguous().data_ptr(), n, m, hd, HALF_IDS[half], out.data_ptr(),
                                                _ld(out), gates.data_ptr(), _stream(out))
        _lib.check(rc, "ptgnn_amd_gru_cell_train16")
        return out, gates
    with _timed("gru_cell", flops=2.0 * n * 3 * hd * (m + hd),
                bytes=4.0 * (n * (m + 2 * hd + 4 * hd) + 3 * hd * (m + hd))):
        rc = lib.ptgnn_amd_gru_cell_train_f32(a.data_ptr(), _ld(a), h.data_ptr(), _ld(h),
                                              w_ih.contiguous().data_ptr(), w_hh.contiguous().data_ptr(),
                                              b_ih.contiguous().data_ptr(), b_hh.contiguous().data_ptr(),
                                              n, m, hd, out.data_ptr(), hd, gates.data_ptr(), _stream(out))
    _lib.check(rc, "ptgnn_amd_gru_cell_train_f32")
    return out, gates


def gru_gates_backward(grad_out: torch.Tensor, gates: torch.Tensor, h: torch.Tensor):
    lib = _lib.load()
    _require_cuda_f32("grad_out", grad_out)
    _require_cuda_f32("h", h)
    grad_out, h = _rowmajor(grad_out), _rowmajor(h)
    n, hd = h.shape
    d_gi = torch.empty(n, 3 * hd, dtype=torch.float32, device=h.device)
    d_gh = torch.empty(n, 3 * hd, dtype=torch.float32, device=h.device)
    d_h = torch.empty(n, hd, dtype=torch.float32, device=h.device)
    with _timed("gru_gates_backward", bytes=4.0 * n * hd * 13):
        rc = lib.ptgnn_amd_gru_cell_backward_gates_f32(grad_out.data_ptr(), _ld(grad_out), gates.data_ptr(),
                                                       h.data_ptr(), _ld(h), n, hd, d_gi.data_ptr(),
                                                       d_gh.data_ptr(), d_h.data_ptr(), _stream(d_h))
    _lib.check(rc, "ptgnn_amd_gru_cell_backward_gates_f32")
    return d_gi, d_gh, d_h


def gather_rows(x: torch.Tensor, idx: torch.Tensor) -> torch.Tensor:
    lib = _lib.load()
    _require_cuda_f32("x", x)
    x = _rowmajor(x)
    if idx.dtype != torch.int64 or not idx.is_cuda:
        raise _lib.PtgnnAmdError("gather_rows: idx must be a CUDA int64 tensor")
    idx = idx.contiguous()
    out = torch.empty(idx.shape[0], x.shape[1], dtype=torch.float32, device=x.device)
    rc = lib.ptgnn_amd_gather_rows_f32(x.data_ptr(), _ld(x), idx.data_ptr(), idx.shape[0],
                                       x.shape[1], out.data_ptr(), x.shape[1], _stream(out))
    _lib.check(rc, "ptgnn_amd_gather_rows_f32")
    return out


def weighted_pool(x: torch.Tensor, w: torch.Tensor, plan: GraphPlan) -> torch.Tensor:
    lib = _lib.load()
    _require_cuda_f32("x", x)
    x = _rowmajor(x)
    n, d = x.shape
    if n != plan.num_edges or w.numel() != d or plan.perm is None:
        raise _lib.PtgnnAmdError(f"weighted_pool: x {tuple(x.shape)}, w {tuple(w.shape)} do not fit a plan over "
                                 f"{plan.num_edges} elements")
    w = w.detach().reshape(-1).contiguous()
    G = plan.num_nodes
    out = torch.empty(G, d, dtype=torch.float32, device=x.device)
    ws_bytes = int(lib.ptgnn_amd_weighted_pool_workspace_bytes(G, n, d))
    ws = _workspace(ws_bytes, x.device)
    plan.wait()
    with _timed("weighted_pool", bytes=4.0 * (n * d + G * d + d) + 4.0 * n):
        rc = lib.ptgnn_amd_weighted_pool_f32(*_rows_arg(x, d), w.data_ptr(),
                                             plan.rowptr.data_ptr(), plan.perm.data_ptr(), G, n, d, out.data_ptr(), d,
                                             ws.data_ptr(), ws_bytes, _stream(out))
    _lib.check(rc, "ptgnn_amd_weighted_pool_f32")
    return out


def weighted_pool_backward(x: torch.Tensor, w: torch.Tensor, index: torch.Tensor, grad_out: torch.Tensor):
    lib = _lib.load()
    _require_cuda_f32("x", x)
    _require_cuda_f32("grad_out", grad_out)
    x, grad_out = _rowmajor(x), _rowmajor(grad_out)
    n, d = x.shape
    if index.dtype != torch.int64 or not index.is_cuda or index.shape[0] != n:
        raise _lib.PtgnnAmdError("weighted_pool_backward: the map must be a CUDA int64 tensor with one entry per element")
    index = index.contiguous()
    w = w.detach().reshape(-1).contiguous()
    gx = torch.empty(n, d, dtype=torch.float32, device=x.device)
    gw = torch.empty(d, dtype=torch.float32, device=x.device)
    ws_bytes = int(lib.ptgnn_amd_weighted_pool_backward_workspace_bytes(n, d))
    ws = _workspace(ws_bytes, x.device)
    with _timed("weighted_pool_backward", bytes=4.0 * (3 * n * d) + 8.0 * n):
        rc = lib.ptgnn_amd_weighted_pool_backward_f32(*_rows_arg(x, d), w.data_ptr(),
                                                      index.data_ptr() if n else None,
                                                      *_rows_arg(grad_out, d), n, d,
                                                      gx.data_ptr() if n else None, d, gw.data_ptr(), ws.data_ptr(),
                                                      ws_bytes, _stream(gx))
    _lib.check(rc, "ptgnn_amd_weighted_pool_backward_f32")
    return gx, gw


def attention_pool_supported(dim: int, num_heads: int) -> bool:
    return bool(_lib.load().ptgnn_amd_attention_pool_supported(int(dim), int(num_heads)))


def _attention_pool_args(x: torch.Tensor, u: torch.Tensor, plan: GraphPlan, what: str):
    _require_cuda_f32("x", x)
    _require_cuda_f32("u", u, dims=3)
    x = _rowmajor(x)
    n, d = x.shape
    G, H = plan.num_nodes, u.shape[1]
    if n != plan.num_edges or tuple(u.shape) != (G, H, d) or plan.perm is None:
        raise _lib.PtgnnAmdError(f"{what}: x {tuple(x.shape)}, u {tuple(u.shape)} do not fit a plan of "
                                 f"{plan.num_edges} elements in {G} samples")
    return x, u.contiguous(), n, d, G, H


def attention_pool(x: torch.Tensor, u: torch.Tensor, plan: GraphPlan):
    lib = _lib.load()
    x, u, n, d, G, H = _attention_pool_args(x, u, plan, "attention_pool")
    out = torch.empty(G, H, d, dtype=torch.float32, device=x.device)
    stats = torch.empty(G, 2 * H, dtype=torch.float32, device=x.device)
    if G == 0:
        return out, stats
    ws_bytes = int(lib.ptgnn_amd_attention_pool_workspace_bytes(G, n, d, H))
    ws = _workspace(ws_bytes, x.device)
    plan.wait()
    with _timed("attention_pool", bytes=4.0 * (n * d + 2 * G * H * d) + 4.0 * n):
        rc = lib.ptgnn_amd_attention_pool_f32(*_rows_arg(x, d), u.data_ptr(),
                                              plan.rowptr.data_ptr(), plan.perm.data_ptr() if n else None, G, n, d, H,
                                              out.data_ptr(), stats.data_ptr(), ws.data_ptr(), ws_bytes, _stream(out))
    _lib.check(rc, "ptgnn_amd_attention_pool_f32")
    return out, stats


def attention_pool_backward(x: torch.Tensor, u: torch.Tensor, plan: GraphPlan, pooled: torch.Tensor,
                            stats: torch.Tensor, grad_out: torch.Tensor):
    lib = _lib.load()
    x, u, n, d, G, H = _attention_pool_args(x, u, plan, "attention_pool_backward")
    _require_cuda_f32("grad_out", grad_out, dims=3)
    pooled, stats, grad_out = pooled.contiguous(), stats.contiguous(), grad_out.contiguous()
    if tuple(grad_out.shape) != (G, H, d) or tuple(pooled.shape) != (G, H, d) or tuple(stats.shape) != (G, 2 * H):
        raise _lib.PtgnnAmdError(f"attention_pool_backward: grad_out {tuple(grad_out.shape)} / pooled "
                                 f"{tuple(pooled.shape)} / stats {tuple(stats.shape)} do not match ({G}, {H}, {d})")
    gx = torch.empty(n, d, dtype=torch.float32, device=x.device)
    gu = torch.empty(G, H, d, dtype=torch.float32, device=x.device)
    if G == 0:
# ... 977 lines not shown
```

Baseline: 1.335 billion edges/s.

## Mirror GRU input rows into concat residual buffer to skip residual copy

The GRU kernel can now write its input hidden state into a preallocated concat-residual buffer while it already has those rows loaded. The Python model loop sets up that buffer ahead of time and tells the later ConcatResidualLayer, which then skips its separate copy when the source tensor's version is unchanged. This removes one N×H read/write pass per residual in exchange for extra stores inside the GRU kernel, cross-layer hint bookkeeping, and an early hoist of the h loads. It also adds a compile-time store-policy macro.

```diff
diff --git a/include/ptgnn_amd.h b/include/ptgnn_amd.h
--- a/include/ptgnn_amd.h
+++ b/include/ptgnn_amd.h
@@ -333,6 +333,10 @@
                            const float *w_ih, const float *w_hh, const float *b_ih,
                            const float *b_hh, int64_t n, int32_t m, int32_t hd, float *out,
                            int64_t ld_out, void *stream);
+int ptgnn_amd_gru_cell_mirror_f32(const float *a, int64_t ld_a, const float *h, int64_t ld_h,
+                                  const float *w_ih, const float *w_hh, const float *b_ih,
+                                  const float *b_hh, int64_t n, int32_t m, int32_t hd, float *out,
+                                  int64_t ld_out, float *mirror, int64_t ld_mirror, int *mirrored, void *stream);
 
 size_t ptgnn_amd_weighted_pool_workspace_bytes(int64_t num_segments, int64_t num_elements, int32_t dim);
 int ptgnn_amd_weighted_pool_f32(const float *x, int64_t ld_x, const float *w, const int32_t *rowptr,
diff --git a/ptgnn_amd/_lib.py b/ptgnn_amd/_lib.py
--- a/ptgnn_amd/_lib.py
+++ b/ptgnn_amd/_lib.py
@@ -85,6 +85,8 @@
                                                        _i64, _vp, _vp, _vp, _c.c_size_t, _vp]),
     "ptgnn_amd_gru_cell_f32": (_c.c_int, [_vp, _i64, _vp, _i64, _vp, _vp, _vp, _vp, _i64, _i32, _i32,
                                           _vp, _i64, _vp]),
+    "ptgnn_amd_gru_cell_mirror_f32": (_c.c_int, [_vp, _i64, _vp, _i64, _vp, _vp, _vp, _vp, _i64, _i32, _i32,
+                                                 _vp, _i64, _vp, _i64, _c.POINTER(_c.c_int), _vp]),
     "ptgnn_amd_gru_cell_train_f32": (_c.c_int, [_vp, _i64, _vp, _i64, _vp, _vp, _vp, _vp, _i64, _i32, _i32,
                                                 _vp, _i64, _vp, _vp]),
     "ptgnn_amd_gru_cell_backward_gates_f32": (_c.c_int, [_vp, _i64, _vp, _vp, _i64, _i64, _i32, _vp, _vp, _vp,
diff --git a/ptgnn_amd/csrc/dense_f32.hip b/ptgnn_amd/csrc/dense_f32.hip
--- a/ptgnn_amd/csrc/dense_f32.hip
+++ b/ptgnn_amd/csrc/dense_f32.hip
@@ -431,13 +431,18 @@
 
 static int gru_launch(const float *a, int64_t ld_a, const float *h, int64_t ld_h, const float *w_ih,
                       const float *w_hh, const float *b_ih, const float *b_hh, int64_t n, int32_t m,
-                      int32_t hd, float *out, int64_t ld_out, float *gates, void *stream_) {
+                      int32_t hd, float *out, int64_t ld_out, float *gates, void *stream_, float *mirror = nullptr,
+                      int64_t ld_mirror = 0, int *mirrored = nullptr) {
+  if (mirrored) *mirrored = 0;
   PTGNN_REQUIRE(n >= 0 && m > 0 && hd > 0, PTGNN_AMD_EINVAL, "gru_cell: bad sizes");
   if (n == 0) return PTGNN_AMD_OK;
   PTGNN_REQUIRE(a && h && w_ih && w_hh && b_ih && b_hh && out, PTGNN_AMD_EINVAL, "gru_cell: null");
   PTGNN_REQUIRE(ld_a >= m && ld_h >= hd && ld_out >= hd, PTGNN_AMD_EINVAL, "gru_cell: bad ld");
   PTGNN_REQUIRE(out != h, PTGNN_AMD_EINVAL, "gru_cell: in-place update is not supported");
-  if (stream_gru(a, ld_a, h, ld_h, w_ih, w_hh, b_ih, b_hh, n, m, hd, out, ld_out, gates, (hipStream_t)stream_)) {
+  PTGNN_REQUIRE(!mirror || (mirrored && mirror != out && ld_mirror >= hd), PTGNN_AMD_EINVAL,
+                "gru_cell: a mirror needs `mirrored`, ld_mirror >= hd and rows of its own");
+  if (stream_gru(a, ld_a, h, ld_h, w_ih, w_hh, b_ih, b_hh, n, m, hd, out, ld_out, gates, (hipStream_t)stream_, mirror,
+                 ld_mirror, mirrored)) {
     PTGNN_LAUNCH_CHECK();
     return PTGNN_AMD_OK;
   }
@@ -464,6 +469,16 @@
                                       const float *b_hh, int64_t n, int32_t m, int32_t hd,
                                       float *out, int64_t ld_out, void *stream_) {
   return gru_launch(a, ld_a, h, ld_h, w_ih, w_hh, b_ih, b_hh, n, m, hd, out, ld_out, nullptr, stream_);
+}
+
+extern "C" int ptgnn_amd_gru_cell_mirror_f32(const float *a, int64_t ld_a, const float *h, int64_t ld_h,
+                                             const float *w_ih, const float *w_hh, const float *b_ih,
+                                             const float *b_hh, int64_t n, int32_t m, int32_t hd,
+                                             float *out, int64_t ld_out, float *mirror, int64_t ld_mirror,
+                                             int *mirrored, void *stream_) {
+  PTGNN_REQUIRE(mirrored != nullptr, PTGNN_AMD_EINVAL, "gru_cell_mirror: mirrored is null");
+  return gru_launch(a, ld_a, h, ld_h, w_ih, w_hh, b_ih, b_hh, n, m, hd, out, ld_out, nullptr, stream_, mirror,
+                    ld_mirror, mirrored);
 }
 
 extern "C" int ptgnn_amd_gru_cell_train_f32(const float *a, int64_t ld_a, const float *h, int64_t ld_h,
diff --git a/ptgnn_amd/csrc/stream_gemm.h b/ptgnn_amd/csrc/stream_gemm.h
--- a/ptgnn_amd/csrc/stream_gemm.h
+++ b/ptgnn_amd/csrc/stream_gemm.h
@@ -25,7 +25,8 @@
                   int64_t ld_add = 0);
 int stream_gru(const float *a, int64_t ld_a, const float *h, int64_t ld_h, const float *w_ih,
                const float *w_hh, const float *b_ih, const float *b_hh, int64_t n, int32_t m, int32_t hd,
-               float *out, int64_t ld_out, float *gates, hipStream_t st);
+               float *out, int64_t ld_out, float *gates, hipStream_t st, float *mirror = nullptr,
+               int64_t ld_mirror = 0, int *mirrored = nullptr);
 int stream_edge_supported(int32_t state_dim, int32_t msg_dim, int use_dst);
 int stream_edge_masked_supported(int32_t state_dim, int32_t msg_dim);
 struct StreamEdgeMask {
diff --git a/ptgnn_amd/csrc/stream_gemm.hip b/ptgnn_amd/csrc/stream_gemm.hip
--- a/ptgnn_amd/csrc/stream_gemm.hip
+++ b/ptgnn_amd/csrc/stream_gemm.hip
@@ -188,9 +188,14 @@
                                            __builtin_amdgcn_readfirstlane((int)bytes), 0x00020000);
 }
 
+#ifndef PTGNN_STORE_POLICY
+#define PTGNN_STORE_POLICY 0
+#endif
+constexpr int kStoreAux = PTGNN_STORE_POLICY == 1 ? 0x10 : PTGNN_STORE_POLICY == 2 ? 0x2 : 0;
+
 __device__ __forceinline__ void store_row4(__amdgpu_buffer_rsrc_t rsrc, int lane_bytes, int uniform_bytes, float4 o) {
   const u32x4 v = {__float_as_uint(o.x), __float_as_uint(o.y), __float_as_uint(o.z), __float_as_uint(o.w)};
-  __builtin_amdgcn_raw_buffer_store_b128(v, rsrc, lane_bytes + uniform_bytes, 0, 0);
+  __builtin_amdgcn_raw_buffer_store_b128(v, rsrc, lane_bytes + uniform_bytes, 0, kStoreAux);
 }
 
 template <int ACT, bool BIAS = true>
@@ -355,6 +360,7 @@
   const float *w_ih, *w_hh, *b_ih, *b_hh;
   int64_t n; int M, H;
   float *out; int64_t ld_out; float *gates;
+  float *mirror; int64_t ld_mirror;
   int nrb, ncs, rps, run_len;
   int lds_floats;
   int split;
@@ -383,13 +389,22 @@
   const __amdgpu_buffer_rsrc_t gate_rsrc =
       rows_descriptor(p.gates ? p.gates + row0 * (int64_t)(4 * p.H) + j0 : p.out, 4 * (int64_t)p.H, p.n - row0, 3 * p.H + 32);
 #endif
+  float4 hv[4];
 #pragma unroll
   for (int q = 0; q < 4; ++q) {
+    const int64_t hrow = row0 + 8 * q + trow;
+    hv[q] = *reinterpret_cast<const float4 *>(p.h + (hrow < p.n ? hrow : p.n - 1) * p.ld_h + j0 + tcol);
+    __builtin_amdgcn_sched_barrier(0);
+  }
+#pragma unroll
+  for (int q = 0; q < 4; ++q) {
+#ifdef PTGNN_GLOBAL_STORES
     int64_t hrow = row0 + 8 * q + trow;
     const bool rvalid = hrow < p.n;
     hrow = rvalid ? hrow : p.n - 1;
+#endif
     float hp[4];
-    tq_untranspose(tq, lane, li, hi, *reinterpret_cast<const float4 *>(p.h + hrow * p.ld_h + j0 + tcol), hp);
+    tq_untranspose(tq, lane, li, hi, hv[q], hp);
     float res[4], rg[4], zg[4], ng[4], hn[4];
     {
 #pragma clang fp contract(off)
@@ -436,6 +451,21 @@
       store_row4(gate_rsrc, gl, gu + 12 * p.H, o_h);
 #endif
     }
+  }
+  if (p.mirror) {
+#ifdef PTGNN_GLOBAL_STORES
+#pragma unroll
+    for (int q = 0; q < 4; ++q) {
+      const int64_t hrow = row0 + 8 * q + trow;
+      if (hrow < p.n) *reinterpret_cast<float4 *>(p.mirror + hrow * p.ld_mirror + j0 + tcol) = hv[q];
+    }
+#else
+    const __amdgpu_buffer_rsrc_t mirror_rsrc =
+        rows_descriptor(p.mirror + row0 * p.ld_mirror + j0, p.ld_mirror, p.n - row0, 32);
+#pragma unroll
+    for (int q = 0; q < 4; ++q)
+      store_row4(mirror_rsrc, trow * (int)p.ld_mirror * 4 + tcol * 4, 8 * q * (int)p.ld_mirror * 4, hv[q]);
+#endif
   }
 }
 
@@ -1258,9 +1288,17 @@
   return 1;
 }
 
+static bool rows_overlap(const float *x, int64_t ld_x, int cols_x, const float *y, int64_t ld_y, int cols_y, int64_t n) {
+  const uintptr_t x0 = (uintptr_t)x, x1 = x0 + (size_t)((n - 1) * ld_x + cols_x) * 4;
+  const uintptr_t y0 = (uintptr_t)y, y1 = y0 + (size_t)((n - 1) * ld_y + cols_y) * 4;
+  return x0 < y1 && y0 < x1;
+}
+
 int stream_gru(const float *a, int64_t ld_a, const float *h, int64_t ld_h, const float *w_ih,
                const float *w_hh, const float *b_ih, const float *b_hh, int64_t n, int32_t m, int32_t hd,
-               float *out, int64_t ld_out, float *gates, hipStream_t st) {
+               float *out, int64_t ld_out, float *gates, hipStream_t st, float *mirror, int64_t ld_mirror,
+               int *mirrored) {
+  if (mirrored) *mirrored = 0;
   const int mode = stream_gemm_mode();
   if (mode == 0) return 0;
   if (m % 64 != 0 || hd % 64 != 0 || ld_a % 4 != 0 || ld_h % 4 != 0 || ld_out % 4 != 0 || !aligned16(a) ||
@@ -1273,6 +1311,7 @@
   GruArgs p;
   p.a = a; p.ld_a = ld_a; p.h = h; p.ld_h = ld_h; p.w_ih = w_ih; p.w_hh = w_hh; p.b_ih = b_ih; p.b_hh = b_hh;
   p.n = n; p.M = m; p.H = hd; p.out = out; p.ld_out = ld_out; p.gates = gates;
+  p.mirror = nullptr; p.ld_mirror = 0;
   p.nrb = (int)((n + 31) / 32);
   p.ncs = hd / 32;
   p.split = 0;
@@ -1297,6 +1336,11 @@
   {
     auto kern = k_stream_gru;
     if (!set_lds(kern, lds_launch)) return 0;
+    if (mirror && mirrored && !gates && aligned16(mirror) && ld_mirror % 4 == 0 && ld_mirror >= hd &&
+        !rows_overlap(mirror, ld_mirror, hd, h, ld_h, hd, n) && !rows_overlap(mirror, ld_mirror, hd, a, ld_a, m, n)) {
+      p.mirror = mirror; p.ld_mirror = ld_mirror;
+      *mirrored = 1;
+    }
     kern<<<grid, 512, lds_launch, st>>>(p);
   }
   count_launch(PTGNN_AMD_KERNEL_STREAM_GRU);
diff --git a/ptgnn_amd/gnn.py b/ptgnn_amd/gnn.py
--- a/ptgnn_amd/gnn.py
+++ b/ptgnn_amd/gnn.py
@@ -4,7 +4,9 @@
 from torch import nn
 
 from ptgnn_amd import ops
-from ptgnn_amd.layers import AbstractMessagePassingLayer, ConcatResidualLayer, forward_scope, set_output_hint
+from ptgnn_amd.layers import (AbstractMessagePassingLayer, ConcatResidualLayer, GatedMessagePassingLayer,
+                              _ResidualOriginLayer, forward_scope, residual_mirror_enabled, set_input_mirror_hint,
+                              set_output_hint, take_input_mirror_report, tensor_version)
 
 try:
     from ptgnn.neuralmodels.gnn.structs import GnnOutput
@@ -120,25 +122,46 @@
         all_states = [node_representations]
         with forward_scope():
             layers = list(self.__message_passing_layers)
+            early = {}
+            offer = None
             for li, mp_layer in enumerate(layers):
                 buf = None
                 nxt = layers[li + 1] if li + 1 < len(layers) else None
-                if (isinstance(nxt, ConcatResidualLayer) and node_representations.is_cuda and not return_all_states
-                        and node_representations.dtype == torch.float32
-                        and not (torch.is_grad_enabled() and (node_representations.requires_grad or self.training))):
+                hints_ok = (node_representations.is_cuda and not return_all_states
+                            and node_representations.dtype == torch.float32
+                            and not (torch.is_grad_enabled() and (node_representations.requires_grad or self.training)))
+                if isinstance(nxt, ConcatResidualLayer) and hints_ok:
                     out_dim = mp_layer.output_state_dimension
-                    buf = nxt.make_result_buffer(node_representations.shape[0], out_dim, node_representations)
+                    buf = early.pop(nxt, None)
+                    if buf is None or buf.shape[1] != nxt.input_state_dimension + out_dim:
+                        buf = nxt.make_result_buffer(node_representations.shape[0], out_dim, node_representations)
                     set_output_hint(buf[:, buf.shape[1] - out_dim:])
+                mirrored_src = None
+                if offer is not None and hints_ok:
+                    mirrored_src = (node_representations, tensor_version(node_representations))
+                    set_input_mirror_hint(offer[1])
                 try:
                     node_representations = mp_layer(
                         node_states=node_representations, adjacency_lists=adjacency_lists,
                         node_to_graph_idx=node_to_graph_idx, reference_node_ids=reference_node_ids,
                         reference_node_graph_idx=reference_node_graph_idx,
                         edge_features=edge_feature_embeddings)
+                    done = take_input_mirror_report() if mirrored_src is not None else None
                 finally:
                     set_output_hint(None)
+                    set_input_mirror_hint(None)
+                if done is not None and done is offer[1] and mirrored_src[1] is not None:
+                    offer[0]._ptgnn_amd_mirror_of = mirrored_src
+                offer = None
                 if buf is not None and node_representations.data_ptr() == buf[:, buf.shape[1] - out_dim:].data_ptr():
                     node_representations._ptgnn_amd_concat_buffer = buf
+                target = mp_layer.target_layer if isinstance(mp_layer, _ResidualOriginLayer) else None
+                if (isinstance(target, ConcatResidualLayer) and isinstance(nxt, GatedMessagePassingLayer) and hints_ok
+                        and residual_mirror_enabled() and target in layers[li + 2:]):
+                    front = layers[layers.index(target, li + 2) - 1]
+                    early[target] = target.make_result_buffer(node_representations.shape[0], front.output_state_dimension,
+                                                              node_representations)
+                    offer = (early[target], early[target][:, :target.input_state_dimension])
                 all_states.append(node_representations)
         if return_all_states:
             node_representations = torch.cat(all_states, dim=-1)
diff --git a/ptgnn_amd/layers.py b/ptgnn_amd/layers.py
--- a/ptgnn_amd/layers.py
+++ b/ptgnn_amd/layers.py
@@ -88,6 +88,42 @@
     if vector_stores and (hint.data_ptr() % 16 != 0 or (rows > 1 and hint.stride(0) % 4 != 0) or hint.stride(1) != 1):
         return None
     return hint
+
+
+def residual_mirror_enabled() -> bool:
+    return os.environ.get("PTGNN_AMD_RESIDUAL_MIRROR", "1") not in ("", "0")
+
+
+def set_input_mirror_hint(buf: Optional[torch.Tensor]) -> None:
+    _SCOPE.mirror_hint = buf
+    _SCOPE.mirror_done = None
+
+
+def _take_input_mirror_hint(rows: int, cols: int, like: torch.Tensor) -> Optional[torch.Tensor]:
+    hint = getattr(_SCOPE, "mirror_hint", None)
+    _SCOPE.mirror_hint = None
+    if hint is None or torch.is_grad_enabled() and like.requires_grad:
+        return None
+    if tuple(hint.shape) != (rows, cols) or hint.dtype != torch.float32 or hint.device != like.device or hint.stride(1) != 1:
+        return None
+    return hint
+
+
+def _report_input_mirrored(view: torch.Tensor) -> None:
+    _SCOPE.mirror_done = view
+
+
+def take_input_mirror_report() -> Optional[torch.Tensor]:
+    done = getattr(_SCOPE, "mirror_done", None)
+    _SCOPE.mirror_done = None
+    return done
+
+
+def tensor_version(t: torch.Tensor) -> Optional[int]:
+    try:
+        return t._version
+    except RuntimeError:
+        return None
 
 
 def _no_grad_needed(*tensors) -> bool:
@@ -434,10 +470,16 @@
             w16 = _half_weights(self, "edge_w16", inputs, ops.HALF_KIND_LINEAR, H, w.shape[0],
                                 lambda: w.to(inputs).contiguous())
             msgs, col, tb = ops.linear(node_states, w, inputs=inputs, rounded=w16), None, None
-        return ops.aggregate_gru(msgs, plan, M, self.__aggregation_fn, node_states, gru.weight_ih, gru.weight_hh,
-                                 gru.bias_ih, gru.bias_hh, type_bits=tb, col=col,
-                                 out=_take_output_hint(num_nodes, H, node_states), inputs=inputs,
-                                 rounded=self._rounded_gru_weights(inputs))
+        mirror = _take_input_mirror_hint(num_nodes, H, node_states)
+        out = ops.aggregate_gru(msgs, plan, M, self.__aggregation_fn, node_states, gru.weight_ih, gru.weight_hh,
+                                gru.bias_ih, gru.bias_hh, type_bits=tb, col=col,
+                                out=_take_output_hint(num_nodes, H, node_states), inputs=inputs,
+                                rounded=self._rounded_gru_weights(inputs), mirror=mirror)
+        if mirror is not None:
+            out, mirrored = out
+            if mirrored:
+                _report_input_mirrored(mirror)
+        return out
 
     def _forward_features_inference(self, node_states, adjacency_lists, plan, edge_features) -> torch.Tensor:
         gru = self.__state_update
@@ -1153,6 +1195,10 @@
         return node_states
 
     @property
+    def target_layer(self):
+        return self.__target_layer
+
+    @property
     def input_state_dimension(self) -> int:
         return self.__input_dim
 
@@ -1197,7 +1243,11 @@
         buf = getattr(node_states, "_ptgnn_amd_concat_buffer", None)
         if (buf is not None and buf.shape[1] == orig.shape[1] + node_states.shape[1] and buf.dtype == orig.dtype
                 and node_states.data_ptr() == buf[:, orig.shape[1]:].data_ptr()):
-            buf[:, : orig.shape[1]].copy_(orig)
+            src, version = buf.__dict__.pop("_ptgnn_amd_mirror_of", (None, None))
+            if src is orig and version is not None and version == tensor_version(orig) and residual_mirror_enabled():
+                ops.count_skipped_residual_copy()
+            else:
+                buf[:, : orig.shape[1]].copy_(orig)
             return buf
         return torch.cat((orig, node_states), dim=-1)
 
diff --git a/ptgnn_amd/ops.py b/ptgnn_amd/ops.py
--- a/ptgnn_amd/ops.py
+++ b/ptgnn_amd/ops.py
@@ -84,6 +84,18 @@
     now = launch_counts(aggregation=True, char_cnn=True, heads=True, sequence=True, decode=True, beam=True, half=True,
                         edge16=True, half_training=True, edge16_dst=True)
     return {k: now[k] - v for k, v in before.items() if now[k] != v}
+
+
+_SKIPPED_RESIDUAL_COPIES = 0
+
+
+def skipped_residual_copies() -> int:
+    return _SKIPPED_RESIDUAL_COPIES
+
+
+def count_skipped_residual_copy() -> None:
+    global _SKIPPED_RESIDUAL_COPIES
+    _SKIPPED_RESIDUAL_COPIES += 1
 
 
 def _stream(t: torch.Tensor) -> int:
@@ -1532,7 +1544,7 @@
 
 
 def gru_cell(a: torch.Tensor, h: torch.Tensor, w_ih, w_hh, b_ih, b_hh, out: Optional[torch.Tensor] = None,
-             inputs=None, rounded=None) -> torch.Tensor:
+             inputs=None, rounded=None, mirror: Optional[torch.Tensor] = None):
     lib = _lib.load()
     _require_cuda_f32("a", a)
     _require_cuda_f32("h", h)
@@ -1543,6 +1555,9 @@
         out = torch.empty(n, hd, dtype=torch.float32, device=a.device)
     elif tuple(out.shape) != (n, hd) or out.dtype != torch.float32 or out.stride(1) != 1 or not out.is_cuda:
         raise _lib.PtgnnAmdError(f"gru_cell: `out` must be a float32 CUDA [{n}, {hd}] view with unit inner stride")
+    if mirror is not None and (tuple(mirror.shape) != (n, hd) or mirror.dtype != torch.float32 or mirror.stride(1) != 1
+                               or mirror.device != out.device):
+        raise _lib.PtgnnAmdError(f"gru_cell: `mirror` must be a float32 CUDA [{n}, {hd}] view with unit inner stride")
     half = _half_inputs(inputs)
     if half is not None and half_supported(HALF_KIND_GRU, m, hd, half) and _half_rows_ok(a) and _half_rows_ok(h):
         given = rounded if rounded is not None else (None, None)
@@ -1552,14 +1567,24 @@
                                              b_ih.contiguous().data_ptr(), b_hh.contiguous().data_ptr(), n, m, hd,
                                              HALF_IDS[half], out.data_ptr(), _ld(out), _stream(out))
         _lib.check(rc, "ptgnn_amd_half_gru_cell")
+        return out if mirror is None else (out, False)
+    if mirror is None:
+        with _timed("gru_cell", flops=2.0 * n * 3 * hd * (m + hd), bytes=4.0 * (n * (m + 2 * hd) + 3 * hd * (m + hd))):
+            rc = lib.ptgnn_amd_gru_cell_f32(a.data_ptr(), _ld(a), h.data_ptr(), _ld(h),
+                                            w_ih.contiguous().data_ptr(), w_hh.contiguous().data_ptr(),
+                                            b_ih.contiguous().data_ptr(), b_hh.contiguous().data_ptr(),
+                                            n, m, hd, out.data_ptr(), _ld(out), _stream(out))
+        _lib.check(rc, "ptgnn_amd_gru_cell_f32")
         return out
-    with _timed("gru_cell", flops=2.0 * n * 3 * hd * (m + hd), bytes=4.0 * (n * (m + 2 * hd) + 3 * hd * (m + hd))):
-        rc = lib.ptgnn_amd_gru_cell_f32(a.data_ptr(), _ld(a), h.data_ptr(), _ld(h),
-                                        w_ih.contiguous().data_ptr(), w_hh.contiguous().data_ptr(),
-                                        b_ih.contiguous().data_ptr(), b_hh.contiguous().data_ptr(),
-                                        n, m, hd, out.data_ptr(), _ld(out), _stream(out))
-    _lib.check(rc, "ptgnn_amd_gru_cell_f32")
-    return out
+    mirrored = ctypes.c_int(0)
+    with _timed("gru_cell", flops=2.0 * n * 3 * hd * (m + hd), bytes=4.0 * (n * (m + 3 * hd) + 3 * hd * (m + hd))):
+        rc = lib.ptgnn_amd_gru_cell_mirror_f32(a.data_ptr(), _ld(a), h.data_ptr(), _ld(h),
+                                               w_ih.contiguous().data_ptr(), w_hh.contiguous().data_ptr(),
+                                               b_ih.contiguous().data_ptr(), b_hh.contiguous().data_ptr(),
+                                               n, m, hd, out.data_ptr(), _ld(out), mirror.data_ptr(), _ld(mirror),
+                                               ctypes.byref(mirrored), _stream(out))
+    _lib.check(rc, "ptgnn_amd_gru_cell_mirror_f32")
+    return out, bool(mirrored.value)
 
 
 AGG_PIPELINE = int(os.environ.get("PTGNN_AMD_AGG_PIPELINE", "1"))
@@ -1568,12 +1593,13 @@
 
 def aggregate_gru(ysrc: torch.Tensor, plan: GraphPlan, msg_dim: int, reduce: str, h: torch.Tensor, w_ih, w_hh, b_ih,
                   b_hh, type_bits: Optional[int] = None, col: Optional[torch.Tensor] = None,
-                  out: Optional[torch.Tensor] = None, inputs=None, rounded=None) -> torch.Tensor:
+                  out: Optional[torch.Tensor] = None, inputs=None, rounded=None,
+                  mirror: Optional[torch.Tensor] = None):
     N = plan.num_nodes
     pieces = AGG_PIPELINE
     if (pieces < 2 or N < AGG_PIPELINE_MIN_ROWS or N < 64 * pieces or torch.cuda.is_current_stream_capturing()):
         agg = gather_reduce(ysrc, plan, msg_dim, reduce, type_bits=type_bits, col=col)
-        return gru_cell(agg, h, w_ih, w_hh, b_ih, b_hh, out=out, inputs=inputs, rounded=rounded)
+        return gru_cell(agg, h, w_ih, w_hh, b_ih, b_hh, out=out, inputs=inputs, rounded=rounded, mirror=mirror)
     dev = h.device
     hd = h.shape[1]
     agg = torch.empty(N, msg_dim, dtype=torch.float32, device=dev)
@@ -1581,6 +1607,7 @@
         out = torch.empty(N, hd, dtype=torch.float32, device=dev)
     bounds = [min(N, (N * i // pieces + 31) // 32 * 32) for i in range(pieces)] + [N]
     main, side = torch.cuda.current_stream(dev), _side_stream(dev)
+    mirrored = mirror is not None
     plan.wait()
     gather_reduce(ysrc, plan, msg_dim, reduce, type_bits=type_bits, col=col, out=agg, rows=(bounds[0], bounds[1]))
     first_done = torch.cuda.Event()
@@ -1598,12 +1625,18 @@
         if i > 0:
             main.wait_event(ready[i - 1])
         lo, hi = bounds[i], bounds[i + 1]
-        if hi > lo:
+        if hi > lo and mirror is None:
             gru_cell(agg[lo:hi], h[lo:hi], w_ih, w_hh, b_ih, b_hh, out=out[lo:hi], inputs=inputs, rounded=rounded)
-    return out
-
-
-def gru_cell_train(a: torch.Tensor, h: torch.Tensor, w_ih, w_hh, b_ih, b_hh, inputs=None, rounded=None):
+        elif hi > lo:
+            mirrored = gru_cell(agg[lo:hi], h[lo:hi], w_ih, w_hh, b_ih, b_hh, out=out[lo:hi], inputs=inputs,
+                                rounded=rounded, mirror=mirror[lo:hi])[1] and mirrored
+    return out if mirror is None else (out, mirrored)
+
+
+def gru_cell_train(a: torch.Tensor, h: torch.Tensor, w_ih, w_hh, b_ih, b_hh, inputs=None, rounded=None,
+                   mirror: Optional[torch.Tensor] = None):
+    if mirror is not None:
+        return gru_cell_train(a, h, w_ih, w_hh, b_ih, b_hh, inputs=inputs, rounded=rounded) + (False,)
     lib = _lib.load()
     _require_cuda_f32("a", a)
     _require_cuda_f32("h", h)
```

New measurement: 1.341 billion edges/s, median of 6. No clear change (+0.5%).
